# Gryph66/gymwipe

Measured on AMD Instinct MI355X. Metric: env.step()/s at 65 536 parallel envs, counter-traffic band-assign, higher is better.
Workload: dtype f64

## Files before the change

### gymwipe_amd/_native.py

```python
import ctypes as C
import os
import subprocess

_PKG = os.path.dirname(os.path.abspath(__file__))
LIB_PATH = os.environ.get("GW_LIB") or os.path.join(_PKG, "lib", "libgymwipe_amd.so")
CSRC = os.path.join(_PKG, "csrc")

ABI_VERSION = 1
MAX_DEVICES = 32
MAX_RADIOS = MAX_DEVICES + 1
QUEUE_CAP = 100
MAX_NSTATES = 16

OK, EINVAL, ENODEVICE, EHIP, ENOMEM, EUNSUPPORTED, EFIELD = 0, -1, -2, -3, -4, -5, -6
FLAG_CARRY, FLAG_REFEXC, FLAG_TIE, FLAG_BADACT, FLAG_INTERNAL = 1, 2, 4, 8, 16
CFG_PER_ENV_STATS = 1
CFG_EXPLICIT_QUEUE = 2
CFG_NO_COUNTER_TRAFFIC = 4
CFG_PEER_RECEIVE = 8
CFG_FLOAT_DURATION = 16
CFG_PER_ENV_GEOMETRY = 32

EXPORTS = (
    "gw_abi_version", "gw_last_error", "gw_device_count", "gw_config_default", "gw_create",
    "gw_destroy", "gw_reset", "gw_step", "gw_step_fb", "gw_rollout", "gw_rollout_policy", "gw_rollout_policy_stats", "gw_transition_stats", "gw_rollout_episodes", "gw_rollout_episodes_stats", "gw_transition_stats_ep", "gw_rollout_autoreset", "gw_rollout_population", "gw_rollout_episodes_scored", "gw_rollout_population_scored", "gw_rollout_autoreset_scored", "gw_rollout_backlog", "gw_rollout_backlog_population", "gw_rollout_controller", "gw_rollout_controller_population", "gw_rollout_policy_stats_delivered", "gw_rollout_episodes_stats_delivered", "gw_transition_stats_delivered", "gw_set_position", "gw_set_positions", "gw_received", "gw_delivered", "gw_enqueue", "gw_pack_feedback", "gw_unpack_feedback", "gw_get_state",
    "gw_stats_read", "gw_clear_flags", "gw_state_bytes", "gw_snapshot_bytes", "gw_get_snapshot", "gw_set_state", "gw_link_info", "gw_noise_states", "gw_selftest_queue", "gw_selftest_runq",
    "gw_selftest_fastmath", "gw_selftest_launches",
    "gw_plant_config_default", "gw_plant_create", "gw_plant_destroy", "gw_plant_update", "gw_plant_set_input",
    "gw_plant_state_ptr", "gw_plant_get_state", "gw_plant_feedback", "gw_plant_update_feedback", "gw_now_ptr", "gw_pendulum_step",
    "gw_ctrl_config_default", "gw_ctrl_create", "gw_ctrl_destroy", "gw_ctrl_step", "gw_ctrl_get_state",
    "gw_ctrl_set_initial", "gw_ctrl_reset", "gw_ctrl_rollout", "gw_ctrl_rollout_schedules",
    "gw_grid_config_default", "gw_grid_create", "gw_grid_destroy", "gw_grid_run", "gw_grid_get_state", "gw_grid_set_position",
)


class Config(C.Structure):
    _fields_ = [
        ("abi_version", C.c_int32),
        ("hip_device", C.c_int32),
        ("num_envs", C.c_int64),
        ("num_devices", C.c_int32),
        ("flags", C.c_int32),
        ("pos", (C.c_double * 2) * MAX_RADIOS),
        ("mult", C.c_int32 * MAX_DEVICES),
        ("dest", C.c_int32 * MAX_DEVICES),
        ("slot", C.c_double),
        ("frequency", C.c_double),
        ("bandwidth", C.c_double),
        ("temperature_c", C.c_double),
        ("bit_rate", C.c_double),
        ("code_rate", C.c_double),
        ("max_ber", C.c_double),
        ("tx_power_dbm", C.c_double),
        ("counter_interval", C.c_double),
        ("counter_bound", C.c_int32),
        ("payload_value", C.c_int32),
        ("mac_header_bytes", C.c_int32),
        ("net_header_bytes", C.c_int32),
        ("duration_factor", C.c_int32),
        ("max_duration", C.c_int32),
        ("extra_att_db", (C.c_double * MAX_RADIOS) * MAX_RADIOS),
        ("start_time", C.c_double),
    ]


class CtrlConfig(C.Structure):
    _fields_ = [
        ("net", Config),
        ("A", C.c_double * 16), ("B", C.c_double * 4), ("x0", C.c_double * 4), ("u0", C.c_double),
        ("ctrl_start_tick", C.c_int32), ("ctrl_period_ticks", C.c_int32),
    ]


class CtrlEpisodes(C.Structure):
    _fields_ = [("max_steps", C.c_int32), ("pad", C.c_int32), ("fail_deg", C.c_double)]


class PlantConfig(C.Structure):
    _fields_ = [
        ("abi_version", C.c_int32),
# ... 152 lines not shown
    L.gw_transition_stats_ep.restype = C.c_int
    L.gw_rollout_autoreset.argtypes = [vp, i32, vp, vp, C.POINTER(Episodes), vp, vp, vp, vp, vp, vp]
    L.gw_rollout_autoreset.restype = C.c_int
    L.gw_rollout_population.argtypes = [vp, i32, C.POINTER(Population), C.c_uint64, C.c_uint64, C.c_uint64, C.POINTER(Episodes), vp, vp, vp]
    L.gw_rollout_population.restype = C.c_int
    L.gw_rollout_episodes_scored.argtypes = [vp, i32, vp, C.c_uint64, C.c_uint64, C.c_uint64, C.POINTER(Episodes), C.POINTER(Score),
                                             vp, vp, vp, vp, vp, vp, vp, vp, vp, vp]
    L.gw_rollout_episodes_scored.restype = C.c_int
    L.gw_rollout_population_scored.argtypes = [vp, i32, C.POINTER(Population), C.c_uint64, C.c_uint64, C.c_uint64, C.POINTER(Episodes),
                                               C.POINTER(Score), vp, vp, vp]
    L.gw_rollout_population_scored.restype = C.c_int
    L.gw_rollout_autoreset_scored.argtypes = [vp, i32, vp, vp, C.POINTER(Episodes), C.POINTER(Score), vp, vp, vp, vp, vp, vp, vp]
    L.gw_rollout_autoreset_scored.restype = C.c_int
    L.gw_rollout_backlog.argtypes = [vp, i32, C.POINTER(BacklogPolicy), C.POINTER(Episodes), C.POINTER(Score), vp, vp, vp, vp, vp, vp, vp,
                                     vp, vp, vp]
    L.gw_rollout_backlog.restype = C.c_int
    L.gw_rollout_backlog_population.argtypes = [vp, i32, C.POINTER(BacklogPopulation), C.POINTER(Episodes), C.POINTER(Score), vp, vp]
    L.gw_rollout_backlog_population.restype = C.c_int
    L.gw_rollout_controller.argtypes = [vp, i32, C.POINTER(Controller), C.c_uint64, C.c_uint64, C.c_uint64, C.POINTER(Episodes),
                                        C.POINTER(Score), vp, vp, vp, vp, vp, vp, vp, vp, vp, vp, vp]
    L.gw_rollout_controller.restype = C.c_int
    L.gw_rollout_controller_population.argtypes = [vp, i32, C.POINTER(ControllerPopulation), C.c_uint64, C.c_uint64, C.c_uint64,
                                                   C.POINTER(Episodes), C.POINTER(Score), vp, vp, vp]
    L.gw_rollout_controller_population.restype = C.c_int
    L.gw_rollout_policy_stats_delivered.argtypes = L.gw_rollout_policy_stats.argtypes
    L.gw_rollout_policy_stats_delivered.restype = C.c_int
    L.gw_rollout_episodes_stats_delivered.argtypes = L.gw_rollout_episodes_stats.argtypes
    L.gw_rollout_episodes_stats_delivered.restype = C.c_int
    L.gw_transition_stats_delivered.argtypes = [vp, i32, vp, vp, vp, vp, vp, vp, vp, vp, vp, vp]
    L.gw_transition_stats_delivered.restype = C.c_int
    L.gw_received.argtypes, L.gw_received.restype = [vp, vp, vp], C.c_int
    L.gw_enqueue.argtypes, L.gw_enqueue.restype = [vp, i32, vp, vp], C.c_int
    L.gw_pack_feedback.argtypes, L.gw_pack_feedback.restype = [vp, C.c_int64, vp, vp, vp, vp, i32, vp], C.c_int
    L.gw_unpack_feedback.argtypes, L.gw_unpack_feedback.restype = [vp, C.c_int64, vp, vp, vp, vp, vp], C.c_int
    L.gw_delivered.argtypes, L.gw_delivered.restype = [vp, vp, vp], C.c_int
    L.gw_get_state.argtypes, L.gw_get_state.restype = [vp, C.c_char_p, vp, C.c_size_t], C.c_int
    L.gw_stats_read.argtypes, L.gw_stats_read.restype = [vp, C.POINTER(Stats)], C.c_int
    L.gw_state_bytes.argtypes, L.gw_state_bytes.restype = [vp, C.POINTER(C.c_uint64)], C.c_int
    L.gw_snapshot_bytes.argtypes, L.gw_snapshot_bytes.restype = [vp, C.POINTER(C.c_uint64)], C.c_int
    L.gw_get_snapshot.argtypes, L.gw_get_snapshot.restype = [vp, vp, C.c_uint64], C.c_int
    L.gw_set_state.argtypes, L.gw_set_state.restype = [vp, vp, C.c_uint64], C.c_int
    L.gw_link_info.argtypes = [vp, i32, i32, C.POINTER(C.c_double), C.POINTER(C.c_double)]
    L.gw_link_info.restype = C.c_int
    L.gw_noise_states.argtypes = [vp, i32, C.POINTER(i32), C.POINTER(C.c_double)]
    L.gw_noise_states.restype = C.c_int
    L.gw_selftest_queue.argtypes, L.gw_selftest_queue.restype = [C.c_uint64, i32, i32, i32], C.c_int
    L.gw_set_position.argtypes, L.gw_set_position.restype = [vp, i32, vp, vp, vp, vp], C.c_int
    L.gw_set_positions.argtypes, L.gw_set_positions.restype = [vp, vp, vp, vp], C.c_int
    L.gw_clear_flags.argtypes, L.gw_clear_flags.restype = [vp, vp], C.c_int
    L.gw_selftest_runq.argtypes, L.gw_selftest_runq.restype = [C.c_uint64, i32, i32, i32], C.c_int
    L.gw_selftest_fastmath.argtypes = [C.POINTER(Config), C.POINTER(i32)]
    L.gw_selftest_fastmath.restype = C.c_int
    L.gw_selftest_launches.argtypes, L.gw_selftest_launches.restype = [vp, C.c_char_p, i64], i64
    L.gw_plant_config_default.argtypes, L.gw_plant_config_default.restype = [C.POINTER(PlantConfig), i64], C.c_int
    L.gw_plant_create.argtypes, L.gw_plant_create.restype = [C.POINTER(PlantConfig), C.POINTER(vp)], C.c_int
    L.gw_plant_destroy.argtypes, L.gw_plant_destroy.restype = [vp], C.c_int
    L.gw_plant_update.argtypes, L.gw_plant_update.restype = [vp, vp, i64, vp], C.c_int
    L.gw_plant_set_input.argtypes, L.gw_plant_set_input.restype = [vp, vp, vp, vp], C.c_int
    L.gw_plant_state_ptr.argtypes, L.gw_plant_state_ptr.restype = [vp, C.POINTER(vp)], C.c_int
    L.gw_plant_get_state.argtypes, L.gw_plant_get_state.restype = [vp, C.c_char_p, vp, C.c_size_t], C.c_int
    L.gw_plant_feedback.argtypes, L.gw_plant_feedback.restype = [vp, vp, vp, vp, vp], C.c_int
    L.gw_ctrl_config_default.argtypes, L.gw_ctrl_config_default.restype = [C.POINTER(CtrlConfig), i64], C.c_int
    L.gw_ctrl_create.argtypes, L.gw_ctrl_create.restype = [C.POINTER(CtrlConfig), C.POINTER(vp)], C.c_int
    L.gw_ctrl_destroy.argtypes, L.gw_ctrl_destroy.restype = [vp], C.c_int
    L.gw_ctrl_step.argtypes, L.gw_ctrl_step.restype = [vp, vp, vp, vp, vp, vp, vp], C.c_int
    L.gw_ctrl_get_state.argtypes, L.gw_ctrl_get_state.restype = [vp, C.c_char_p, vp, C.c_size_t], C.c_int
    L.gw_ctrl_set_initial.argtypes, L.gw_ctrl_set_initial.restype = [vp, vp, vp, vp, vp], C.c_int
    L.gw_ctrl_reset.argtypes, L.gw_ctrl_reset.restype = [vp, vp, vp, vp], C.c_int
    L.gw_ctrl_rollout.argtypes = [vp, C.c_int32, vp, vp, C.POINTER(CtrlEpisodes), vp, vp, vp, vp, vp]
    L.gw_ctrl_rollout.restype = C.c_int
    L.gw_ctrl_rollout_schedules.argtypes = [vp, C.c_int32, vp, C.c_int32, C.c_int32, C.POINTER(CtrlEpisodes), vp, vp]
    L.gw_ctrl_rollout_schedules.restype = C.c_int
    L.gw_plant_update_feedback.argtypes, L.gw_plant_update_feedback.restype = [vp, vp, C.c_int64, vp, vp, vp, vp], C.c_int
    L.gw_now_ptr.argtypes, L.gw_now_ptr.restype = [vp, C.POINTER(vp), C.POINTER(i64)], C.c_int
    L.gw_pendulum_step.argtypes, L.gw_pendulum_step.restype = [vp, vp, vp, vp, vp, vp, vp, vp], C.c_int
    L.gw_grid_config_default.argtypes, L.gw_grid_config_default.restype = [C.POINTER(GridConfig), i64, i32], C.c_int
    L.gw_grid_create.argtypes, L.gw_grid_create.restype = [C.POINTER(GridConfig), vp, C.POINTER(vp)], C.c_int
    L.gw_grid_destroy.argtypes, L.gw_grid_destroy.restype = [vp], C.c_int
    L.gw_grid_run.argtypes, L.gw_grid_run.restype = [vp, C.c_double, vp], C.c_int
    L.gw_grid_get_state.argtypes, L.gw_grid_get_state.restype = [vp, C.c_char_p, vp, C.c_size_t], C.c_int
    L.gw_grid_set_position.argtypes, L.gw_grid_set_position.restype = [vp, i32, vp, vp, vp], C.c_int
    if L.gw_abi_version() != ABI_VERSION:
        raise ImportError("gymwipe_amd: ABI mismatch (library %d, python %d); rebuild"
                          % (L.gw_abi_version(), ABI_VERSION))
    _lib = L
    return L


_fast = False


def fast():
    global _fast
    if _fast is False:
        _fast = None
        path = os.path.join(os.path.dirname(LIB_PATH), "_gw_fast.so")
        if os.path.exists(path) and not os.environ.get("GW_NO_PYFAST"):
            try:
                import importlib.machinery
                import importlib.util
                loader = importlib.machinery.ExtensionFileLoader("_gw_fast", path)
                spec = importlib.util.spec_from_loader("_gw_fast", loader)
                mod = importlib.util.module_from_spec(spec)
                loader.exec_module(mod)
                L = lib()
                mod.bind(C.cast(L.gw_step, C.c_void_p).value, C.cast(L.gw_pendulum_step, C.c_void_p).value,
# ... 18 lines not shown
```

### gymwipe_amd/csrc/ct_common.hip.h

```cpp
#pragma once
#include <hip/hip_runtime.h>
#include "gw_internal.h"
#include "gw_queue.h"
#include "gw_fastmath.h"

#ifdef GW_STAMPS
#define STAMP(i)                                                                              \
    do {                                                                                      \
        __builtin_amdgcn_sched_barrier(0);                                                    \
        unsigned long long _t;                                                                \
        asm volatile("s_memtime %0\n\ts_waitcnt lgkmcnt(0)" : "=s"(_t)::"memory");            \
        __builtin_amdgcn_sched_barrier(0);                                                    \
        if ((threadIdx.x & 63) == 0)                                                          \
            st.stamps[(((size_t)blockIdx.x * ((blockDim.x + 63) >> 6)) + (threadIdx.x >> 6)) * 16 + (i)] = _t; \
    } while (0)
#else
#define STAMP(i) do { } while (0)
#endif

namespace gwk {

typedef GwTally Tally;

struct TxTimes { double t_s, t_h, t_e, stop; };
// ... 70 lines not shown
        u32x4_ w; __builtin_memcpy(&w, &v, 16);
        asm volatile("global_store_dwordx4 %0, %1, off sc1\n\ts_nop 1" ::"v"(ptr), "v"(w) : "memory");
    } else if constexpr (sizeof(T) == 8) {
        unsigned long long w; __builtin_memcpy(&w, &v, 8);
        asm volatile("global_store_dwordx2 %0, %1, off sc1" ::"v"(ptr), "v"(w) : "memory");
    } else if constexpr (sizeof(T) == 4) {
        unsigned w; __builtin_memcpy(&w, &v, 4);
        asm volatile("global_store_dword %0, %1, off sc1" ::"v"(ptr), "v"(w) : "memory");
    } else {
        static_assert(sizeof(T) == 1, "gw_store_wt: 1, 4, 8 or 16 bytes");
        unsigned w = (unsigned)*reinterpret_cast<const uint8_t*>(&v);
        asm volatile("global_store_byte %0, %1, off sc1" ::"v"(ptr), "v"(w) : "memory");
    }
#endif
}

template <class T, class Off>
__device__ __forceinline__ T ld(const void* base, Off byte_off)
{
    return *reinterpret_cast<const T*>(reinterpret_cast<const char*>(base) + byte_off);
}
template <class T, class Off>
__device__ __forceinline__ T ld_global(const void* base, Off byte_off)
{
#if defined(__HIP_DEVICE_COMPILE__)
    return *(const __attribute__((address_space(1))) T*)(reinterpret_cast<const char*>(base) + byte_off);
#else
    return *reinterpret_cast<const T*>(reinterpret_cast<const char*>(base) + byte_off);
#endif
}
template <class T, class Off>
__device__ __forceinline__ void st_(void* base, Off byte_off, const T& v)
{
    gw_store_wt(reinterpret_cast<T*>(reinterpret_cast<char*>(base) + byte_off), v);
}
template <class T, class Off>
__device__ __forceinline__ void st_plain(void* base, Off byte_off, const T& v)
{
    *reinterpret_cast<T*>(reinterpret_cast<char*>(base) + byte_off) = v;
}

__device__ __forceinline__ uint32_t byte_of(uint32_t x, uint32_t y, uint32_t z, uint32_t w, uint32_t idx)
{
    const uint32_t lo = (idx & 4u) ? y : x;
    const uint32_t hi = (idx & 4u) ? w : z;
    const uint32_t v = (idx & 8u) ? hi : lo;
    return (v >> ((idx & 3u) * 8u)) & 0xffu;
}
__device__ __forceinline__ uint32_t word_of(const uint4& w, int i)
{
    return i == 0 ? w.x : (i == 1 ? w.y : (i == 2 ? w.z : w.w));
}

__device__ __forceinline__ void publish_env_counters(uint32_t* sa, uint32_t N, uint32_t e, uint32_t pop, uint32_t deliv,
                                                     uint32_t bad, uint32_t fl, uint32_t steps)
{
    if (pop)
        __hip_atomic_fetch_add(reinterpret_cast<unsigned long long*>(sa) + e, (unsigned long long)pop | ((unsigned long long)deliv << 32),
                               __ATOMIC_RELAXED, __HIP_MEMORY_SCOPE_AGENT);
    if (bad) __hip_atomic_fetch_add(sa + (size_t)2 * N + e, bad, __ATOMIC_RELAXED, __HIP_MEMORY_SCOPE_AGENT);
    if (fl)  __hip_atomic_fetch_or(sa + (size_t)3 * N + e, fl, __ATOMIC_RELAXED, __HIP_MEMORY_SCOPE_AGENT);
    if (e == 0u)
        __hip_atomic_fetch_add(reinterpret_cast<unsigned long long*>(sa + (size_t)4 * N), (unsigned long long)steps,
                               __ATOMIC_RELAXED, __HIP_MEMORY_SCOPE_AGENT);
}

__device__ __forceinline__ double ber_bpsk_dev(double sig_mw, double noise_mw, double ten_log_br)
{
    const double s = 10 * log10(sig_mw);
    const double n = 10 * log10(noise_mw);
    if (s <= n) return 0.5;
    const double ratio_db = s - n - ten_log_br;
    const double ratio = pow(10.0, ratio_db / 10);
    const double x = sqrt(2 * ratio);
    const double e = 2.718281828459045;
    const double sqrt2pi = 2.5066282746310002;
    return (1 - pow(e, -1.4 * x)) * pow(e, -(pow(x, 2.0) / 2)) / (1.135 * sqrt2pi * x);
}

template <bool PER_ENV>
__device__ __forceinline__ double gw_link(const GwState& st, int R, int from, int to, uint32_t e)
{
    if (PER_ENV) return st.prx_env[((size_t)e * R + from) * gw_rp(R) + to];
    return st.prx_tab[from * R + to];
}
__device__ __forceinline__ double& gw_rx(const GwState& st, int R, int j, int64_t e)
{
    return st.rxp[(size_t)e * gw_rp(R) + j];
}


#define GW_LEAD_PARAMS uint32_t* __restrict__ ip, double* __restrict__ tw, uint32_t* __restrict__ tk, uint8_t* __restrict__ qb, \
                       const int32_t* __restrict__ device, const int32_t* __restrict__ duration, uint32_t n_envs, uint32_t dev_stage
#define GW_LEAD_PARAMS_U64 uint64_t ip_a, uint64_t tw_a, uint64_t tk_a, uint64_t qb_a, uint64_t device_a, uint64_t duration_a, \
                           uint32_t n_envs, uint32_t dev_stage
#define GW_LEAD_ARGS(st_) (st_).ip, (st_).tw, (st_).tk, (st_).qb, device, duration, (uint32_t)(st_).N, \
                          ((uint32_t)(st_).D | ((uint32_t)(st_).stage_chunks << 8))
#if defined(__HIP_DEVICE_COMPILE__)
#define GW_AS_CONST __attribute__((address_space(4)))
#else
#define GW_AS_CONST
#endif
template <int DT>
__device__ __forceinline__ GwDevConst hdr_const(const uint32_t* ip, int n_dev)
{
    const int D = DT > 0 ? DT : n_dev;
    const uint8_t* at = reinterpret_cast<const uint8_t*>(ip) - gw_blob_header(D) + gw_hdr_cst_off(D);
    return *(const GW_AS_CONST GwDevConst*)at;
}
template <class T>
__device__ __forceinline__ T* gw_as_global(T* p)
{
    return (T*)(__attribute__((address_space(1))) T*)p;
}
template <class T>
__device__ __forceinline__ T* gw_global_at(uint64_t address)
{
    return (T*)(__attribute__((address_space(1))) T*)address;
}
template <int DT>
__device__ __forceinline__ GwState hdr_state(uint32_t* ip, double* tw, uint32_t* tk, uint8_t* qb, uint32_t n_envs, int n_dev)
{
    const int D = DT > 0 ? DT : n_dev;
    const uint8_t* base = reinterpret_cast<const uint8_t*>(ip) - gw_blob_header(D);
    GwState st = *(const GW_AS_CONST GwState*)(base + gw_hdr_st_off(D));
    st.ip = ip; st.tw = tw; st.tk = tk; st.qb = qb; st.N = (int64_t)n_envs; st.D = D;
    st.blob = base;
#define GW_G(m) st.m = gw_as_global(st.m)
    GW_G(bph); GW_G(sa); GW_G(trans); GW_G(ber); GW_G(cls); GW_G(ber2); GW_G(cls2); GW_G(rxp); GW_G(prx_tab); GW_G(pos_tab);
    GW_G(extra_tab); GW_G(prx_env); GW_G(pos_env); GW_G(bcache); GW_G(talk); GW_G(stamps); GW_G(cst);
#undef GW_G
    return st;
}

__device__ __forceinline__ int ndigits(int v)
{
    return 1 + (v >= 10) + (v >= 100) + (v >= 1000) + (v >= 10000) + (v >= 100000) + (v >= 1000000) +
           (v >= 10000000) + (v >= 100000000) + (v >= 1000000000);
}


template <int CTRL, int ROW_MASK, bool OR>
__device__ __forceinline__ uint32_t gw_dpp_step(uint32_t v)
{
    const uint32_t o = (uint32_t)__builtin_amdgcn_update_dpp(0, (int)v, CTRL, ROW_MASK, 0xf, false);
    return OR ? (v | o) : (v + o);
}
template <bool OR>
__device__ __forceinline__ uint32_t gw_wave_total(uint32_t v)
{
    v = gw_dpp_step<0x111, 0xf, OR>(v);
    v = gw_dpp_step<0x112, 0xf, OR>(v);
    v = gw_dpp_step<0x114, 0xf, OR>(v);
    v = gw_dpp_step<0x118, 0xf, OR>(v);
    v = gw_dpp_step<0x142, 0xa, OR>(v);
    v = gw_dpp_step<0x143, 0xc, OR>(v);
    return (uint32_t)__builtin_amdgcn_readlane((int)v, 63);
}

__device__ __forceinline__ void publish_totals(unsigned long long* totals, const Tally& k, uint32_t k_steps,
                                               uint32_t k_bad, uint32_t fl_new)
{
    const uint32_t lane = threadIdx.x & 63u;
    const uint32_t w_deliv = gw_wave_total<false>(k.deliv), w_pop = gw_wave_total<false>(k.pop);
    const uint32_t w_app = gw_wave_total<false>(k.app), w_drop = gw_wave_total<false>(k.drop);
    const uint32_t w_steps = (uint32_t)__builtin_popcountll(__builtin_amdgcn_ballot_w64(k_steps != 0u));
    const uint32_t w_bad = (uint32_t)__builtin_popcountll(__builtin_amdgcn_ballot_w64(k_bad != 0u));
    const uint32_t w_tx = w_steps + w_pop;
    uint32_t w_fl = 0u;
    if (__builtin_amdgcn_ballot_w64(fl_new != 0u)) w_fl = gw_wave_total<true>(fl_new);
    if (lane < (uint32_t)GW_T_COUNT) {
        uint32_t w = w_steps;
        w = lane == (uint32_t)GW_T_TX ? w_tx : w;
        w = lane == (uint32_t)GW_T_DELIV ? w_deliv : w;
        w = lane == (uint32_t)GW_T_APP ? w_app : w;
        w = lane == (uint32_t)GW_T_POP ? w_pop : w;
        w = lane == (uint32_t)GW_T_DROP ? w_drop : w;
        w = lane == (uint32_t)GW_T_FLAGS ? w_fl : w;
        w = lane == (uint32_t)GW_T_BAD ? w_bad : w;
// ... 15 lines not shown
```

### gymwipe_amd/csrc/ct_rollout_backlog.hip

```cpp
#include "ct_rollout_sync.hip.h"

namespace {

struct BacklogEpisodes : ScoredStagedEpisodes {
    const uint32_t* s_w;
    const uint8_t* s_dur;
    int32_t* device_out;
    int32_t* duration_out;
    int32_t* seen_len;
    int du_cur;
    uint32_t q_cur;
    __device__ __forceinline__ void stage(const gw_backlog_policy& pol, int D, uint32_t* lds_w, uint8_t* lds_dur) const
    {
        for (int i = threadIdx.x; i < D; i += blockDim.x) lds_w[i] = (uint32_t)pol.w_len[i];
        for (int i = threadIdx.x; i <= GW_QUEUE_CAP; i += blockDim.x) lds_dur[i] = pol.duration_of_len[i];
    }
    template <int DT, class ARR>
    __device__ __forceinline__ int pick(ARR& len, int D, int max_duration)
    {
        const int n = DT ? DT : D;
        uint32_t q = len[0], p = s_w[0] * q;
        int d = 0;
#pragma unroll
        for (int i = 1; i < n; ++i) {
// ... 70 lines not shown
            if (i < (uint32_t)D) lds_w[i] = gw_backlog_weight((int32_t)v);
            if (i >= W) reinterpret_cast<uint32_t*>(lds_dur)[i - W] = v;
        }
    }
};

template <int DT, int MODE>
__global__ __launch_bounds__(64) void ct_rollout_backlog_pop(GwState st, GwDevConst c, int K, GwEpisodeArgs ea, gw_score w,
                                                            const gw_backlog_policy* __restrict__ policies, uint32_t M, int64_t* pop_tally)
{
    __shared__ uint32_t s_score_w[DT == 0 ? GW_MAX_DEVICES : DT];
    __shared__ uint32_t s_backlog_w[DT == 0 ? GW_MAX_DEVICES : DT];
    __shared__ __attribute__((aligned(4))) uint8_t s_backlog_dur[(GW_QUEUE_CAP + 1 + 3) / 4 * 4];
    __shared__ unsigned long long s_ep_tally[GW_EP_COLS];
    static_assert(sizeof(gw_backlog_policy) == 4u * GW_MAX_DEVICES + sizeof s_backlog_dur, "the table's dwords fill its LDS copy");
    BacklogPopulationEpisodes src;
    src.ended = nullptr;
    src.latest_next = 0;
    src.sc.weights_at(s_score_w, w);
    src.delivered_out = nullptr;
    src.d_cur = 0; src.du_cur = 0; src.q_cur = 0;
    src.s_w = s_backlog_w; src.s_dur = s_backlog_dur;
    src.device_out = nullptr; src.duration_out = nullptr; src.seen_len = nullptr;
    const uint32_t pol_next = (blockIdx.x * 64u) / M;
    src.row = pop_tally + (size_t)pol_next * GW_EP_COLS;
#define GW_ROLLOUT_SRC_RESETS
#define GW_ROLLOUT_SRC_QUEUES
#define GW_ROLLOUT_SRC_STAGE                                                                                                     \
    src.sc.stage(w, DT == 0 ? c.D : DT);                                                                                         \
    src.stage_from(policies + pol_next, DT == 0 ? c.D : DT, s_backlog_w, s_backlog_dur);                                         \
    gw_ep_zero(s_ep_tally);
#define GW_BACKLOG_POP_PIN(x) asm volatile("" : "+s"(x))
    GW_BACKLOG_POP_PIN(K);
#define GW_ROLLOUT_SRC_FIRST                                                                                                     \
    src.ep.load(ea, e); src.sc.first();                                                                                          \
    GW_BACKLOG_POP_PIN(src.ep.max_steps); GW_BACKLOG_POP_PIN(src.ep.on_done); GW_BACKLOG_POP_PIN(src.sc.w_reward);
#define GW_ROLLOUT_SRC_TAKE                                                                                                      \
    queues_now();                                                                                                                \
    const int d = src.pick<DT>(len, D, c.max_duration), du = src.du_cur;
#define GW_ROLLOUT_SRC_CHECKED(bad) false
#define GW_ROLLOUT_SRC_STEPPED(at, latest, r, dn)                                                                                \
    (void)at;                                                                                                                    \
    {                                                                                                                            \
        const int32_t score_next = src.sc.of(r, src.d_cur, src.sc.delivered(kt.deliv));                                          \
        GW_ROLLOUT_EP_STEPPED(score_next, dn)                                                                                    \
        src.latest_next = cause_next ? 0 : latest;                                                                               \
    }
#include "ct_rollout_sync_body.h"
#undef GW_BACKLOG_POP_PIN
    GW_ROLLOUT_EP_TAIL(true, src.row)
}

template <bool CLAMP>
__device__ __forceinline__ void gw_backlog_select(const uint8_t* row, uint32_t D, uint32_t md, const gw_backlog_policy& pol, uint32_t& d_out,
                                                  uint32_t& du_out, uint32_t& q_out)
{
    auto weight = [&](uint32_t i) { return CLAMP ? gw_backlog_weight(pol.w_len[i]) : (uint32_t)pol.w_len[i]; };
    uint32_t q = row[0], p = weight(0) * q, d = 0;
    for (uint32_t i = 1; i < D; ++i) {
        const uint32_t qi = row[i], pi = weight(i) * qi;
        const bool more = pi > p;
        p = more ? pi : p; q = more ? qi : q; d = more ? i : d;
    }
    d_out = d;
    du_out = gw_min_u32((uint32_t)pol.duration_of_len[gw_min_u32(q, (uint32_t)GW_QUEUE_CAP)], md - 1u);
    q_out = q;
}
__global__ __launch_bounds__(256) void backlog_select_rows(uint32_t N, uint32_t D, uint32_t RB, uint32_t md, gw_backlog_policy pol,
                                                           const uint8_t* __restrict__ qb, int32_t* __restrict__ device_out,
                                                           int32_t* __restrict__ duration_out, int32_t* __restrict__ seen_len)
{
    const uint32_t e = blockIdx.x * blockDim.x + threadIdx.x;
    if (e >= N) return;
    uint32_t d, du, q;
    gw_backlog_select<false>(qb + (size_t)e * RB, D, md, pol, d, du, q);
    device_out[e] = (int32_t)d;
    duration_out[e] = (int32_t)du;
    seen_len[e] = (int32_t)q;
}
__global__ __launch_bounds__(256) void backlog_select_pop_rows(uint32_t N, uint32_t D, uint32_t RB, uint32_t md, uint32_t M,
                                                               const gw_backlog_policy* __restrict__ policies,
                                                               const uint8_t* __restrict__ qb, int32_t* __restrict__ device_out,
                                                               int32_t* __restrict__ duration_out)
{
    const uint32_t e = blockIdx.x * blockDim.x + threadIdx.x;
    if (e >= N) return;
    uint32_t d, du, q;
    gw_backlog_select<true>(qb + (size_t)e * RB, D, md, policies[e / M], d, du, q);
    device_out[e] = (int32_t)d;
    duration_out[e] = (int32_t)du;
}

}

int gw_launch_rollout_backlog_sfx(const GwState& st, const GwDevConst& cst, const GwChunk& ch, const gw_backlog_policy& pol,
                                  const gw_episodes& ep, const gw_score& score, int32_t* obs_next, const GwRows& out, int32_t* seen_len,
                                  int32_t* delivered)
{
    if (fused_unavailable(st, cst, ch.K, GW_FUSED_NO_TABLE)) return GW_EUNSUPPORTED;
    return launch_fused(st, cst, ch, GW_LS_ROLLOUT_BACKLOG, GW_FUSED_NO_TABLE, GW_KERNEL_OF(ct_rollout_backlog), episode_args(ep, obs_next),
                        score, pol, out.device, out.duration, seen_len, out.obs, out.reward, out.done, out.ended, delivered);
}
int gw_launch_backlog_select(const GwState& st, const GwDevConst& cst, const gw_backlog_policy& pol, const GwRows& row, int32_t* seen_len,
                             void* stream)
{
    hipLaunchKernelGGL(backlog_select_rows, dim3((unsigned)((st.N + 255) / 256)), dim3(256), 0, (hipStream_t)stream, (uint32_t)st.N,
                       (uint32_t)st.D, (uint32_t)st.RB, (uint32_t)cst.max_duration, pol, (const uint8_t*)st.qb, row.device, row.duration,
                       seen_len);
    return gw_launch_status();
}

int gw_launch_rollout_backlog_pop_sfx(const GwState& st, const GwDevConst& cst, const GwChunk& ch, const gw_backlog_population& pop,
                                      const gw_episodes& ep, const gw_score& score, int32_t* obs_next)
{
    if (fused_unavailable(st, cst, ch.K, GW_FUSED_NO_TABLE) || pop.envs_per_policy % 64 != 0) return GW_EUNSUPPORTED;
    return launch_fused(st, cst, ch, GW_LS_ROLLOUT_BACKLOG_POP, GW_FUSED_NO_TABLE, GW_KERNEL_OF(ct_rollout_backlog_pop),
                        episode_args(ep, obs_next), score, pop.policies_dev, (uint32_t)pop.envs_per_policy, pop.tally_dev);
}
int gw_launch_backlog_select_pop(const GwState& st, const GwDevConst& cst, const gw_backlog_population& pop, const GwRows& row, void* stream)
{
    hipLaunchKernelGGL(backlog_select_pop_rows, dim3((unsigned)((st.N + 255) / 256)), dim3(256), 0, (hipStream_t)stream, (uint32_t)st.N,
                       (uint32_t)st.D, (uint32_t)st.RB, (uint32_t)cst.max_duration, (uint32_t)pop.envs_per_policy, pop.policies_dev,
                       (const uint8_t*)st.qb, row.device, row.duration);
    return gw_launch_status();
}
```

### gymwipe_amd/csrc/ct_rollout_sfx.hip

```cpp
#include "ct_rollout_sync.hip.h"

namespace {


constexpr int TP_ENVS = 64, TP_STEPS = 64;

__global__ __launch_bounds__(256) void pack_actions_kernel(uint32_t N, int K, int Kp, const int32_t* __restrict__ device,
                                                           const int32_t* __restrict__ duration, uint16_t* __restrict__ packed)
{
    __shared__ __attribute__((aligned(16))) uint16_t tile[TP_ENVS][TP_STEPS + 2];
    const uint32_t e0 = blockIdx.x * TP_ENVS;
    const int t = threadIdx.x;
    const bool vec_ok = (N & 3u) == 0;
    for (int k0 = 0; k0 < Kp; k0 += TP_STEPS) {
        const int c4 = (t & 15) * 4, r = t >> 4;
#pragma unroll
        for (int pass = 0; pass < TP_STEPS / 16; ++pass) {
            const int kk = pass * 16 + r, k = k0 + kk;
            uint32_t v[4] = {0xffffu, 0xffffu, 0xffffu, 0xffffu};
            if (k < K) {
                int32_t dv[4], du[4];
                const uint32_t e = e0 + (uint32_t)c4;
                if (vec_ok && e + 3 < N) {
                    const int4 a = *reinterpret_cast<const int4*>(device + (size_t)k * N + e);
// ... 66 lines not shown
                    *reinterpret_cast<int4*>(obs + (size_t)k * N + e) = make_int4(o[0], o[1], o[2], o[3]);
                    *reinterpret_cast<float4*>(reward + (size_t)k * N + e) = make_float4(rw[0], rw[1], rw[2], rw[3]);
                    *reinterpret_cast<uchar4*>(done + (size_t)k * N + e) = make_uchar4(dn[0], dn[1], dn[2], dn[3]);
                } else {
                    for (int j = 0; j < 4 && e + j < N; ++j) {
                        obs[(size_t)k * N + e + j] = o[j]; reward[(size_t)k * N + e + j] = rw[j]; done[(size_t)k * N + e + j] = dn[j];
                    }
                }
            }
        }
        __syncthreads();
    }
}

template <int DT, int MODE>
__global__ __launch_bounds__(256) void ct_rollout_sfx_kernel(GwState st, GwDevConst c, int K, int Kp,
                                                            const uint16_t* __restrict__ actions,
                                                            uint8_t* __restrict__ feedback)
{
    constexpr bool GEN = DT == 0;
    constexpr int DM = GEN ? GW_MAX_DEVICES : DT;
    constexpr int NWC = (2 * DM + 1 + 15) / 16;
    constexpr int S = GW_MAX_NSTATES;
    const int D = GEN ? c.D : DT, R = D + 1, RRM = D;
    const uint32_t N = (uint32_t)st.N;
    const uint32_t e = blockIdx.x * blockDim.x + threadIdx.x;

    constexpr int TRANS_B = ((DM + 1) * (DM + 1) * S + 15) / 16 * 16;
    __shared__ __attribute__((aligned(16))) uint8_t s_trans[TRANS_B];
    __shared__ __attribute__((aligned(16))) double  s_ber[2 * DM * S];
    __shared__ __attribute__((aligned(16))) uint8_t s_cls[2 * DM * S];
    __shared__ uint32_t s_cols[GEN ? (3 * DM + 1) * 64 : 1];
    __shared__ uint2 s_mi[GEN ? DM : 1];
    __shared__ uint32_t s_term[GEN ? DM : 1];
    if constexpr (GEN) {
        for (int i = threadIdx.x; i < D; i += blockDim.x) {
            s_mi[i] = make_uint2((uint32_t)st.cst->mult[i], st.cst->inv16[i]);
            s_term[i] = st.cst->term[i];
        }
    }
    {
        const int n_tr = (R * R * S + 15) >> 4, n_be = (2 * D * S * 8) >> 4, n_cl = (2 * D * S) >> 4;
        for (int i = threadIdx.x; i < n_tr; i += blockDim.x) *reinterpret_cast<uint4*>(s_trans + ((uint32_t)i << 4)) = ld<uint4>(st.trans, (uint32_t)i << 4);
        for (int i = threadIdx.x; i < n_be; i += blockDim.x) *reinterpret_cast<uint4*>(reinterpret_cast<uint8_t*>(s_ber) + ((uint32_t)i << 4)) = ld<uint4>(st.ber2, (uint32_t)i << 4);
        for (int i = threadIdx.x; i < n_cl; i += blockDim.x) *reinterpret_cast<uint4*>(s_cls + ((uint32_t)i << 4)) = ld<uint4>(st.cls2, (uint32_t)i << 4);
    }
    __syncthreads();
    if (e >= N) return;

    const uint32_t RB = GEN ? (uint32_t)st.RB : 16u * NWC;
    const uint32_t o16 = e << 4, oq = e * RB;
    const uint4 ip = ld<uint4>(st.ip, o16);
    const double2 tw = ld<double2>(st.tw, o16);
    const uint4 tk = ld<uint4>(st.tk, o16);
    typename ArrSel<GEN, DM>::rw len, tb;
    typename ArrSel<GEN, DM + 1>::rw sta;
    if constexpr (GEN) {
        uint32_t* col = s_cols + (threadIdx.x & 63);
        len.p = col; tb.p = col + DM * 64; sta.p = col + 2 * DM * 64;
        for (int i = 0; i < D; ++i) len[i] = st.qb[oq + (uint32_t)i];
        for (int j = 0; j < R; ++j) sta[j] = st.qb[oq + (uint32_t)(D + j)];
    } else {
        uint4 qw[NWC];
#pragma unroll
        for (int w = 0; w < NWC; ++w) qw[w] = ld<uint4>(st.qb, oq + 16u * w);
#pragma unroll
        for (int i = 0; i < DT; ++i) len[i] = (word_of(qw[i >> 4], (i >> 2) & 3) >> ((i & 3) * 8)) & 0xffu;
#pragma unroll
        for (int j = 0; j < DT + 1; ++j) sta[j] = (word_of(qw[(DT + j) >> 4], ((DT + j) >> 2) & 3) >> (((DT + j) & 3) * 8)) & 0xffu;
    }
    double now = tw.x, wake = tw.y;
    uint32_t tau = tk.x;
    const uint32_t nbp = tk.y;
    GwBp bpc, bpp;
    bpc.t0 = ip.x; bpc.c0 = ip.y;
    bpp.t0 = ip.z; bpp.c0 = ip.w;
    const GwBp* hist = st.bph + ((size_t)e << 7);
    uint32_t rvm = tk.z;
    int32_t last_abs = (int32_t)(tk.w & 0x7fffffffu);
    uint32_t dn = tk.w >> 31;

    constexpr bool FAST = MODE >= 1, NOLIM = MODE == 2;
    const StepMathT<FAST, NOLIM> m(c);
    const double slot = c.slot, br = c.bit_rate, hd = c.hdr_dur, hdr_bits = c.hdr_bits, interval = c.counter_interval;
    const double inv_interval = c.inv_interval, tie_filter = c.tie_filter;
    const bool fast_ticks = FAST || c.fast_ticks != 0;
    const uint32_t bound = (uint32_t)c.counter_bound, base_bytes = (uint32_t)(c.mac_hdr + c.net_hdr);
    const int mh = c.mac_hdr, pv = c.payload_value;
    uint32_t live_mask = 0u;
    if constexpr (GEN) {
        for (int i = 0; i < D; ++i) live_mask |= ((s_term[i] >> sta[i]) & 1u) ? 0u : (1u << i);
    }
    typename ArrSel<GEN, DM>::ro mult, term, inv16;
    if constexpr (GEN) {
        mult.p = st.cst->mult; mult.shift16 = 0; term.p = st.cst->term; term.shift16 = 1; inv16.p = st.cst->inv16; inv16.shift16 = 0;
    } else {
#pragma unroll
        for (int i = 0; i < DT; ++i) { mult.v[i] = (uint32_t)c.mult[i]; term.v[i] = c.term[i]; inv16.v[i] = c.inv16[i]; }
    }

    Tally kt = {0, 0, 0, 0, 0};
    uint32_t k_bad = 0, fl = 0;

    int k = 0;
    bool data_mode = false;
    bool finish = false;
    int d = 0;
    uint32_t len_d = 0, mult_d = 0, inv16_d = 65536u;
#pragma unroll
    for (int i = 0; i < D; ++i) tb[i] = tau;
    uint32_t n_data = 0, s_r_run = 0;
    double cur = now, stopw = 0.0, t_end = 0.0;
    bool cls_valid = false;
    uint32_t fbw = 0;

    const uint16_t* act = actions + (size_t)e * Kp;
    uint8_t* fbp = feedback + (size_t)e * Kp;
    uint4 aw = ld<uint4>(act, 0);

    auto put_feedback = [&](uint32_t byte) {
        fbw |= byte << ((k & 3) * 8);
        if ((k & 3) == 3 || k == K - 1) { st_plain(fbp, (uint32_t)(k & ~3), fbw); fbw = 0; }
        k++;
        if ((k & 7) == 0 && k < K) aw = ld<uint4>(act, (uint32_t)k * 2u);
    };

    while (k < K) {
        uint32_t s = 0;
        if (data_mode && !finish) {
            bool have = true;
            if (len_d == 0) {
                if (mult_d != 0u && wake < stopw) {
// ... 147 lines not shown
        {
            uint32_t kk = 0;
            double wj = wake;
            bool tiej = false;
            if (fast_ticks && gw_tick_jump(wake, cur, interval, inv_interval, incl, &kk, &wj, &tiej)) {
                wake = wj;
                if (tiej) fl |= GW_FLAG_TIE;
            } else {
                kk = 0;
                for (;;) {
                    const double w1 = wake + interval, w2 = w1 + interval, w3 = w2 + interval, w4 = w3 + interval;
                    const bool b0 = incl ? (wake <= cur) : (wake < cur);
                    const bool b1 = incl ? (w1 <= cur) : (w1 < cur);
                    const bool b2 = incl ? (w2 <= cur) : (w2 < cur);
                    const bool b3 = incl ? (w3 <= cur) : (w3 < cur);
                    if (incl && (wake == cur || w1 == cur || w2 == cur || w3 == cur)) fl |= GW_FLAG_TIE;
                    kk += (uint32_t)b0 + (uint32_t)b1 + (uint32_t)b2 + (uint32_t)b3;
                    wake = b3 ? w4 : (b2 ? w3 : (b1 ? w2 : (b0 ? w1 : wake)));
                    if (!b3) break;
                }
            }
            tau += kk;
            len_d = gw_len_after_ticks(len_d, kk, mult_d, kt);
        }
    }

    {
        uint32_t kk = 0;
        while (wake <= now) { if (wake == now) fl |= GW_FLAG_TIE; wake = wake + interval; kk++; }
        tau += kk;
#pragma unroll
        for (int i = 0; i < D; ++i) len[i] = gw_len_after_ticks(len[i], tau - tb[i], mult[i], kt);
    }

    if constexpr (GEN) {
        for (int i = 0; i < D; ++i) st.qb[oq + (uint32_t)i] = (uint8_t)len[i];
        for (int j = 0; j < R; ++j) st.qb[oq + (uint32_t)(D + j)] = (uint8_t)sta[j];
    } else {
        uint32_t nb[16 * NWC];
#pragma unroll
        for (int b = 0; b < 16 * NWC; ++b) nb[b] = 0u;
#pragma unroll
        for (int i = 0; i < DT; ++i) nb[i] = len[i];
#pragma unroll
        for (int j = 0; j < DT + 1; ++j) nb[DT + j] = sta[j];
#pragma unroll
        for (int w = 0; w < NWC; ++w) {
            const int b = 16 * w;
            uint4 o;
            o.x = nb[b + 0] | (nb[b + 1] << 8) | (nb[b + 2] << 16) | (nb[b + 3] << 24);
            o.y = nb[b + 4] | (nb[b + 5] << 8) | (nb[b + 6] << 16) | (nb[b + 7] << 24);
            o.z = nb[b + 8] | (nb[b + 9] << 8) | (nb[b + 10] << 16) | (nb[b + 11] << 24);
            o.w = nb[b + 12] | (nb[b + 13] << 8) | (nb[b + 14] << 16) | (nb[b + 15] << 24);
            st_plain(st.qb, oq + 16u * w, o);
        }
    }
    st_plain(st.tw, o16, make_double2(now, wake));
    st_plain(st.tk, o16, make_uint4(tau, nbp, rvm, (uint32_t)last_abs | (dn << 31)));
    publish_env_counters(st.sa, N, e, kt.pop, kt.deliv, k_bad, fl, (uint32_t)K);
}

template <int DT, int MODE>
__global__ __launch_bounds__(64) void ct_rollout_sync_kernel(GwState st, GwDevConst c, int K,
                                                            const int32_t* __restrict__ device, const int32_t* __restrict__ duration,
                                                            int32_t* __restrict__ obs, float* __restrict__ reward, uint8_t* __restrict__ done)
{
#define GW_ROLLOUT_SRC_STAGE
#define GW_ROLLOUT_SRC_FIRST GW_ROLLOUT_STAGED_FIRST
#define GW_ROLLOUT_SRC_TAKE GW_ROLLOUT_STAGED_TAKE
#define GW_ROLLOUT_SRC_CHECKED(bad) GW_ROLLOUT_STAGED_CHECKED(bad)
#define GW_ROLLOUT_SRC_STEPPED(at, latest, r, dn) GW_ROLLOUT_STORE_OUTPUTS(at, latest, r, dn)
#include "ct_rollout_sync_body.h"
}

}

int gw_launch_rollout_sfx(const GwState& st, const GwDevConst& cst, const GwChunk& ch, const int32_t* device, const int32_t* duration,
                          const GwRows& out)
{
    const int K = ch.K, Kp = (K + 15) / 16 * 16, k_cap = st.rcap;
    uint16_t* const act_buf = st.ract;
    uint8_t* const fb_buf = st.rfb;
    int32_t* const obs = out.obs;
    float* const reward = out.reward;
    uint8_t* const done = out.done;
    if (K <= 0 || Kp > k_cap) return GW_EUNSUPPORTED;
    const bool event_loop = getenv("GW_ROLLOUT_EVENT_LOOP") != nullptr && act_buf != nullptr && fb_buf != nullptr;
    if (!event_loop)
        return launch_fused(st, cst, ch, GW_LS_ROLLOUT_SYNC, GW_FUSED_NO_TABLE, GW_KERNEL_OF(ct_rollout_sync_kernel), device, duration,
                            obs, reward, done);
    const unsigned grid = (unsigned)((st.N + 63) / 64);
    const int mode = gw_step_mode(cst, ch.below_limits, false);
    hipStream_t s = (hipStream_t)ch.stream;
    uint64_t* const rec = ch.rec;
    if (cst.max_duration > 0xfe) return GW_EUNSUPPORTED;
    const uint32_t N = (uint32_t)st.N;
    const unsigned g256 = (unsigned)((st.N + TP_ENVS - 1) / TP_ENVS);
    hipLaunchKernelGGL(pack_actions_kernel, dim3(g256), dim3(256), 0, s, N, K, Kp, device, duration, act_buf);
    gw_with_dt<GW_DTS_ROLLOUT_LOOP>(st.D, [&](auto dt) {
        gw_with_mode(mode, [&](auto m) {
            gw_note_launch(rec, GW_LS_ROLLOUT + 3 * gw_ls_dt(decltype(dt)::value) + decltype(m)::value);
            hipLaunchKernelGGL((ct_rollout_sfx_kernel<decltype(dt)::value, decltype(m)::value>), dim3(grid), dim3(64), 0, s,
                               st, cst, K, Kp, (const uint16_t*)act_buf, fb_buf);
        });
    });
    if (const int rc = gw_launch_status()) return rc;
    hipLaunchKernelGGL(expand_feedback_kernel, dim3(g256), dim3(256), 0, s, N, K, Kp, cst.counter_bound,
                       cst.payload_value, fb_buf, obs, reward, done);
    return gw_launch_status();
}
```

### gymwipe_amd/csrc/ct_rollout_sync_body.h

```cpp
    constexpr bool GEN = DT == 0;
    constexpr int DM = GEN ? GW_MAX_DEVICES : DT;
    constexpr int NWC = (2 * DM + 1 + 15) / 16;
    constexpr int S = GW_MAX_NSTATES;
    const int D = GEN ? c.D : DT, R = D + 1, RRM = D;
    const uint32_t N = (uint32_t)st.N;
    const uint32_t e = blockIdx.x * blockDim.x + threadIdx.x;

    constexpr int TRANS_B = ((DM + 1) * (DM + 1) * S + 15) / 16 * 16;
    __shared__ __attribute__((aligned(16))) uint8_t s_trans[TRANS_B];
    __shared__ __attribute__((aligned(16))) double  s_ber[2 * DM * S];
    __shared__ __attribute__((aligned(16))) uint8_t s_cls[2 * DM * S];
    __shared__ uint32_t s_cols[GEN ? (3 * DM + 1) * 64 : 1];
    __shared__ uint2 s_mi[GEN ? DM : 1];
    __shared__ uint32_t s_term[GEN ? DM : 1];
    if constexpr (GEN) {
        for (int i = threadIdx.x; i < D; i += blockDim.x) {
            s_mi[i] = make_uint2((uint32_t)st.cst->mult[i], st.cst->inv16[i]);
            s_term[i] = st.cst->term[i];
        }
    }
    {
        const int n_tr = (R * R * S + 15) >> 4, n_be = (2 * D * S * 8) >> 4, n_cl = (2 * D * S) >> 4;
        for (int i = threadIdx.x; i < n_tr; i += blockDim.x) *reinterpret_cast<uint4*>(s_trans + ((uint32_t)i << 4)) = ld<uint4>(st.trans, (uint32_t)i << 4);
        for (int i = threadIdx.x; i < n_be; i += blockDim.x) *reinterpret_cast<uint4*>(reinterpret_cast<uint8_t*>(s_ber) + ((uint32_t)i << 4)) = ld<uint4>(st.ber2, (uint32_t)i << 4);
        for (int i = threadIdx.x; i < n_cl; i += blockDim.x) *reinterpret_cast<uint4*>(s_cls + ((uint32_t)i << 4)) = ld<uint4>(st.cls2, (uint32_t)i << 4);
    }
    GW_ROLLOUT_SRC_STAGE
    __syncthreads();
    if (e >= N) return;

    const uint32_t RB = GEN ? (uint32_t)st.RB : 16u * NWC;
    const uint32_t o16 = e << 4, oq = e * RB;
    const uint4 ip = ld<uint4>(st.ip, o16);
    const double2 tw = ld<double2>(st.tw, o16);
    const uint4 tk = ld<uint4>(st.tk, o16);
    typename ArrSel<GEN, DM>::rw len, tb;
    typename ArrSel<GEN, DM + 1>::rw sta;
    if constexpr (GEN) {
        uint32_t* col = s_cols + (threadIdx.x & 63);
        len.p = col; tb.p = col + DM * 64; sta.p = col + 2 * DM * 64;
        for (int i = 0; i < D; ++i) len[i] = st.qb[oq + (uint32_t)i];
        for (int j = 0; j < R; ++j) sta[j] = st.qb[oq + (uint32_t)(D + j)];
    } else {
        uint4 qw[NWC];
#pragma unroll
        for (int w = 0; w < NWC; ++w) qw[w] = ld<uint4>(st.qb, oq + 16u * w);
#pragma unroll
        for (int i = 0; i < DT; ++i) len[i] = (word_of(qw[i >> 4], (i >> 2) & 3) >> ((i & 3) * 8)) & 0xffu;
#pragma unroll
        for (int j = 0; j < DT + 1; ++j) sta[j] = (word_of(qw[(DT + j) >> 4], ((DT + j) >> 2) & 3) >> (((DT + j) & 3) * 8)) & 0xffu;
    }
    double now = tw.x, wake = tw.y;
    uint32_t tau = tk.x;
    uint32_t nbp = tk.y;
    GwBp bpc, bpp;
    bpc.t0 = ip.x; bpc.c0 = ip.y;
    bpp.t0 = ip.z; bpp.c0 = ip.w;
    const GwBp* hist = st.bph + ((size_t)e << 7);
    uint32_t rvm = tk.z;
    int32_t last_abs = (int32_t)(tk.w & 0x7fffffffu);
    uint32_t dn = tk.w >> 31;

    constexpr bool FAST = MODE >= 1, NOLIM = MODE == 2;
    const StepMathT<FAST, NOLIM> m(c);
    const double slot = c.slot, br = c.bit_rate, hd = c.hdr_dur, hdr_bits = c.hdr_bits, interval = c.counter_interval;
    const double inv_interval = c.inv_interval, tie_filter = c.tie_filter, coded_factor = c.coded_factor;
    const bool fast_ticks = FAST || c.fast_ticks != 0;
    const bool idem = c.idem_states != 0;
    const uint32_t bound = (uint32_t)c.counter_bound, base_bytes = (uint32_t)(c.mac_hdr + c.net_hdr);
    const int mh = c.mac_hdr, pv = c.payload_value;
    uint32_t live_mask = 0u;
    if constexpr (GEN) {
        for (int i = 0; i < D; ++i) live_mask |= ((s_term[i] >> sta[i]) & 1u) ? 0u : (1u << i);
    }
    typename ArrSel<GEN, DM>::ro mult, term, inv16;
    if constexpr (GEN) {
        mult.p = st.cst->mult; mult.shift16 = 0; term.p = st.cst->term; term.shift16 = 1; inv16.p = st.cst->inv16; inv16.shift16 = 0;
    } else {
#pragma unroll
        for (int i = 0; i < DT; ++i) { mult.v[i] = (uint32_t)c.mult[i]; term.v[i] = c.term[i]; inv16.v[i] = c.inv16[i]; }
    }
#pragma unroll
    for (int i = 0; i < D; ++i) tb[i] = tau;

    Tally kt = {0, 0, 0, 0, 0};
    uint32_t k_bad = 0, fl = 0;
    int k = 0;
    GW_ROLLOUT_SRC_FIRST
#ifdef GW_ROLLOUT_SRC_RESETS
    auto reset_env = [&]() {
        uint32_t kk = 0;
        while (wake <= now) { if (wake == now) fl |= GW_FLAG_TIE; wake = wake + interval; kk++; }
        tau += kk;
        GwBp* ring = st.bph + ((size_t)e << 7);
        GwBp cur; cur.t0 = bpc.t0; cur.c0 = 0u;
        if (bpc.t0 == tau) {
            ring[(nbp - 1u) & GW_RING_MASK] = cur;
        } else {
            bpp = bpc;
            cur.t0 = tau;
            ring[nbp & GW_RING_MASK] = cur;
            nbp += 1u;
        }
        bpc = cur;
        rvm = 0u; last_abs = 0; dn = 0u;
    };
#endif
#ifdef GW_ROLLOUT_SRC_QUEUES
    auto queues_now = [&]() {
        uint32_t kk = 0;
        while (wake <= now) { if (wake == now) fl |= GW_FLAG_TIE; wake = wake + interval; kk++; }
        tau += kk;
#pragma unroll
// ... 189 lines not shown
            for (int i = 0; i < D; ++i)
                if (i == d) { len[i] = len_d; tb[i] = tau; }
        }
        if (!all_term) {
#pragma unroll
            for (int i = 0; i < D; ++i) {
                if (i == d) continue;
                uint32_t si = s_trans[(uint32_t)((i * R + RRM) * S) + sta[i]];
                for (uint32_t n = 0; n < n_data; ++n) {
                    const uint32_t s2 = s_trans[(uint32_t)((i * R + d) * S) + si];
                    if (s2 == si) break;
                    si = s2;
                }
                sta[i] = si;
                if constexpr (GEN) live_mask = ((term[i] >> si) & 1u) ? (live_mask & ~(1u << i)) : (live_mask | (1u << i));
            }
        }
        sta[RRM] = s_r;
        const int32_t latest = pv * ((int)(rvm & 1u) - (int)((rvm >> 1) & 1u));
        const int32_t abs_d = latest < 0 ? -latest : latest;
        int32_t r = last_abs - abs_d;
        last_abs = abs_d;
        r = r > 10 ? 10 : (r < -10 ? -10 : r);
        now = t_end;
        put_feedback(latest, r);
    }

    {
        uint32_t kk = 0;
        while (wake <= now) { if (wake == now) fl |= GW_FLAG_TIE; wake = wake + interval; kk++; }
        tau += kk;
#pragma unroll
        for (int i = 0; i < D; ++i) len[i] = gw_len_after_ticks(len[i], tau - tb[i], mult[i], kt);
    }
    if constexpr (GEN) {
        for (int i = 0; i < D; ++i) st.qb[oq + (uint32_t)i] = (uint8_t)len[i];
        for (int j = 0; j < R; ++j) st.qb[oq + (uint32_t)(D + j)] = (uint8_t)sta[j];
    } else {
        uint32_t nb[16 * NWC];
#pragma unroll
        for (int b = 0; b < 16 * NWC; ++b) nb[b] = 0u;
#pragma unroll
        for (int i = 0; i < DT; ++i) nb[i] = len[i];
#pragma unroll
        for (int j = 0; j < DT + 1; ++j) nb[DT + j] = sta[j];
#pragma unroll
        for (int w = 0; w < NWC; ++w) {
            const int b = 16 * w;
            uint4 o;
            o.x = nb[b + 0] | (nb[b + 1] << 8) | (nb[b + 2] << 16) | (nb[b + 3] << 24);
            o.y = nb[b + 4] | (nb[b + 5] << 8) | (nb[b + 6] << 16) | (nb[b + 7] << 24);
            o.z = nb[b + 8] | (nb[b + 9] << 8) | (nb[b + 10] << 16) | (nb[b + 11] << 24);
            o.w = nb[b + 12] | (nb[b + 13] << 8) | (nb[b + 14] << 16) | (nb[b + 15] << 24);
            st_plain(st.qb, oq + 16u * w, o);
        }
    }
    st_plain(st.tw, o16, make_double2(now, wake));
    st_plain(st.tk, o16, make_uint4(tau, nbp, rvm, (uint32_t)last_abs | (dn << 31)));
    publish_env_counters(st.sa, N, e, kt.pop, kt.deliv, k_bad, fl, (uint32_t)K);
#undef GW_ROLLOUT_SRC_RESETS
#undef GW_ROLLOUT_SRC_QUEUES
#undef GW_ROLLOUT_SRC_STAGE
#undef GW_ROLLOUT_SRC_FIRST
#undef GW_ROLLOUT_SRC_TAKE
#undef GW_ROLLOUT_SRC_CHECKED
#undef GW_ROLLOUT_SRC_STEPPED
```

### gymwipe_amd/csrc/ct_step_sfx.hip

```cpp
#include "ct_common.hip.h"
#include "gw_dispatch.h"
#include "gw_queue.h"

using namespace gwk;


namespace {



#define PIN_V(x) asm volatile("" : "+v"(x))
#define PIN_S(x) asm volatile("" : "+s"(x))

template <int DT, bool FEEDBACK, int MODE, bool HALF = false>
__device__ __forceinline__ void ct_step_sfx_body(const GwState& st, const GwDevConst& c,
                                                 const int32_t* __restrict__ device,
                                                 const int32_t* __restrict__ duration,
                                                 int32_t* __restrict__ obs,
                                                 float* __restrict__ reward,
                                                 uint8_t* __restrict__ done,
                                                 uint8_t* __restrict__ fb,
                                                 int n_stage,
                                                 double& now_out, bool& live_out)
{
    constexpr bool PACKED = DT > 0;
    constexpr bool FAST = MODE >= 1, NOLIM = MODE == 2;
    constexpr int NWC = DT > 0 ? (2 * DT + 1 + 15) / 16 : 1;
    const uint32_t N = (uint32_t)st.N;
    const uint32_t e = HALF ? blockIdx.x * 32u + (threadIdx.x & 31u) : blockIdx.x * 64u + threadIdx.x;
    const int D = DT > 0 ? DT : c.D;
    const int R = D + 1, RRM = D;
    constexpr int S = GW_MAX_NSTATES;
    const uint32_t RB = PACKED ? 16u * NWC : (uint32_t)st.RB;

    STAMP(0);
    constexpr int DM = DT > 0 ? DT : GW_MAX_DEVICES;
    constexpr GwStripeLayout LM(DM);
    const GwStripeLayout L(D);
    constexpr int MAX_CH = LM.staged_chunks(GW_MAX_NSTATES);
    const int n_ch = n_stage < MAX_CH ? n_stage : MAX_CH;
    const int tid = threadIdx.x;
    constexpr int nthr = 64;
    constexpr int PER_FULL = (MAX_CH + 63) / 64;
    constexpr int PER = (DT > 0 && PER_FULL <= 11) ? PER_FULL : 1;
    constexpr bool one_pass = DT > 0 && PER_FULL <= 11;
    __shared__ __attribute__((aligned(16))) uint8_t s_blob[one_pass ? PER * 64 * 16 : MAX_CH * 16];
    uint4 r_ch[PER];
    if (one_pass) {
#pragma unroll
        for (int i = 0; i < PER; ++i) {
            const int ch = tid + i * nthr;
            r_ch[i] = ld<uint4>(st.blob, (uint32_t)(ch < n_ch ? ch : 0) << 4);
        }
    }

    Tally k = {0, 0, 0, 0, 0};
    uint32_t k_bad = 0;

    const bool live = e < N && (!HALF || threadIdx.x < 32u);
    const uint32_t el = live ? e : 0u;
    const uint32_t o16 = e << 4, o16l = el << 4;
    const uint32_t oq = e * RB, oql = el * RB;
    int d = device[el];
    int du = duration[el];
    uint4 ip = ld<uint4>(st.ip, o16l);
    const double2 tw = ld<double2>(st.tw, o16l);
    const uint4 tk = ld<uint4>(st.tk, o16l);
    uint4 qw[NWC];
#pragma unroll
    for (int w = 0; w < NWC; ++w) qw[w] = PACKED ? ld<uint4>(st.qb, oql + 16u * w) : make_uint4(0u, 0u, 0u, 0u);
    now_out = tw.x;
    live_out = live;
    if (one_pass) {
#pragma unroll
        for (int i = 0; i < PER; ++i) {
            const int ch = tid + i * nthr;
            *reinterpret_cast<uint4*>(s_blob + ((uint32_t)ch << 4)) = r_ch[i];
        }
    } else {
        for (int i = tid; i < n_ch; i += nthr) *reinterpret_cast<uint4*>(s_blob + ((uint32_t)i << 4)) = ld<uint4>(st.blob, (uint32_t)i << 4);
    }
    STAMP(1);
    __syncthreads();
    STAMP(2);

    StepMathT<FAST, NOLIM> m(c);
    double slot = c.slot, br = c.bit_rate, hd = c.hdr_dur, hdr_bits = c.hdr_bits, interval = c.counter_interval;
    double coded_factor = c.coded_factor, cls_limit = c.cls_limit, inv_interval_lo = c.inv_interval_lo, inv_slot_lo = c.inv_slot_lo;
    int pv = c.payload_value, cbound = c.counter_bound, max_duration = c.max_duration, dfactor = c.duration_factor;
    int mh = c.mac_hdr, base_b = c.mac_hdr + c.net_hdr, idem_i = c.idem_states, fast_ticks = c.fast_ticks;
    __builtin_amdgcn_sched_barrier(0);
    PIN_S(m.slot); PIN_S(m.inv_slot); PIN_S(m.fmod_limit); PIN_S(m.dr); PIN_S(m.rcp_dr); PIN_S(m.max_ber);
    if (!FAST) { PIN_S(m.fast_fmod); PIN_S(m.fast_div); PIN_S(m.fast_decide); }
    PIN_S(slot); PIN_S(br); PIN_S(hd); PIN_S(hdr_bits); PIN_S(interval); PIN_S(coded_factor); PIN_S(cls_limit); PIN_S(inv_interval_lo); PIN_S(inv_slot_lo);
    PIN_S(pv); PIN_S(cbound); PIN_S(max_duration); PIN_S(dfactor); PIN_S(mh); PIN_S(base_b); PIN_S(idem_i); PIN_S(fast_ticks);
    if (FEEDBACK) { PIN_S(obs); PIN_S(reward); PIN_S(done); PIN_S(fb); }
    __builtin_amdgcn_sched_barrier(0);

    PIN_V(d); PIN_V(du);
    PIN_V(ip.x); PIN_V(ip.y); PIN_V(ip.z); PIN_V(ip.w);
    const uint2* s_mi = reinterpret_cast<const uint2*>(s_blob + L.mi);
    const uint8_t* s_st = s_blob + L.s0;
    const uint8_t* g_h2 = st.blob + L.h2;
    const uint32_t STR = (uint32_t)L.stripe, DD = (uint32_t)D;
    auto t_ber0 = [&](uint32_t dd, uint32_t ss) { return *reinterpret_cast<const double*>(s_st + ss * STR + (uint32_t)L.ber0 + dd * 8u); };
    auto t_ber1 = [&](uint32_t dd, uint32_t ss) { return *reinterpret_cast<const double*>(s_st + ss * STR + (uint32_t)L.ber1 + dd * 8u); };
    auto t_h1 = [&](uint32_t j, uint32_t ss) { return (uint32_t)s_st[ss * STR + (uint32_t)L.h1 + j]; };
    auto t_r1 = [&](uint32_t dd, uint32_t ss) { return (uint32_t)s_st[ss * STR + (uint32_t)L.r1 + dd]; };
    auto t_cls0 = [&](uint32_t dd, uint32_t ss) { return (uint32_t)s_st[ss * STR + (uint32_t)L.cls0 + dd]; };
    auto t_cls1 = [&](uint32_t dd, uint32_t ss) { return (uint32_t)s_st[ss * STR + (uint32_t)L.cls1 + dd]; };
    auto t_h2 = [&](uint32_t j, uint32_t dd, uint32_t ss) { return (uint32_t)g_h2[(ss * DD + j) * DD + dd]; };

    if (live) {
        uint32_t rvm = tk.z;
#ifdef GW_STAMPS
        asm volatile("" : "+v"(rvm));
#endif
        STAMP(3);
        int32_t last_abs = (int32_t)(tk.w & 0x7fffffffu);
        uint32_t dn = tk.w >> 31;
        uint32_t fl = 0;

        if ((unsigned)d >= (unsigned)D || (unsigned)du >= (unsigned)max_duration) {
            fl = GW_FLAG_BADACT;
            k_bad = 1;
            const int32_t latest = pv * ((int)(rvm & 1u) - (int)((rvm >> 1) & 1u));
            if (FEEDBACK) {
                obs[e] = latest + cbound;
                reward[e] = 0.0f;
                done[e] = (uint8_t)dn;
                if (fb) fb[e] = (uint8_t)((uint32_t)(((latest > 0) - (latest < 0)) + 1) | (10u << 2) | (dn << 7));
            }
        } else {
            const uint32_t bound = (uint32_t)cbound;
            const uint32_t base_bytes = (uint32_t)base_b;
            const bool idem = FAST || idem_i != 0;

            uint32_t len_d, s_d_old, s_r_old;
            if (PACKED) {
                if (NWC == 1) {
                    uint32_t q0 = qw[0].x, q1 = qw[0].y, q2 = qw[0].z, q3 = qw[0].w;
                    asm volatile("" : "+v"(q0), "+v"(q1), "+v"(q2), "+v"(q3));
                    len_d = byte_of(q0, q1, q2, q3, (uint32_t)d);
                    s_d_old = byte_of(q0, q1, q2, q3, (uint32_t)(DT + d));
                } else {
                    uint32_t lx = 0, ly = 0, lz = 0, lw = 0, sx = 0, sy = 0, sz = 0, sw = 0;
#pragma unroll
                    for (int w = 0; w < NWC; ++w) {
                        uint32_t q0 = qw[w].x, q1 = qw[w].y, q2 = qw[w].z, q3 = qw[w].w;
                        asm volatile("" : "+v"(q0), "+v"(q1), "+v"(q2), "+v"(q3));
                        const bool hl = ((uint32_t)d >> 4) == (uint32_t)w, hs = ((uint32_t)(DT + d) >> 4) == (uint32_t)w;
                        lx = hl ? q0 : lx; ly = hl ? q1 : ly; lz = hl ? q2 : lz; lw = hl ? q3 : lw;
                        sx = hs ? q0 : sx; sy = hs ? q1 : sy; sz = hs ? q2 : sz; sw = hs ? q3 : sw;
                    }
                    len_d = byte_of(lx, ly, lz, lw, (uint32_t)d & 15u);
                    s_d_old = byte_of(sx, sy, sz, sw, (uint32_t)(DT + d) & 15u);
                }
                s_r_old = (word_of(qw[(2 * DT) >> 4], ((2 * DT) >> 2) & 3) >> (((2 * DT) & 3) * 8)) & 0xffu;
            } else {
                len_d = st.qb[oq + (uint32_t)d];
                s_d_old = st.qb[oq + (uint32_t)(D + d)];
                s_r_old = st.qb[oq + (uint32_t)(2 * D)];
            }
            const double t_a = tw.x;
            double wake = tw.y;
            const uint32_t tau0 = tk.x, nbp = tk.y;
            GwBp bpc, bpp;
            bpc.t0 = ip.x; bpc.c0 = ip.y;
            bpp.t0 = ip.z; bpp.c0 = ip.w;
            const GwBp* hist = st.bph + ((size_t)e << 7);
            const uint32_t s_d = t_h1((uint32_t)d, s_d_old);
            const uint32_t s_r1 = t_r1((uint32_t)d, s_r_old);
            const uint2 mi = s_mi[d];
            uint32_t nb[PACKED ? 16 * NWC : 1];
            uint32_t n1[PACKED ? DT : 1], n2[PACKED ? DT : 1], mlt[PACKED ? DT : 1];
            if (PACKED) {
#pragma unroll
                for (int b = 0; b < 16 * NWC; ++b) nb[b] = (word_of(qw[b >> 4], (b >> 2) & 3) >> ((b & 3) * 8)) & 0xffu;
#pragma unroll
                for (int i = 0; i < DT; ++i) {
                    n1[i] = t_h1((uint32_t)i, nb[DT + i]);
                    n2[i] = t_h2((uint32_t)i, (uint32_t)d, nb[DT + i]);
                    mlt[i] = s_mi[i].x;
                }
            }
            const double ber_a = t_ber0((uint32_t)d, s_d);
            const uint32_t cls_a = t_cls0((uint32_t)d, s_d);
            const double ber_x1 = t_ber1((uint32_t)d, s_r1);
            const uint32_t cls_x1 = t_cls1((uint32_t)d, s_r1);
            uint32_t s_r = s_r_old;
            const uint32_t mult_d = mi.x;
            const uint32_t inv16_d = mi.y;
// ... 132 lines not shown
                        s_r = s_r1;
                    } else {
                        s_r = st.trans[(uint32_t)((RRM * R + d) * S) + s_r];
                        ber_x = st.ber[(uint32_t)((RRM * R + d) * S) + s_r];
                        cls_x = st.cls[(uint32_t)((RRM * R + d) * S) + s_r];
                    }
                    const bool ok = decode(m, cls_x, cls_valid, ber_x, x, br, hdr_bits,
                                           (double)(pay * 8) * coded_factor, fl);
                    k.deliv += ok ? 1u : 0u;
                    rvm |= ok ? (1u << d) : 0u;
                    dn = (ok && pv == cbound) ? 1u : dn;
                    fl |= !(x.t_e < t_end) ? (uint32_t)GW_FLAG_CARRY : 0u;
                    ticks_upto(x.t_e, true);
                    cur = x.t_e;
                    if (!(cur < stopw)) break;
                }
            }

            STAMP(7);
            ticks_upto(t_end, true);
            STAMP(8);
            const uint32_t n_ticks = tau - tau0;
            k.app += kd.app;
            k.drop += kd.drop;

            auto heard_slow = [&](int j, uint32_t s0) {
                uint32_t s = st.trans[(uint32_t)((j * R + RRM) * S) + s0];
                for (int n = 0; n < n_data; ++n) s = st.trans[(uint32_t)((j * R + d) * S) + s];
                return s;
            };
            if (PACKED) {
                const uint32_t heard_data = n_data ? 0xffffffffu : 0u;
#pragma unroll
                for (int i = 0; i < DT; ++i) {
                    Tally ki = {0, 0, 0, 0, 0};
                    const uint32_t li = gw_len_after_ticks(nb[i], n_ticks, mlt[i], ki);
                    uint32_t si = (n2[i] & heard_data) | (n1[i] & ~heard_data);
                    if (!idem) si = heard_slow(i, nb[DT + i]);
                    if (i != d) { k.app += ki.app; k.drop += ki.drop; }
                    nb[i] = (i == d) ? len_d : li;
                    nb[DT + i] = (i == d) ? s_d : si;
                }
                nb[2 * DT] = s_r;
                uint4 o[NWC];
#pragma unroll
                for (int w = 0; w < NWC; ++w) {
                    const int b = 16 * w;
                    o[w].x = nb[b + 0] | (nb[b + 1] << 8) | (nb[b + 2] << 16) | (nb[b + 3] << 24);
                    o[w].y = nb[b + 4] | (nb[b + 5] << 8) | (nb[b + 6] << 16) | (nb[b + 7] << 24);
                    o[w].z = nb[b + 8] | (nb[b + 9] << 8) | (nb[b + 10] << 16) | (nb[b + 11] << 24);
                    o[w].w = nb[b + 12] | (nb[b + 13] << 8) | (nb[b + 14] << 16) | (nb[b + 15] << 24);
                }
                STAMP(9);
#pragma unroll
                for (int w = 0; w < NWC; ++w) st_(st.qb, oq + 16u * w, o[w]);
            } else {
                for (int i = 0; i < D; ++i) {
                    if (i == d) continue;
                    const uint32_t l0 = st.qb[oq + (uint32_t)i];
                    const uint32_t s0 = st.qb[oq + (uint32_t)(D + i)];
                    const uint32_t s1 = !idem ? heard_slow(i, s0)
                                              : (n_data ? t_h2((uint32_t)i, (uint32_t)d, s0) : t_h1((uint32_t)i, s0));
                    st.qb[oq + (uint32_t)i] = (uint8_t)gw_len_after_ticks(l0, n_ticks, s_mi[i].x, k);
                    if (s1 != s0) st.qb[oq + (uint32_t)(D + i)] = (uint8_t)s1;
                }
                st.qb[oq + (uint32_t)d] = (uint8_t)len_d;
                if (s_d != s_d_old) st.qb[oq + (uint32_t)(D + d)] = (uint8_t)s_d;
                if (s_r != s_r_old) st.qb[oq + (uint32_t)(2 * D)] = (uint8_t)s_r;
            }

            STAMP(10);
            const int32_t latest = pv * ((int)(rvm & 1u) - (int)((rvm >> 1) & 1u));
            const int32_t abs_d = latest < 0 ? -latest : latest;
            int32_t r = last_abs - abs_d;
            last_abs = abs_d;
            r = r > 10 ? 10 : (r < -10 ? -10 : r);
            if (FEEDBACK) {
                st_(obs, e << 2, (int32_t)(latest + cbound));
                st_(reward, e << 2, (float)r);
                st_(done, e, (uint8_t)dn);
                if (fb) st_(fb, e, (uint8_t)((uint32_t)(((latest > 0) - (latest < 0)) + 1) | ((uint32_t)(r + 10) << 2) | (dn << 7)));
            }
            now_out = t_end;

            st_(st.tw, o16, make_double2(t_end, wake));
            st_(st.tk, o16, make_uint4(tau, nbp, rvm, (uint32_t)last_abs | (dn << 31)));
        }
        STAMP(11);
        publish_env_counters(st.sa, N, e, k.pop, k.deliv, k_bad, fl, 1u);
    }
    STAMP(12);
}

template <int DT, int MODE>
__global__ __launch_bounds__(64) void ct_step_sfx_kernel(GW_LEAD_PARAMS_U64, uint64_t obs_a, uint64_t reward_a, uint64_t done_a, uint64_t fb_a)
{
    uint32_t* __restrict__ ip = gw_global_at<uint32_t>(ip_a);
    double* __restrict__ tw = gw_global_at<double>(tw_a);
    uint32_t* __restrict__ tk = gw_global_at<uint32_t>(tk_a);
    uint8_t* __restrict__ qb = gw_global_at<uint8_t>(qb_a);
    const int32_t* __restrict__ device = gw_global_at<const int32_t>(device_a);
    const int32_t* __restrict__ duration = gw_global_at<const int32_t>(duration_a);
    int32_t* __restrict__ obs = gw_global_at<int32_t>(obs_a);
    float* __restrict__ reward = gw_global_at<float>(reward_a);
    uint8_t* __restrict__ done = gw_global_at<uint8_t>(done_a);
    uint8_t* __restrict__ fb = gw_global_at<uint8_t>(fb_a);
    const int n_dev = (int)(dev_stage & 0xffu);
    const GwState st = hdr_state<DT>(ip, tw, tk, qb, n_envs, n_dev);
    const GwDevConst c = hdr_const<DT>(ip, n_dev);
    double now_new;
    bool live;
    ct_step_sfx_body<DT, true, MODE>(st, c, device, duration, obs, reward, done, fb, (int)(dev_stage >> 8), now_new, live);
}

typedef double v4f64 __attribute__((ext_vector_type(4)));

template <int MODE, bool HALF>
__global__ __launch_bounds__(64) void pend_step_kernel(GW_LEAD_PARAMS, GwPlantDev p,
                                                       int32_t* __restrict__ obs, float* __restrict__ reward,
                                                       double* __restrict__ angle_deg)
{
    const int n_dev = (int)(dev_stage & 0xffu);
    const GwState st = hdr_state<2>(ip, tw, tk, qb, n_envs, n_dev);
    const GwDevConst c = hdr_const<2>(ip, n_dev);
    constexpr int EPW = HALF ? 32 : 64;
    constexpr int NR = EPW / 16;
    __shared__ double s_x[EPW][5];
    const int lane = threadIdx.x;
    const int64_t e = (int64_t)blockIdx.x * EPW + (lane & (EPW - 1));
    const bool mine = e < p.N && lane < EPW;
    const int64_t el = e < p.N ? e : 0;
    const double2 x01 = *reinterpret_cast<const double2*>(p.x + el * 4);
    const double2 x23 = *reinterpret_cast<const double2*>(p.x + el * 4 + 2);
    const double u = p.u[el];
    const double tl = p.t_last[el];
    const unsigned long long nsub0 = p.nsub[el];
    __shared__ double s_pop[(GW_PLANT_KMAX / 4) * 64];
#pragma unroll
    for (int grp = 0; grp < GW_PLANT_KMAX / 4; ++grp) s_pop[grp * 64 + lane] = p.Pop[grp * 64 + lane];
    __shared__ double s_q[(GW_PLANT_KMAX + 1) * 4];
    for (int i = lane; i < (GW_PLANT_KMAX + 1) * 4; i += 64) s_q[i] = p.Qtab[i];

    double now_new;
    bool live;
    ct_step_sfx_body<2, false, MODE, HALF>(st, c, device, duration, nullptr, nullptr, nullptr, nullptr, (int)(dev_stage >> 8), now_new, live);
#ifdef GW_EXP_NO_EPILOGUE
    if (now_new >= 0.0) return;
#endif

    int n = 0;
    if (mine && live && now_new > tl) n = (int)llrint((now_new - tl) * p.inv_dt);
    STAMP(13);
    if (lane < EPW) { s_x[lane][0] = x01.x; s_x[lane][1] = x01.y; s_x[lane][2] = x23.x; s_x[lane][3] = x23.y; }
    __syncthreads();
    const int g = lane >> 4, col = lane & 15;
    double xg[NR], uq[NR];
    int nq[NR];
#pragma unroll
    for (int q = 0; q < NR; ++q) {
        const int src = 16 * q + col;
        xg[q] = s_x[src][g];
        uq[q] = __shfl(u, src);
        nq[q] = __shfl(n, src);
    }
    int nmax = n;
#pragma unroll
    for (int o = 32; o > 0; o >>= 1) { const int t = __shfl_xor(nmax, o); nmax = t > nmax ? t : nmax; }
    nmax = __builtin_amdgcn_readfirstlane(nmax);
    STAMP(14);
#ifdef GW_EXP_NO_MFMA
    nmax = 0;
#endif
    while (nmax > 0) {
        const int cmax = nmax > GW_PLANT_KMAX ? GW_PLANT_KMAX : nmax;
        int chunk[NR], mygrp[NR];
        v4f64 acc[NR];
#pragma unroll
        for (int q = 0; q < NR; ++q) {
            chunk[q] = nq[q] > GW_PLANT_KMAX ? GW_PLANT_KMAX : nq[q];
            mygrp[q] = (chunk[q] - 1) >> 2;
            acc[q] = v4f64{0.0, 0.0, 0.0, 0.0};
        }
        const int ngrp = (cmax + 3) >> 2;
#pragma unroll 1
        for (int grp = 0; grp < ngrp; ++grp) {
            const double a_p = s_pop[grp * 64 + lane];
#pragma unroll
            for (int q = 0; q < NR; ++q) {
                const double b = (mygrp[q] == grp) ? xg[q] : 0.0;
                acc[q] = __builtin_amdgcn_mfma_f64_16x16x4f64(a_p, b, acc[q], 0, 0, 0);
            }
        }
#pragma unroll
        for (int q = 0; q < NR; ++q) {
            const int r = (chunk[q] - 1) & 3;
            const double lo = (r & 1) ? acc[q].y : acc[q].x, hi = (r & 1) ? acc[q].w : acc[q].z;
            const double pick = (r & 2) ? hi : lo;
            xg[q] = chunk[q] > 0 ? fma(s_q[chunk[q] * 4 + g], uq[q], pick) : xg[q];
            nq[q] -= chunk[q];
        }
        nmax -= cmax;
    }
    STAMP(15);
#pragma unroll
    for (int q = 0; q < NR; ++q) s_x[16 * q + col][g] = xg[q];
    __syncthreads();
    if (mine) {
        const double a0 = s_x[lane][0], a1 = s_x[lane][1], a2 = s_x[lane][2], a3 = s_x[lane][3];
        if (n > 0) {
            gwk::gw_store_wt(reinterpret_cast<double2*>(p.x + e * 4), make_double2(a0, a1));
            gwk::gw_store_wt(reinterpret_cast<double2*>(p.x + e * 4 + 2), make_double2(a2, a3));
            gwk::gw_store_wt(p.t_last + e, now_new);
            gwk::gw_store_wt(p.nsub + e, nsub0 + (unsigned long long)n);
        }
        const double deg = a2 * (180.0 / 3.141592653589793);
        if (obs) gwk::gw_store_wt(obs + e, (int32_t)deg);
        if (reward) gwk::gw_store_wt(reward + e, (float)fabs(180.0 - deg));
        if (angle_deg) gwk::gw_store_wt(angle_deg + e, deg);
    }
}

__global__ void ct_init_sfx_kernel(GwState st)
{
    const uint32_t e = blockIdx.x * blockDim.x + threadIdx.x;
    if (e >= (uint32_t)st.N) return;
    const uint32_t o16 = e << 4;
    st_(st.tw, o16, make_double2(st.cst->start_time, st.cst->start_time));
    st_(st.tk, o16, make_uint4(0u, 1u, 0u, 0u));
    st_(st.ip, o16, make_uint4(0u, 1u, 0u, 0u));
    for (int b = 0; b < st.RB; ++b) st.qb[e * (uint32_t)st.RB + b] = 0;
    GwBp b0; b0.t0 = 0u; b0.c0 = 1u;
    st.bph[(size_t)e << 7] = b0;
    for (int w = 0; w < GW_SA_WORDS; ++w) st.sa[(size_t)w * st.N + e] = 0u;
    if (e == 0u) { st.sa[(size_t)4 * st.N] = 0u; st.sa[(size_t)4 * st.N + 1] = 0u; }
}

__global__ void ct_reset_sfx_kernel(uint32_t* __restrict__ ip, uint32_t n_envs, uint32_t n_dev, const uint8_t* __restrict__ mask,
                                    int32_t* __restrict__ obs)
{
    const uint32_t e = blockIdx.x * blockDim.x + threadIdx.x;
    if (e >= n_envs) return;
    const uint8_t* base = reinterpret_cast<const uint8_t*>(ip) - gw_blob_header((int)n_dev);
    const GW_AS_CONST GwState* hs = (const GW_AS_CONST GwState*)(base + gw_hdr_st_off((int)n_dev));
    uint32_t* tkp = gw_as_global(hs->tk);
    GwBp* bph = gw_as_global(hs->bph);
    const GW_AS_CONST GwDevConst* c = (const GW_AS_CONST GwDevConst*)(base + gw_hdr_cst_off((int)n_dev));
    const uint32_t o16 = e << 4;
    uint32_t rvm;
    if (!mask || mask[e]) {
        uint4 tk = ld<uint4>(tkp, o16);
        uint4 bp = ld<uint4>(ip, o16);
        GwBp cur; cur.t0 = bp.x; cur.c0 = 0u;
        if (bp.x == tk.x) {
            bph[((size_t)e << 7) + ((tk.y - 1u) & GW_RING_MASK)] = cur;
            bp.y = 0u;
        } else {
            bp.z = bp.x; bp.w = bp.y;
            cur.t0 = tk.x;
            bph[((size_t)e << 7) + (tk.y & GW_RING_MASK)] = cur;
            tk.y += 1u; bp.x = cur.t0; bp.y = 0u;
        }
        tk.z = 0u; tk.w = 0u;
        st_(tkp, o16, tk);
        st_(ip, o16, bp);
        rvm = 0u;
    } else {
        rvm = ld<uint4>(tkp, o16).z;
    }
    if (obs) obs[e] = c->payload_value * ((int)(rvm & 1u) - (int)((rvm >> 1) & 1u)) + c->counter_bound;
}

__global__ void ct_received_sfx_kernel(GwState st, int32_t* __restrict__ out)
{
    const int64_t idx = (int64_t)blockIdx.x * blockDim.x + threadIdx.x;
    const int D = st.D;
    if (idx >= st.N * D) return;
    const uint32_t e = (uint32_t)(idx / D);
    const int i = (int)(idx - (int64_t)e * D);
    const uint32_t rvm = ld<uint4>(st.tk, e << 4).z;
    out[idx] = ((rvm >> i) & 1u) ? st.cst->payload_value : 0;
}

__global__ void ct_delivered_sfx_kernel(GwState st, uint32_t* __restrict__ out)
{
    const uint32_t e = blockIdx.x * blockDim.x + threadIdx.x;
    if (e < (uint32_t)st.N) out[e] = st.sa[(size_t)2 * e + 1];
}

__global__ void ct_clear_flags_kernel(GwState st)
{
    const int64_t e = (int64_t)blockIdx.x * blockDim.x + threadIdx.x;
    if (e < st.N) {
        if (st.sa) st.sa[(size_t)3 * st.N + e] = 0u;
        if (st.xc) st.xc[(size_t)e * 4 + 3] = 0u;
    }
    if (st.totals && e < st.n_slots) st.totals[(size_t)e * GW_T_COUNT + GW_T_FLAGS] = 0ull;
}

struct StepArgs {
    uint64_t ip, tw, tk, qb, device, duration;
    uint32_t n_envs, dev_stage;
    uint64_t obs, reward, done, fb;
};
static_assert(sizeof(StepArgs) == 88, "StepArgs must mirror ct_step_sfx_kernel's parameter list");

template <class K>
void* function_of(K kernel)
{
    hipFunction_t f = nullptr;
    if (hipGetFuncBySymbol(&f, reinterpret_cast<const void*>(kernel)) != hipSuccess) { (void)hipGetLastError(); f = nullptr; }
    return f;
}

}

void gw_resolve_sfx_functions(int D, GwSfxFns* out)
{
    gw_with_dt<GW_DTS_STEP>(D, [&](auto dt) {
        constexpr int DT = decltype(dt)::value;
        out->step[0] = function_of(&ct_step_sfx_kernel<DT, 0>);
        out->step[1] = function_of(&ct_step_sfx_kernel<DT, 1>);
        out->step[2] = function_of(&ct_step_sfx_kernel<DT, 2>);
        out->step_slot = GW_LS_STEP_SFX + 3 * gw_ls_dt(DT);
    });
    out->reset = function_of(&ct_reset_sfx_kernel);
}

int gw_launch_step_sfx(const GwState& st, const GwDevConst& cst, const int32_t* device, const int32_t* duration,
                       int32_t* obs, float* reward, uint8_t* done, uint8_t* fb, void* stream, bool below_limits, uint64_t* rec,
                       const GwSfxFns* fns)
{
    const unsigned grid = (unsigned)((st.N + 63) / 64);
    const int mode = gw_step_mode(cst, below_limits, true);
    const uint32_t dev_stage = (uint32_t)st.D | ((uint32_t)st.stage_chunks << 8);
    if (fns && fns->step[mode]) {
        gw_note_launch(rec, fns->step_slot + mode);
        StepArgs a = {(uint64_t)st.ip, (uint64_t)st.tw, (uint64_t)st.tk, (uint64_t)st.qb, (uint64_t)device, (uint64_t)duration,
                      (uint32_t)st.N, dev_stage, (uint64_t)obs, (uint64_t)reward, (uint64_t)done, (uint64_t)fb};
        size_t size = sizeof a;
        void* extra[] = {HIP_LAUNCH_PARAM_BUFFER_POINTER, &a, HIP_LAUNCH_PARAM_BUFFER_SIZE, &size, HIP_LAUNCH_PARAM_END};
        return gw_launch_status(hipModuleLaunchKernel((hipFunction_t)fns->step[mode], grid, 1, 1, 64, 1, 1, 0, (hipStream_t)stream, nullptr, extra));
    }
    gw_with_dt<GW_DTS_STEP>(st.D, [&](auto dt) {
        gw_with_mode(mode, [&](auto m) {
            gw_note_launch(rec, GW_LS_STEP_SFX + 3 * gw_ls_dt(decltype(dt)::value) + decltype(m)::value);
            hipLaunchKernelGGL((ct_step_sfx_kernel<decltype(dt)::value, decltype(m)::value>), dim3(grid), dim3(64), 0, (hipStream_t)stream,
                               (uint64_t)st.ip, (uint64_t)st.tw, (uint64_t)st.tk, (uint64_t)st.qb, (uint64_t)device, (uint64_t)duration,
                               (uint32_t)st.N, dev_stage, (uint64_t)obs, (uint64_t)reward, (uint64_t)done, (uint64_t)fb);
        });
    });
    return gw_launch_status();
}

int gw_launch_init_sfx(const GwState& st, void* stream)
{
    const unsigned grid = (unsigned)((st.N + 255) / 256);
    hipLaunchKernelGGL(ct_init_sfx_kernel, dim3(grid), dim3(256), 0, (hipStream_t)stream, st);
    return gw_launch_status();
}

struct ResetArgs { uint32_t* ip; uint32_t n_envs, n_dev; const uint8_t* mask; int32_t* obs; };
static_assert(sizeof(ResetArgs) == 32, "ResetArgs must mirror ct_reset_sfx_kernel's parameter list");

int gw_launch_reset_sfx(const GwState& st, const uint8_t* mask, int32_t* obs, void* stream, const GwSfxFns* fns)
{
    const unsigned grid = (unsigned)((st.N + 255) / 256);
    if (fns && fns->reset) {
        ResetArgs a = {st.ip, (uint32_t)st.N, (uint32_t)st.D, mask, obs};
        size_t size = sizeof a;
        void* extra[] = {HIP_LAUNCH_PARAM_BUFFER_POINTER, &a, HIP_LAUNCH_PARAM_BUFFER_SIZE, &size, HIP_LAUNCH_PARAM_END};
        return gw_launch_status(hipModuleLaunchKernel((hipFunction_t)fns->reset, grid, 1, 1, 256, 1, 1, 0, (hipStream_t)stream, nullptr, extra));
    }
    hipLaunchKernelGGL(ct_reset_sfx_kernel, dim3(grid), dim3(256), 0, (hipStream_t)stream, st.ip, (uint32_t)st.N, (uint32_t)st.D, mask, obs);
    return gw_launch_status();
}

int gw_launch_delivered_sfx(const GwState& st, uint32_t* out, void* stream)
{
    hipLaunchKernelGGL(ct_delivered_sfx_kernel, dim3((unsigned)((st.N + 255) / 256)), dim3(256), 0, (hipStream_t)stream, st, out);
    return gw_launch_status();
}

int gw_launch_received_sfx(const GwState& st, int32_t* out, void* stream)
{
    const int64_t total = st.N * (int64_t)st.D;
    const unsigned grid = (unsigned)((total + 255) / 256);
    hipLaunchKernelGGL(ct_received_sfx_kernel, dim3(grid), dim3(256), 0, (hipStream_t)stream, st, out);
    return gw_launch_status();
}

int gw_launch_pend_step(const GwState& st, const GwDevConst& cst, const GwPlantDev& p, const int32_t* device, const int32_t* duration,
                        int32_t* obs, float* reward, double* angle_deg, void* stream, bool below_limits, uint64_t* rec)
{
    const bool half = st.N <= 32 * 1024;
    const unsigned grid = (unsigned)((st.N + (half ? 31 : 63)) / (half ? 32 : 64));
    gw_with_mode(gw_step_mode(cst, below_limits, true), [&](auto m) {
        gw_with_flag(half, [&](auto h) {
            gw_note_launch(rec, GW_LS_PEND + 2 * decltype(m)::value + (decltype(h)::value ? 1 : 0));
            hipLaunchKernelGGL((pend_step_kernel<decltype(m)::value, decltype(h)::value>), dim3(grid), dim3(64), 0, (hipStream_t)stream,
                               GW_LEAD_ARGS(st), p, obs, reward, angle_deg);
// ... 12 lines not shown
```

### gymwipe_amd/csrc/gw_api.cpp

```cpp
#include "gw_internal.h"
#include "gw_queue.h"
#include "gw_runq.h"
#include "gw_fastmath.h"

#include <hip/hip_runtime.h>

#include <math.h>
#include <stdarg.h>
#include <stdio.h>
#include <stdlib.h>
#include <string.h>
#include <new>
#include <vector>
#include <deque>
#include <atomic>
#include <string>

namespace {

thread_local char g_err[512] = "";

int fail(int code, const char* fmt, ...)
{
    va_list ap;
// ... 113 lines not shown
    if ((c.flags & (GW_CFG_NO_COUNTER_TRAFFIC | GW_CFG_PEER_RECEIVE | GW_CFG_FLOAT_DURATION)) && !(c.flags & GW_CFG_EXPLICIT_QUEUE))
        return fail(GW_EUNSUPPORTED, "GW_CFG_NO_COUNTER_TRAFFIC / PEER_RECEIVE / FLOAT_DURATION need GW_CFG_EXPLICIT_QUEUE");
    for (int a = 0; a <= c.num_devices; ++a)
        for (int b = 0; b <= c.num_devices; ++b)
            if (!(c.extra_att_db[a][b] == c.extra_att_db[b][a]) || (a == b && c.extra_att_db[a][b] != 0.0))
                return fail(GW_EINVAL, "extra_att_db must be symmetric with a zero diagonal (pair %d,%d)", a, b);
    if (!(c.start_time >= 0.0) || !(c.start_time < 1e12)) return fail(GW_EINVAL, "start_time out of range");
    if ((int64_t)c.max_duration * c.duration_factor > 100000000)
        return fail(GW_EINVAL, "max_duration*duration_factor too large");
    return GW_OK;
}

void set_fast_paths(const gw_config& cfg_ref, const GwHostTables& tab, GwDevConst& k)
{
    const gw_config* cfg = &cfg_ref;
    const int R = tab.R;
    k.inv_slot = 1.0 / cfg->slot;
    k.rcp_data_rate = 1.0 / tab.data_rate;
    k.fmod_limit = 0.0;
    const bool no_fast = getenv("GW_NO_FASTMATH") != nullptr;
    k.fast_fmod = (!no_fast && gw_fast_fmod_ok(cfg->slot, &k.fmod_limit)) ? 1 : 0;
    const int64_t max_bytes = (int64_t)cfg->mac_header_bytes + cfg->net_header_bytes + cfg->counter_bound + 64;
    k.fast_div = (!no_fast && gw_fast_div_ok(tab.data_rate, max_bytes)) ? 1 : 0;
    k.cls_limit = (no_fast || getenv("GW_NO_CLASSES")) ? 0.0 : 1.0e6;
    k.fast_decide = (!no_fast && cfg->max_ber == 0.25 && tab.coded_factor * 8.0 == floor(tab.coded_factor * 8.0)) ? 1 : 0;
    k.inv_interval = 1.0 / cfg->counter_interval;
    k.inv_slot_lo = gw_inv_lo(cfg->slot);
    k.inv_interval_lo = gw_inv_c_lo(cfg->counter_interval);
    {
        const double step_max = (double)cfg->max_duration * cfg->duration_factor * cfg->slot + 0.05;
        const double jmax = ceil(step_max / cfg->counter_interval) + 2.0;
        k.tie_filter = 8.0 * jmax * ldexp(1.0, 21 - 52) / (2.0 * cfg->counter_interval);
        if (!(k.tie_filter < 0.25)) k.tie_filter = 1.0;
    }
    k.fast_ticks = (!no_fast && !getenv("GW_NO_TICKJUMP") && gw_fast_ticks_ok(cfg->counter_interval)) ? 1 : 0;
    k.idem_states = 1;
    for (int to = 0; to < R && k.idem_states; ++to)
        for (int from = 0; from < R && k.idem_states; ++from) {
            if (to == from) continue;
            for (int s = 0; s < tab.nstates[to]; ++s) {
                const uint8_t s1 = tab.trans[((size_t)to * R + from) * GW_MAX_NSTATES + s];
                const uint8_t s2 = tab.trans[((size_t)to * R + from) * GW_MAX_NSTATES + s1];
                if (s1 != s2) { k.idem_states = 0; break; }
            }
        }
    if (tab.overflow) k.idem_states = 0;
    if (getenv("GW_NO_IDEM")) k.idem_states = 0;
}

int launch_step(gw_env* env, const int32_t* device, const int32_t* duration,
                int32_t* obs, float* reward, uint8_t* done, void* stream, uint8_t* fb, bool* fb_done)
{
    if (fb_done) *fb_done = false;
    if (env->dyn && env->st.tk) return gw_launch_step_dyn(env->st, env->cst_host, device, duration, obs, reward, done, stream, env->launches);
    if (env->st.tk) {
        if (fb_done) *fb_done = true;
        return gw_launch_step_sfx(env->st, env->cst_host, device, duration, obs, reward, done, fb, stream, gw_env_below_limits(env, stream),
                                  env->launches, &env->fns);
    }
    return gw_launch_step(env->st, device, duration, obs, reward, done, stream, env->no_split != 0, env->launches);
}

void expand_sfx(uint32_t bound, uint32_t base, uint32_t mult, uint32_t len, uint32_t tau,
                GwBp cur, GwBp prev, uint32_t nbp, const GwBp* hist, uint32_t* out )
{
    const uint64_t total = (uint64_t)mult * tau;
    for (uint32_t p = 0; p < len; ++p) {
        const uint64_t a = total - len + p;
        out[p] = base + gw_tick_value((uint32_t)(a / mult), cur, prev, nbp, hist, bound);
    }
}

}

int gw_fill_dev_const(const gw_config& cfg, const GwHostTables& tab, GwDevConst& k)
{
    const int D = cfg.num_devices, R = D + 1;
    k.D = D; k.R = R;
    k.counter_bound = cfg.counter_bound; k.payload_value = cfg.payload_value;
    k.mac_hdr = cfg.mac_header_bytes; k.net_hdr = cfg.net_header_bytes;
    k.duration_factor = cfg.duration_factor; k.max_duration = cfg.max_duration;
    for (int i = 0; i < D; ++i) { k.mult[i] = cfg.mult[i]; k.inv16[i] = cfg.mult[i] > 0 ? (65536u + (uint32_t)cfg.mult[i] - 1u) / (uint32_t)cfg.mult[i] : 0u; }
    for (int i = 0; i < D; ++i) k.inv20[i] = cfg.mult[i] > 0 ? ((1u << 20) + (uint32_t)cfg.mult[i] - 1u) / (uint32_t)cfg.mult[i] : 0u;
    k.ten_log_br = 10 * log10(cfg.bit_rate);
    k.twenty_log_f = 20 * log10(cfg.frequency);
    k.tx_power_dbm = cfg.tx_power_dbm;
    k.start_time = cfg.start_time;
    k.no_traffic = (cfg.flags & GW_CFG_NO_COUNTER_TRAFFIC) ? 1 : 0;
    k.peer_receive = (cfg.flags & GW_CFG_PEER_RECEIVE) ? 1 : 0;
    k.float_duration = (cfg.flags & GW_CFG_FLOAT_DURATION) ? 1 : 0;
    for (int i = 0; i < D; ++i) k.dest[i] = cfg.dest[i];
    k.slot = cfg.slot; k.data_rate = tab.data_rate; k.bit_rate = cfg.bit_rate;
    k.coded_factor = tab.coded_factor; k.max_ber = cfg.max_ber; k.counter_interval = cfg.counter_interval;
    {
        volatile double hb = (double)(cfg.mac_header_bytes * 8);
        k.hdr_dur = hb / tab.data_rate;
        k.hdr_bits = hb * tab.coded_factor;
    }

    set_fast_paths(cfg, tab, k);
    for (int j = 0; j < R; ++j) {
        uint16_t m = 0;
        for (int s0 = 0; s0 < tab.nstates[j]; ++s0) {
            bool fixed = true;
            for (int f = 0; f < R && fixed; ++f)
                if (f != j && tab.trans[((size_t)j * R + f) * GW_MAX_NSTATES + s0] != s0) fixed = false;
            if (fixed) m |= (uint16_t)(1u << s0);
        }
        k.term[j] = m;
    }
    return GW_OK;
}

int gw_validate_config(const gw_config& cfg) { return validate(cfg); }

struct GwEnvCounts { std::vector<uint64_t> steps, tx, deliv, app, pop, drop, bad; std::vector<uint32_t> flags; };
static int derive_env_counts(gw_env* env, GwEnvCounts& c)
{
    const GwState& st = env->st;
    const int64_t N = st.N;
    const int D = st.D, RB = st.RB;
    std::vector<uint32_t> sa((size_t)N * GW_SA_WORDS + 2), tk((size_t)N * 4);
    std::vector<uint8_t> qb((size_t)N * RB);
    HIP_TRY(hipMemcpy(sa.data(), st.sa, sa.size() * sizeof(uint32_t), hipMemcpyDeviceToHost));
    HIP_TRY(hipMemcpy(tk.data(), st.tk, tk.size() * sizeof(uint32_t), hipMemcpyDeviceToHost));
    HIP_TRY(hipMemcpy(qb.data(), st.qb, qb.size(), hipMemcpyDeviceToHost));
    uint64_t mult_sum = 0;
    for (int i = 0; i < D; ++i) mult_sum += (uint64_t)env->cfg.mult[i];
    const uint64_t n_steps = (uint64_t)sa[(size_t)4 * N] | ((uint64_t)sa[(size_t)4 * N + 1] << 32);
    c.steps.resize(N); c.tx.resize(N); c.deliv.resize(N); c.app.resize(N); c.pop.resize(N); c.drop.resize(N); c.bad.resize(N);
    c.flags.resize(N);
    for (int64_t e = 0; e < N; ++e) {
        uint64_t queued = 0;
        for (int i = 0; i < D; ++i) queued += qb[(size_t)e * RB + i];
        c.pop[e] = sa[(size_t)2 * e];
        c.deliv[e] = sa[(size_t)2 * e + 1];
        c.bad[e] = sa[(size_t)2 * N + e];
        c.flags[e] = sa[(size_t)3 * N + e];
        c.steps[e] = n_steps - c.bad[e];
        c.tx[e] = c.steps[e] + c.pop[e];
        c.app[e] = (uint64_t)tk[(size_t)e * 4] * mult_sum;
        c.drop[e] = c.app[e] - c.pop[e] - queued;
    }
    return GW_OK;
}

void gw_env_add_steps(gw_env* env, uint64_t n) { env->t_bound += (double)n * env->step_max; }
uint64_t* gw_env_launch_record(gw_env* env) { return env->launches; }

static std::atomic<uint64_t> g_launches[GW_LS_COUNT];
void gw_note_launch(uint64_t* rec, int slot)
{
    if (rec) ++rec[slot];
    g_launches[slot].fetch_add(1, std::memory_order_relaxed);
}
bool gw_env_below_limits(gw_env* env, void* stream)
{
    if (env->captured) return false;
    hipStreamCaptureStatus cs = hipStreamCaptureStatusNone;
    if (stream) {
        if (hipStreamIsCapturing((hipStream_t)stream, &cs) != hipSuccess) (void)hipGetLastError();
        else if (cs != hipStreamCaptureStatusNone) {
            env->captured = 1;
            return false;
        }
    }
    return env->t_bound + env->step_max < env->t_limit;
}

template <class F>
static int fused_chunks(gw_env* env, int32_t steps, void* stream, int32_t* s, F&& launch, int32_t longest)
{
    const int32_t cap = env->st.rcap < longest ? env->st.rcap : longest;
    while (env->st.tk && !env->dyn && cap > 0 && *s < steps) {
        const int32_t chunk = steps - *s < cap ? steps - *s : cap;
        const bool below = gw_env_below_limits(env, stream) && env->t_bound + (double)(chunk + 1) * env->step_max < env->t_limit;
        const int rc = launch(*s, GwChunk{chunk, stream, below, env->launches});
        if (rc == GW_EUNSUPPORTED) {
            if (getenv("GW_ROLLOUT_STRICT")) return fail(GW_EUNSUPPORTED, "no fused rollout for this handle (GW_ROLLOUT_STRICT is set)");
            break;
        }
        if (rc) return fail(GW_EHIP, "rollout kernel launch failed at step %d", *s);
        *s += chunk;
        gw_env_add_steps(env, (uint64_t)chunk);
    }
    return GW_OK;
}

int gw_env_internals(gw_env* env, const GwState** st, const GwDevConst** cst, int* hip_device)
{
    if (!env) return fail(GW_EINVAL, "env is NULL");
    if (env->dyn) return fail(GW_EUNSUPPORTED, "not available in the live-PHY mode (per-env geometry / open noise-state set)");
    *st = &env->st; *cst = &env->cst_host; *hip_device = env->cfg.hip_device;
    return GW_OK;
}

namespace {

struct EnvGuard {
    gw_env* env;
    ~EnvGuard() { if (env) gw_destroy(env); }
};

int create_host_side(gw_env* env)
{
    const gw_config& cfg = env->cfg;
    char msg[256] = "";
    int rc = gw_build_tables(cfg, env->tab, msg, sizeof msg);
    if (rc) return fail(rc, "%s", msg);
    if ((rc = select_device(env))) return rc;
    if (!(cfg.flags & GW_CFG_EXPLICIT_QUEUE)) gw_resolve_sfx_functions(cfg.num_devices, &env->fns);

    GwDevConst& k = env->cst_host;
    gw_fill_dev_const(cfg, env->tab, k);
    const double max_slots = (double)(cfg.max_duration - 1) * cfg.duration_factor;
    env->step_max = ((max_slots + 3.0) * cfg.slot + (double)(cfg.mac_header_bytes + 16) * 8.0 / env->tab.data_rate) * (1.0 + 1e-9) + 1e-9;
    env->t_bound = cfg.start_time;
    env->t_limit = (k.fast_fmod && k.cls_limit > 0.0) ? (k.fmod_limit < k.cls_limit ? k.fmod_limit : k.cls_limit) : 0.0;

    GwState& st = env->st;
    st.N = cfg.num_envs; st.D = cfg.num_devices; st.R = st.D + 1;
    const char* kb = getenv("GW_BLOCK");
    st.block = kb ? atoi(kb) : 64;
    if (st.block != 16 && st.block != 32 && st.block != 64 && st.block != 128 && st.block != 256) st.block = 64;
    env->no_split = getenv("GW_NO_SPLIT") ? 1 : 0;
    env->dyn = ((cfg.flags & GW_CFG_PER_ENV_GEOMETRY) || env->tab.overflow) ? 1 : 0;
    return GW_OK;
}

int create_alloc(gw_env* env)
{
    const gw_config& cfg = env->cfg;
    GwState& st = env->st;
    const int64_t N = st.N;
    const int D = st.D, R = st.R;
    const bool explicit_q = (cfg.flags & GW_CFG_EXPLICIT_QUEUE) != 0;
    const bool per_env_geo = (cfg.flags & GW_CFG_PER_ENV_GEOMETRY) != 0;
    int rc = GW_OK;
    auto alloc = [&](auto& ptr, size_t count) { if (!rc) rc = dev_alloc(env, &ptr, count); };
    if (explicit_q) {
        st.XB = 16 * ((R + 15) / 16);
        alloc(st.xw, N * 2);    alloc(st.xc, N * 4);    alloc(st.xs, N * st.XB);
        alloc(st.qrec, N * D);  alloc(st.runs, N * D * GW_RING_PHYS);
    } else {
        st.RB = 16 * ((2 * D + 1 + 15) / 16);
        alloc(st.tw, N * 2);   alloc(st.tk, N * 4);
        alloc(st.blob, (size_t)gw_blob_header(D) + (size_t)N * 16);
        if (!rc) st.ip = reinterpret_cast<uint32_t*>(const_cast<uint8_t*>(st.blob) + gw_blob_header(D));
        alloc(st.qb, N * st.RB);  alloc(st.bph, N * GW_RING_PHYS);
        alloc(st.sa, N * GW_SA_WORDS + 2);
        const char* rc_env = getenv("GW_ROLLOUT_CAP");
        int cap = rc_env ? atoi(rc_env) : 64;
        if (cap < 0) cap = 0;
        st.rcap = (cap + 15) / 16 * 16;
        if (st.rcap > 0 && getenv("GW_ROLLOUT_EVENT_LOOP")) { alloc(st.ract, N * st.rcap);  alloc(st.rfb, N * st.rcap); }
    }
    if (env->dyn) {
        const int RP = gw_rp(R);
        alloc(st.rxp, N * RP);  alloc(st.prx_tab, R * R);  alloc(st.pos_tab, R * 2);  alloc(st.extra_tab, R * R);
        if (!explicit_q) { alloc(st.bcache, N * 2 * D * 2);  alloc(st.rxr, N); }
        if (per_env_geo) { alloc(st.prx_env, N * R * RP);  alloc(st.pos_env, N * R * 2); }
        if (per_env_geo && explicit_q) alloc(st.talk, N);
    }
    if (explicit_q && (cfg.flags & GW_CFG_PEER_RECEIVE)) alloc(st.peer_rx, N * D);
    if (explicit_q && (cfg.flags & GW_CFG_PER_ENV_STATS)) alloc(st.pe_stats, N * 5);
    st.n_slots = (N + 15) / 16 + 1;
    if (explicit_q) alloc(st.totals, st.n_slots * GW_T_COUNT);
#ifdef GW_STAMPS
    alloc(st.stamps, st.n_slots * 16);
#endif
    const size_t tcount = (size_t)R * R * GW_MAX_NSTATES;
    alloc(st.cst, 1);  alloc(st.trans, tcount + 16);  alloc(st.ber, tcount);  alloc(st.cls, tcount);
    alloc(st.ber2, 2 * D * GW_MAX_NSTATES + 2);  alloc(st.cls2, 2 * D * GW_MAX_NSTATES + 16);
    if (explicit_q) alloc(st.blob, GwBlobLayout(D).total + 16);
    return rc;
}

int upload(const void* dev, const void* host, size_t bytes)
{
    HIP_TRY(hipMemcpy(const_cast<void*>(dev), host, bytes, hipMemcpyHostToDevice));
    return GW_OK;
}

int upload_header_structs(const gw_env* env)
{
    const int D = env->st.D;
    int rc = upload(env->st.blob + gw_hdr_cst_off(D), &env->cst_host, sizeof env->cst_host);
    return rc ? rc : upload(env->st.blob + gw_hdr_st_off(D), &env->st, sizeof env->st);
}

int create_upload(gw_env* env)
{
    GwState& st = env->st;
    const GwHostTables& tab = env->tab;
    const int64_t N = st.N;
    const int D = st.D, R = st.R;
    const size_t tcount = (size_t)R * R * GW_MAX_NSTATES;
    int rc;
    if ((rc = upload(st.cst, &env->cst_host, sizeof env->cst_host)) || (rc = upload(st.trans, tab.trans, tcount * sizeof(uint8_t))) ||
        (rc = upload(st.ber, tab.ber, tcount * sizeof(double))) || (rc = upload(st.cls, tab.cls, tcount * sizeof(uint8_t))))
        return rc;
    std::vector<double> ber2;
// ... 163 lines not shown
    c->code_rate = 0.75;
    c->max_ber = 0.25;
    c->tx_power_dbm = 0.0;
    c->counter_interval = 0.001;
    c->counter_bound = 65536;
    c->payload_value = 2;
    c->mac_header_bytes = 13;
    c->net_header_bytes = 12;
    c->duration_factor = 1000;
    c->max_duration = 20;
    return GW_OK;
}

int gw_create(const gw_config* cfg, gw_env** out)
{
    if (!cfg || !out) return fail(GW_EINVAL, "cfg/out is NULL");
    *out = nullptr;
    int rc = validate(*cfg);
    if (rc) return rc;

    int ndev = 0;
    if (hipGetDeviceCount(&ndev) != hipSuccess || ndev <= 0)
        return fail(GW_ENODEVICE, "no HIP device available (this library has no CPU fallback)");
    if (cfg->hip_device < 0 || cfg->hip_device >= ndev)
        return fail(GW_EINVAL, "hip_device %d out of range (have %d)", cfg->hip_device, ndev);

    EnvGuard guard = {new (std::nothrow) gw_env()};
    gw_env* env = guard.env;
    if (!env) return fail(GW_ENOMEM, "out of host memory");
    memset(env, 0, sizeof *env);
    env->cfg = *cfg;
    if ((rc = create_host_side(env)) || (rc = create_alloc(env)) || (rc = create_upload(env)) || (rc = create_init(env))) return rc;
    env->nblocks_create = env->nblocks;
    if ((rc = dev_alloc(env, &env->ep_mask, (size_t)cfg->num_envs))) return rc;
    guard.env = nullptr;
    *out = env;
    return GW_OK;
}

int gw_destroy(gw_env* env)
{
    if (!env) return GW_OK;
    (void)hipSetDevice(env->cfg.hip_device);
    for (int i = 0; i < env->nblocks; ++i) (void)hipFree(env->blocks[i]);
    delete env;
    return GW_OK;
}

int gw_reset(gw_env* env, const uint8_t* mask_dev, int32_t* obs_dev, void* stream)
{
    if (!env) return fail(GW_EINVAL, "env is NULL");
    int rc = select_device(env);
    if (rc) return rc;
    if (env->st.tk ? gw_launch_reset_sfx(env->st, mask_dev, obs_dev, stream, &env->fns)
                    : gw_launch_reset(env->st, mask_dev, obs_dev, stream))
        return fail(GW_EHIP, "reset kernel launch failed");
    return GW_OK;
}

int gw_step(gw_env* env, const int32_t* device_dev, const int32_t* duration_dev,
            int32_t* obs_dev, float* reward_dev, uint8_t* done_dev, void* stream)
{
    if (!env) return fail(GW_EINVAL, "env is NULL");
    if (!device_dev || !duration_dev || !obs_dev || !reward_dev || !done_dev)
        return fail(GW_EINVAL, "gw_step: NULL device pointer");
    int rc = select_device(env);
    if (rc) return rc;
    if (launch_step(env, device_dev, duration_dev, obs_dev, reward_dev, done_dev, stream))
        return fail(GW_EHIP, "step kernel launch failed: %s", hipGetErrorString(hipGetLastError()));
    gw_env_add_steps(env, 1);
    return GW_OK;
}

int gw_step_fb(gw_env* env, const int32_t* device_dev, const int32_t* duration_dev,
               int32_t* obs_dev, float* reward_dev, uint8_t* done_dev, uint8_t* feedback_byte_dev, void* stream)
{
    if (!feedback_byte_dev) return gw_step(env, device_dev, duration_dev, obs_dev, reward_dev, done_dev, stream);
    if (!env) return fail(GW_EINVAL, "env is NULL");
    if (!device_dev || !duration_dev || !obs_dev || !reward_dev || !done_dev)
        return fail(GW_EINVAL, "gw_step_fb: NULL device pointer");
    int rc = select_device(env);
    if (rc) return rc;
    bool fused = false;
    if (launch_step(env, device_dev, duration_dev, obs_dev, reward_dev, done_dev, stream, feedback_byte_dev, &fused))
        return fail(GW_EHIP, "step kernel launch failed: %s", hipGetErrorString(hipGetLastError()));
    gw_env_add_steps(env, 1);
    if (!fused)
        return gw_pack_feedback(env, env->st.N, obs_dev, reward_dev, done_dev, feedback_byte_dev, 0, stream);
    return GW_OK;
}

int gw_rollout(gw_env* env, int32_t steps, const int32_t* device_dev, const int32_t* duration_dev,
               int32_t* obs_dev, float* reward_dev, uint8_t* done_dev, void* stream)
{
    int rc = rollout_checks(env, steps, device_dev && duration_dev && obs_dev && reward_dev && done_dev, "gw_rollout");
    if (rc || (rc = select_device(env))) return rc;
    const int64_t N = env->st.N;
    const GwRows out = {nullptr, nullptr, obs_dev, reward_dev, done_dev, nullptr};
    return rollout_drive(env, steps, stream, true, INT32_MAX, nullptr,
        [&](int32_t s0, const GwChunk& ch) {
            return gw_launch_rollout_sfx(env->st, env->cst_host, ch, device_dev + s0 * N, duration_dev + s0 * N, out.at(s0 * N));
        },
        [&](int32_t s) { return plain_step(env, s, device_dev + s * N, duration_dev + s * N, out.at(s * N), stream); });
}

int gw_rollout_policy(gw_env* env, int32_t steps, const uint32_t* cdf_dev, uint64_t seed, uint64_t step0, uint64_t env_id0,
                      const int32_t* obs_prev_dev, int32_t* device_out_dev, int32_t* duration_out_dev,
// ... 453 lines not shown
    if (count > 0 && gw_launch_pack_feedback(count, env->cfg.counter_bound, env->cfg.payload_value, obs_dev, reward_dev, done_dev,
                                             packed_dev, env->pack_bad, stream))
        return fail(GW_EHIP, "pack kernel launch failed");
    if (check) {
        uint32_t bad = 0;
        HIP_TRY(hipStreamSynchronize((hipStream_t)stream));
        HIP_TRY(hipMemcpy(&bad, env->pack_bad, sizeof bad, hipMemcpyDeviceToHost));
        if (bad) return fail(GW_EINVAL, "%u element group(s) were not the built-in interpreter's feedback (not representable in one byte)", bad);
    }
    return GW_OK;
}

int gw_unpack_feedback(gw_env* env, int64_t count, const uint8_t* packed_dev, int32_t* obs_dev, float* reward_dev,
                       uint8_t* done_dev, void* stream)
{
    if (!env || count < 0) return fail(GW_EINVAL, "env is NULL or count negative");
    if (count == 0) return GW_OK;
    if (!obs_dev || !reward_dev || !done_dev || !packed_dev) return fail(GW_EINVAL, "a buffer is NULL");
    int rc = select_device(env);
    if (rc) return rc;
    if (gw_launch_unpack_feedback(count, env->cfg.counter_bound, env->cfg.payload_value, packed_dev, obs_dev, reward_dev, done_dev, stream))
        return fail(GW_EHIP, "unpack kernel launch failed");
    return GW_OK;
}

int gw_set_position(gw_env* env, int32_t radio, const double* x_dev, const double* y_dev, const uint8_t* mask_dev, void* stream)
{
    if (!env || !x_dev || !y_dev) return fail(GW_EINVAL, "env/x/y is NULL");
    if (!env->st.prx_env) return fail(GW_EUNSUPPORTED, "gw_set_position needs GW_CFG_PER_ENV_GEOMETRY");
    if (radio < 0 || radio > env->st.D) return fail(GW_EINVAL, "radio index out of range");
    int rc = select_device(env);
    if (rc) return rc;
    if (gw_launch_set_position(env->st, env->cst_host, radio, x_dev, y_dev, nullptr, mask_dev, stream))
        return fail(GW_EHIP, "set_position kernel launch failed");
    return GW_OK;
}

int gw_set_positions(gw_env* env, const double* pos_dev, const uint8_t* mask_dev, void* stream)
{
    if (!env || !pos_dev) return fail(GW_EINVAL, "env/pos is NULL");
    if (!env->st.prx_env) return fail(GW_EUNSUPPORTED, "gw_set_positions needs GW_CFG_PER_ENV_GEOMETRY");
    int rc = select_device(env);
    if (rc) return rc;
    if (gw_launch_set_position(env->st, env->cst_host, -1, nullptr, nullptr, pos_dev, mask_dev, stream))
        return fail(GW_EHIP, "set_position kernel launch failed");
    return GW_OK;
}

int gw_received(gw_env* env, int32_t* out_dev, void* stream)
{
    if (!env || !out_dev) return fail(GW_EINVAL, "env/out is NULL");
    int rc = select_device(env);
    if (rc) return rc;
    if (env->st.tk ? gw_launch_received_sfx(env->st, out_dev, stream) : gw_launch_received(env->st, out_dev, stream))
        return fail(GW_EHIP, "received kernel launch failed");
    return GW_OK;
}

int gw_clear_flags(gw_env* env, void* stream)
{
    if (!env) return fail(GW_EINVAL, "env is NULL");
    int rc = select_device(env);
    if (rc) return rc;
    if (gw_launch_clear_flags(env->st, stream)) return fail(GW_EHIP, "clear_flags kernel launch failed");
    return GW_OK;
}

int gw_stats_read(gw_env* env, gw_stats* out)
{
    if (!env || !out) return fail(GW_EINVAL, "env/out is NULL");
    int rc = select_device(env);
    if (rc) return rc;
    unsigned long long t[GW_T_COUNT] = {0};
    HIP_TRY(hipDeviceSynchronize());
    if (env->st.sa) {
        GwEnvCounts c;
        if ((rc = derive_env_counts(env, c))) return rc;
        memset(out, 0, sizeof *out);
        for (int64_t e = 0; e < env->st.N; ++e) {
            out->steps += c.steps[e]; out->transmissions += c.tx[e]; out->delivered += c.deliv[e]; out->appended += c.app[e];
            out->popped += c.pop[e]; out->dropped += c.drop[e]; out->bad_actions += c.bad[e]; out->flags_or |= c.flags[e];
        }
        return GW_OK;
    }
    std::vector<unsigned long long> slots((size_t)env->st.n_slots * GW_T_COUNT);
    HIP_TRY(hipMemcpy(slots.data(), env->st.totals, slots.size() * sizeof(unsigned long long), hipMemcpyDeviceToHost));
    for (int64_t w = 0; w < env->st.n_slots; ++w)
        for (int j = 0; j < GW_T_COUNT; ++j) {
            if (j == GW_T_FLAGS) t[j] |= slots[(size_t)w * GW_T_COUNT + j];
            else t[j] += slots[(size_t)w * GW_T_COUNT + j];
        }
    out->steps = t[GW_T_STEPS]; out->transmissions = t[GW_T_TX]; out->delivered = t[GW_T_DELIV];
    out->appended = t[GW_T_APP]; out->popped = t[GW_T_POP]; out->dropped = t[GW_T_DROP];
    out->flags_or = t[GW_T_FLAGS]; out->bad_actions = t[GW_T_BAD];
    return GW_OK;
}

int gw_now_ptr(gw_env* env, const void** now_dev, int64_t* stride_bytes)
{
    if (!env || !now_dev || !stride_bytes) return fail(GW_EINVAL, "env/now/stride is NULL");
    if (env->st.tw) { *now_dev = env->st.tw; *stride_bytes = 16; }
    else { *now_dev = env->st.xw; *stride_bytes = 16; }
    return GW_OK;
}

struct GwSnapHeader {
    uint32_t magic, abi;
    uint64_t total;
    gw_config cfg;
    int32_t nblocks, dyn;
    uint64_t block_bytes[32];
    double t_bound;
    int32_t captured, pad;
};
static const uint32_t kSnapMagic = 0x4e535747u;

int gw_snapshot_bytes(gw_env* env, uint64_t* bytes)
{
    if (!env || !bytes) return fail(GW_EINVAL, "env/bytes is NULL");
    uint64_t t = sizeof(GwSnapHeader);
    for (int i = 0; i < env->nblocks_create; ++i) t += env->block_bytes[i];
    *bytes = t;
    return GW_OK;
}

int gw_get_snapshot(gw_env* env, void* dst, uint64_t bytes)
{
    if (!env || !dst) return fail(GW_EINVAL, "env/dst is NULL");
    uint64_t need = 0;
    int rc = gw_snapshot_bytes(env, &need);
    if (rc) return rc;
    if (bytes != need) return fail(GW_EINVAL, "snapshot needs %llu bytes, got %llu", (unsigned long long)need, (unsigned long long)bytes);
    if ((rc = select_device(env))) return rc;
    HIP_TRY(hipDeviceSynchronize());
    GwSnapHeader h;
    memset(&h, 0, sizeof h);
    h.magic = kSnapMagic; h.abi = GW_ABI_VERSION; h.total = need; h.cfg = env->cfg; h.nblocks = env->nblocks_create; h.dyn = env->dyn;
    for (int i = 0; i < env->nblocks_create; ++i) h.block_bytes[i] = env->block_bytes[i];
    h.t_bound = env->t_bound;
    h.captured = env->captured;
    uint8_t* o = (uint8_t*)dst;
    memcpy(o, &h, sizeof h);
    o += sizeof h;
    for (int i = 0; i < env->nblocks_create; ++i) {
        HIP_TRY(hipMemcpy(o, env->blocks[i], env->block_bytes[i], hipMemcpyDeviceToHost));
        o += env->block_bytes[i];
    }
    return GW_OK;
}

int gw_set_state(gw_env* env, const void* src, uint64_t bytes)
{
    if (!env || !src) return fail(GW_EINVAL, "env/src is NULL");
    uint64_t need = 0;
    int rc = gw_snapshot_bytes(env, &need);
    if (rc) return rc;
    if (bytes != need) return fail(GW_EINVAL, "a snapshot of this handle has %llu bytes, got %llu", (unsigned long long)need, (unsigned long long)bytes);
    GwSnapHeader h;
    memcpy(&h, src, sizeof h);
    if (h.magic != kSnapMagic || h.abi != (uint32_t)GW_ABI_VERSION || h.total != bytes) return fail(GW_EINVAL, "not a snapshot of this ABI");
    gw_config a = h.cfg, b = env->cfg;
    a.hip_device = b.hip_device = 0;
    if (memcmp(&a, &b, sizeof a) != 0 || h.nblocks != env->nblocks_create || h.dyn != env->dyn)
        return fail(GW_EINVAL, "snapshot belongs to a handle with another configuration");
    for (int i = 0; i < h.nblocks; ++i)
        if (h.block_bytes[i] != env->block_bytes[i]) return fail(GW_EINVAL, "snapshot belongs to a handle with another layout");
    if ((rc = select_device(env))) return rc;
    HIP_TRY(hipDeviceSynchronize());
    const uint8_t* in = (const uint8_t*)src + sizeof h;
    for (int i = 0; i < h.nblocks; ++i) {
        HIP_TRY(hipMemcpy(env->blocks[i], in, env->block_bytes[i], hipMemcpyHostToDevice));
        in += env->block_bytes[i];
    }
    if (env->st.ip && (rc = upload_header_structs(env))) return rc;
    env->t_bound = h.t_bound > env->t_bound ? h.t_bound : env->t_bound;
    env->captured |= h.captured;
    HIP_TRY(hipDeviceSynchronize());
    return GW_OK;
}

int gw_state_bytes(gw_env* env, uint64_t* bytes)
{
    if (!env || !bytes) return fail(GW_EINVAL, "env/bytes is NULL");
    *bytes = env->bytes;
    return GW_OK;
}

int gw_link_info(gw_env* env, int32_t from, int32_t to, double* att, double* prx)
{
    if (!env) return fail(GW_EINVAL, "env is NULL");
    const int R = env->tab.R;
    if (from < 0 || from >= R || to < 0 || to >= R || from == to) return fail(GW_EINVAL, "radio index out of range");
    if (att) *att = env->tab.att[from][to];
    if (prx) *prx = env->tab.prx[from][to];
    return GW_OK;
}

int gw_noise_states(gw_env* env, int32_t radio, int32_t* count, double* values)
{
    if (!env || !count) return fail(GW_EINVAL, "env/count is NULL");
    if (radio < 0 || radio >= env->tab.R) return fail(GW_EINVAL, "radio index out of range");
    *count = env->tab.nstates[radio];
    if (values) for (int i = 0; i < GW_MAX_NSTATES; ++i) values[i] = i < *count ? env->tab.state_val[radio][i] : 0.0;
    return GW_OK;
}

static void launch_slot_name(int slot, char* out, size_t cap)
{
    static const int dts[GW_LS_NDT] = {GW_LS_DTS};
    static const char* const tf[2] = {"false", "true"};
    if (slot < GW_LS_PEND) {
        static const char* const fam[3] = {"ct_step_sfx_kernel", "ct_rollout_sync_kernel", "ct_rollout_sfx_kernel"};
        const int f = slot / (3 * GW_LS_NDT), i = slot % (3 * GW_LS_NDT);
// ... 10 lines not shown
    } else if (slot < GW_LS_ROLLOUT_PSTATS) {
        const int i = slot - GW_LS_ROLLOUT_POLICY;
        snprintf(out, cap, "ct_rollout_policy<%d, %d>", dts[i / 3], i % 3);
    } else {
        static const char* const fam[14] = {"ct_rollout_pstats", "ct_rollout_policy_ep", "ct_rollout_pstats_ep", "ct_rollout_sync_ep",
                                            "ct_rollout_pop_ep", "ct_rollout_policy_eps", "ct_rollout_pop_eps", "ct_rollout_sync_eps",
                                            "ct_rollout_backlog", "ct_rollout_backlog_pop", "ct_rollout_fsc", "ct_rollout_fsc_pop",
                                            "ct_rollout_pstats_d", "ct_rollout_pstats_epd"};
        static_assert(GW_LS_COUNT == GW_LS_ROLLOUT_PSTATS + 14 * 3 * GW_LS_NDT, "a family without a name");
        const int f = (slot - GW_LS_ROLLOUT_PSTATS) / (3 * GW_LS_NDT), i = (slot - GW_LS_ROLLOUT_PSTATS) % (3 * GW_LS_NDT);
        snprintf(out, cap, "%s<%d, %d>", fam[f], dts[i / 3], i % 3);
    }
}

int64_t gw_selftest_launches(gw_env* env, char* out, int64_t cap)
{
    if (cap < 0 || (cap > 0 && !out)) return fail(GW_EINVAL, "gw_selftest_launches: bad buffer");
    std::string text;
    for (int s = 0; s < GW_LS_COUNT; ++s) {
        const uint64_t n = env ? env->launches[s] : g_launches[s].load(std::memory_order_relaxed);
        if (!n) continue;
        char line[96];
        launch_slot_name(s, line, sizeof line);
        text += line;
        snprintf(line, sizeof line, " %llu\n", (unsigned long long)n);
        text += line;
    }
    if (cap > 0) {
        const size_t k = text.size() < (size_t)cap ? text.size() : (size_t)cap - 1;
        memcpy(out, text.data(), k);
        out[k] = 0;
    }
    return (int64_t)text.size();
}

int gw_selftest_fastmath(const gw_config* cfg, int32_t* max_noise_states)
{
    if (!cfg) return fail(GW_EINVAL, "cfg is NULL");
    int rc = validate(*cfg);
    if (rc) return rc;
    GwHostTables* tab = new GwHostTables();
    char msg[256] = "";
    rc = gw_build_tables(*cfg, *tab, msg, sizeof msg);
    if (rc) { delete tab; return fail(rc, "%s", msg); }
    GwDevConst k;
    memset(&k, 0, sizeof k);
    set_fast_paths(*cfg, *tab, k);
    int mx = 0;
    for (int r = 0; r < tab->R; ++r) mx = tab->nstates[r] > mx ? tab->nstates[r] : mx;
    if (tab->overflow) mx = GW_MAX_NSTATES + 1;
    if (max_noise_states) *max_noise_states = mx;
    delete tab;
    return (k.fast_fmod ? 1 : 0) | (k.fast_div ? 2 : 0) | (k.fast_decide ? 4 : 0) | (k.idem_states ? 8 : 0) | (k.fast_ticks ? 16 : 0);
}

int gw_selftest_queue(uint64_t seed, int32_t operations, int32_t mult, int32_t counter_bound)
{
    if (operations < 0 || mult < 1 || mult > GW_MAX_MULT || counter_bound < 1)
        return fail(GW_EINVAL, "gw_selftest_queue: bad arguments");
    uint64_t x = seed * 6364136223846793005ull + 1442695040888963407ull;
    auto rnd = [&x](uint32_t n) {
        x ^= x >> 12; x ^= x << 25; x ^= x >> 27;
        return (uint32_t)(((x * 2685821657736338717ull) >> 33) % n);
    };
    const uint32_t bound = (uint32_t)counter_bound, base = 25u;
    const uint32_t mults[2] = {(uint32_t)mult, mult > 1 ? 1u : 3u};
    uint32_t inv16[2];
    for (int i = 0; i < 2; ++i) inv16[i] = (65536u + mults[i] - 1u) / mults[i];
    std::vector<GwBp> hist(GW_RING_PHYS);
    GwBp cur = {0u, 1u}, prev = cur;
    hist[0] = cur;
    uint32_t nbp = 1, tau = 0, len[2] = {0, 0}, bad = 0, ctr = 1;
    std::deque<uint32_t> ref[2];
    GwTally tally = {0, 0, 0, 0, 0};
    uint64_t ref_drops = 0;
    for (int32_t op = 0; op < operations; ++op) {
        const uint32_t what = rnd(16);
        if (what < 9) {
            const uint32_t kk = 1 + rnd(what < 5 ? 3 : 22);
            for (uint32_t t = 0; t < kk; ++t) {
                for (int i = 0; i < 2; ++i)
                    for (uint32_t j = 0; j < mults[i]; ++j) {
                        if (ref[i].size() == GW_QUEUE_CAP) { ref[i].pop_front(); ++ref_drops; }
                        ref[i].push_back(base + ctr);
                    }
                if (ctr < bound) ++ctr;
            }
            tau += kk;
            for (int i = 0; i < 2; ++i) len[i] = gw_len_after_ticks(len[i], kk, mults[i], tally);
        } else if (what < 12) {
            ctr = 0;
            if (cur.t0 == tau) { cur.c0 = 0; hist[(nbp - 1) & GW_RING_MASK] = cur; }
            else { prev = cur; cur.t0 = tau; cur.c0 = 0; hist[nbp & GW_RING_MASK] = cur; ++nbp; }
        } else {
            const int i = (int)rnd(2);
            uint32_t n = 1 + rnd(what == 15 ? 40 : 4);
            while (n-- && !ref[i].empty()) {
                const uint32_t age = gw_ceil_div(len[i], mults[i], inv16[i]);
                const uint32_t hv = base + gw_tick_value(tau - age, cur, prev, nbp, hist.data(), bound);
                if (len[i] != ref[i].size() || hv != ref[i].front()) ++bad;
                ref[i].pop_front();
                len[i]--;
            }
        }
        if (gw_min_u32(cur.c0 + (tau - cur.t0), bound) != ctr) ++bad;
        for (int i = 0; i < 2; ++i) {
// ... 77 lines not shown
                    if (c < bound) ++c;
                }
                gw_runq_pop1_ticks(q, k, ctr, bound, base, ring.data(), m, inv20, tally);
                ctr = c;
            }
        }
        q = gw_runq_unpack(gw_runq_pack(q));
        uint32_t out[GW_QUEUE_CAP];
        const uint32_t n = gw_runq_expand(q, ring.data(), m, cap, out);
        bool same = n == ref.size() && q.len == ref.size();
        for (uint32_t p = 0; same && p < n; ++p) same = out[p] == ref[p];
        if (!same) ++bad;
    }
    if (tally.drop != ref_drops || tally.app != ref_apps) ++bad;
    return (int)bad;
}

static int read_geometry(const GwState& st, bool positions, void* dst, size_t bytes, const char* field)
{
    const int64_t N = st.N;
    const int R = st.R, RP = gw_rp(R);
    const int per = positions ? R * 2 : R * R;
    if (bytes != (size_t)N * per * sizeof(double))
        return fail(GW_EFIELD, "field %s needs %zu bytes, got %zu", field, (size_t)N * per * sizeof(double), bytes);
    double* o = (double*)dst;
    if (positions) { HIP_TRY(hipMemcpy(o, st.pos_env, bytes, hipMemcpyDeviceToHost)); return GW_OK; }
    std::vector<double> v((size_t)N * R * RP);
    HIP_TRY(hipMemcpy(v.data(), st.prx_env, v.size() * sizeof(double), hipMemcpyDeviceToHost));
    for (int64_t e = 0; e < N; ++e)
        for (int a = 0; a < R; ++a) for (int b = 0; b < R; ++b) o[(e * R + a) * R + b] = v[((size_t)e * R + a) * RP + b];
    return GW_OK;
}

int gw_get_state(gw_env* env, const char* field, void* dst, size_t bytes)
{
    if (!env || !field || !dst) return fail(GW_EINVAL, "env/field/dst is NULL");
    int rc = select_device(env);
    if (rc) return rc;
    HIP_TRY(hipDeviceSynchronize());
    const GwState& st = env->st;
    const int64_t N = st.N;
    const int D = st.D, R = st.R;

#define NEED(count, type) do { if (bytes != (size_t)(count) * sizeof(type)) \
        return fail(GW_EFIELD, "field %s needs %zu bytes, got %zu", field, (size_t)(count) * sizeof(type), bytes); } while (0)

#ifdef GW_STAMPS
    if (!strcmp(field, "stamps")) {
        NEED(st.n_slots * 16, uint64_t);
        HIP_TRY(hipMemcpy(dst, st.stamps, bytes, hipMemcpyDeviceToHost));
        return GW_OK;
    }
#endif
    if (st.tk) {
        {
            static const char* names[6] = {"n_tx", "n_delivered", "n_appended", "n_popped", "n_dropped", "flags"};
            for (int k = 0; k < 6; ++k)
                if (!strcmp(field, names[k])) {
                    GwEnvCounts c;
                    if ((rc = derive_env_counts(env, c))) return rc;
                    if (k == 5) { NEED(N, uint32_t); memcpy(dst, c.flags.data(), bytes); return GW_OK; }
                    NEED(N, uint64_t);
                    const std::vector<uint64_t>& v = k == 0 ? c.tx : (k == 1 ? c.deliv : (k == 2 ? c.app : (k == 3 ? c.pop : c.drop)));
                    memcpy(dst, v.data(), bytes);
                    return GW_OK;
                }
        }
        const int RB = st.RB;
        std::vector<double> tw((size_t)N * 2);
        std::vector<uint32_t> tk((size_t)N * 4), ip((size_t)N * 4);
        std::vector<uint8_t> qb((size_t)N * RB);
        HIP_TRY(hipMemcpy(tw.data(), st.tw, tw.size() * sizeof(double), hipMemcpyDeviceToHost));
        HIP_TRY(hipMemcpy(tk.data(), st.tk, tk.size() * sizeof(uint32_t), hipMemcpyDeviceToHost));
        HIP_TRY(hipMemcpy(ip.data(), st.ip, ip.size() * sizeof(uint32_t), hipMemcpyDeviceToHost));
        HIP_TRY(hipMemcpy(qb.data(), st.qb, qb.size(), hipMemcpyDeviceToHost));
        const uint32_t bound = (uint32_t)env->cfg.counter_bound;
        const int pv = env->cfg.payload_value;
        if (!strcmp(field, "now")) { NEED(N, double); double* o = (double*)dst; for (int64_t e = 0; e < N; ++e) o[e] = tw[e * 2]; return GW_OK; }
        if (!strcmp(field, "wake")) {
            NEED(N * D, double); double* o = (double*)dst;
            for (int64_t e = 0; e < N; ++e) for (int i = 0; i < D; ++i) o[e * D + i] = tw[e * 2 + 1];
            return GW_OK;
        }
        if (!strcmp(field, "counter")) {
            NEED(N * D, uint32_t); uint32_t* o = (uint32_t*)dst;
            for (int64_t e = 0; e < N; ++e) {
                const uint32_t v = gw_min_u32(ip[e * 4 + 1] + (tk[e * 4] - ip[e * 4]), bound);
                for (int i = 0; i < D; ++i) o[e * D + i] = v;
            }
            return GW_OK;
        }
        if (!strcmp(field, "last_abs")) { NEED(N, int32_t); int32_t* o = (int32_t*)dst; for (int64_t e = 0; e < N; ++e) o[e] = (int32_t)(tk[e * 4 + 3] & 0x7fffffffu); return GW_OK; }
        if (!strcmp(field, "latest_diff")) {
            NEED(N, int32_t); int32_t* o = (int32_t*)dst;
            for (int64_t e = 0; e < N; ++e) { const uint32_t m = tk[e * 4 + 2]; o[e] = pv * ((int)(m & 1u) - (int)((m >> 1) & 1u)); }
            return GW_OK;
        }
        if (!strcmp(field, "received")) {
            NEED(N * D, int32_t); int32_t* o = (int32_t*)dst;
            for (int64_t e = 0; e < N; ++e) for (int i = 0; i < D; ++i) o[e * D + i] = ((tk[e * 4 + 2] >> i) & 1u) ? pv : 0;
            return GW_OK;
        }
        if (!strcmp(field, "qlen")) {
            NEED(N * D, int32_t); int32_t* o = (int32_t*)dst;
            for (int64_t e = 0; e < N; ++e) for (int i = 0; i < D; ++i) o[e * D + i] = qb[(size_t)e * RB + i];
            return GW_OK;
        }
        if (!strcmp(field, "rx_power")) {
            NEED(N * R, double); double* o = (double*)dst;
            if (st.rxp) {
                const int RP = gw_rp(R);
                std::vector<double> rx((size_t)N * RP);
                HIP_TRY(hipMemcpy(rx.data(), st.rxp, rx.size() * sizeof(double), hipMemcpyDeviceToHost));
                for (int64_t e = 0; e < N; ++e) for (int r = 0; r < R; ++r) o[e * R + r] = rx[(size_t)e * RP + r];
                return GW_OK;
            }
            for (int64_t e = 0; e < N; ++e) for (int r = 0; r < R; ++r) o[e * R + r] = env->tab.state_val[r][qb[(size_t)e * RB + D + r]];
            return GW_OK;
        }
        if (!strcmp(field, "pos") || !strcmp(field, "link_power")) {
            if (!st.prx_env) return fail(GW_EFIELD, "field %s needs GW_CFG_PER_ENV_GEOMETRY", field);
            return read_geometry(st, field[0] == 'p', dst, bytes, field);
        }
        if (!strcmp(field, "queue")) {
            NEED(N * D * GW_QUEUE_CAP, uint32_t);
            std::vector<GwBp> hist((size_t)N * GW_RING_PHYS);
            HIP_TRY(hipMemcpy(hist.data(), st.bph, hist.size() * sizeof(GwBp), hipMemcpyDeviceToHost));
            uint32_t* o = (uint32_t*)dst;
// ... 110 lines not shown
```

### gymwipe_amd/csrc/gw_internal.h

```cpp
#pragma once
#include <stdint.h>
#include <stddef.h>
#include <vector>
#include "../../include/gymwipe_amd.h"

#define GW_RING_PHYS      128
#define GW_RING_MASK      (GW_RING_PHYS - 1)
#ifndef GW_MAX_NSTATES
#define GW_MAX_NSTATES    16
#endif

struct GwDevConst {
    int32_t D, R;
    int32_t counter_bound, payload_value, mac_hdr, net_hdr, duration_factor, max_duration;
    int32_t mult[GW_MAX_DEVICES];
    double  slot, data_rate, bit_rate, coded_factor, max_ber, counter_interval;
    double  hdr_dur;
    double  hdr_bits;
    uint32_t inv16[GW_MAX_DEVICES];
    uint16_t term[GW_MAX_RADIOS + 1];
    double  inv_slot;
    double  fmod_limit;
    double  rcp_data_rate;
    double  cls_limit;
    int32_t fast_fmod, fast_div, fast_decide, idem_states;
    double  start_time;
    int32_t fast_ticks;
    double  inv_interval;
    double  tie_filter;
    int32_t no_traffic, peer_receive, float_duration;
    int32_t dest[GW_MAX_DEVICES];
    double  ten_log_br, twenty_log_f, tx_power_dbm;
    uint32_t inv20[GW_MAX_DEVICES];
    double  inv_slot_lo, inv_interval_lo;
};

struct GwBp { uint32_t t0, c0; };
struct alignas(16) GwRec { uint32_t x, y, z, w; };

struct GwState {
    int64_t   N;
    int32_t   D, R;
    int32_t   stage_chunks;

    double*   xw;
    uint32_t* xc;
    uint8_t*  xs;
    int32_t   XB;
    GwRec*    qrec;
    uint64_t* runs;

    double*   tw;
    uint32_t* tk;
    uint32_t* ip;
    uint8_t*  qb;
    GwBp*     bph;
    int32_t   RB;
    uint16_t* ract;
    uint8_t*  rfb;
    int32_t   rcap;
    uint32_t* sa;

    uint32_t* peer_rx;
    int32_t   block;
    uint64_t* pe_stats;
    unsigned long long* totals;

    int64_t   n_slots;
    unsigned long long* stamps;
    const GwDevConst* cst;
    const uint8_t*    trans;
    const double*     ber;
    const uint8_t*    cls;
    const double*     ber2;
    const uint8_t*    cls2;
    const uint8_t*    blob;

    double*   rxp;
    const double* prx_tab;
    const double* pos_tab;
    const double* extra_tab;
    double*   prx_env;
    double*   pos_env;
    double*   bcache;
    double*   rxr;
    uint64_t* talk;
};
#if defined(__HIPCC__)
__host__ __device__
#endif
constexpr int gw_rp(int R)
{
    return R <= 2 ? 2 : (R <= 4 ? 4 : (R <= 8 ? 8 : (R <= 16 ? 16 : ((R + 15) & ~15))));
}

struct GwBlobLayout {
    int ber, mi, h1, r1, cls, lds_total, h2, total;
#if defined(__HIPCC__)
    __host__ __device__
#endif
    constexpr explicit GwBlobLayout(int D)
        : ber(0), mi(2 * D * GW_MAX_NSTATES * 8), h1(mi + (D * 8 + 15) / 16 * 16), r1(h1 + D * GW_MAX_NSTATES),
          cls(r1 + D * GW_MAX_NSTATES), lds_total(cls + 2 * D * GW_MAX_NSTATES), h2(lds_total),
          total(h2 + D * D * GW_MAX_NSTATES) {}
};

struct GwStripeLayout {
    int mi, s0, stripe, ber0, ber1, h1, r1, cls0, cls1, h2, total;
#if defined(__HIPCC__)
    __host__ __device__
#endif
    constexpr explicit GwStripeLayout(int D)
        : mi(0), s0((8 * D + 15) / 16 * 16), stripe((20 * D + 15) / 16 * 16), ber0(0), ber1(8 * D), h1(16 * D), r1(17 * D),
          cls0(18 * D), cls1(19 * D), h2(s0 + GW_MAX_NSTATES * stripe), total(h2 + D * D * GW_MAX_NSTATES) {}
#if defined(__HIPCC__)
    __host__ __device__
#endif
    constexpr int staged_chunks(int nstates) const { return (s0 + nstates * stripe + 15) / 16; }
};

#if defined(__HIPCC__)
#define GW_HDC __host__ __device__
#else
#define GW_HDC
#endif
GW_HDC constexpr int gw_hdr_cst_off(int D) { return (GwStripeLayout(D).total + 16 + 15) / 16 * 16; }
GW_HDC constexpr int gw_hdr_st_off(int D) { return gw_hdr_cst_off(D) + ((int)sizeof(GwDevConst) + 15) / 16 * 16; }
GW_HDC constexpr int gw_blob_header(int D) { return (gw_hdr_st_off(D) + (int)sizeof(GwState) + 255) / 256 * 256; }

enum { GW_CLS_COMPUTE = 0, GW_CLS_OK = 1, GW_CLS_HDR_FAIL = 2, GW_CLS_PAY_FAIL = 3 };

enum { GW_SA_WORDS = 4 };

enum { GW_T_STEPS = 0, GW_T_TX, GW_T_DELIV, GW_T_APP, GW_T_POP, GW_T_DROP, GW_T_FLAGS, GW_T_BAD, GW_T_COUNT };

struct GwPlantDev {
    int64_t N;
    double* x;
    double* u;
    double* t_last;
// ... 133 lines not shown
                                  const gw_episodes& ep, const gw_score& score, int32_t* obs_next, const GwRows& out, int32_t* seen_len,
                                  int32_t* delivered);
int gw_launch_backlog_select(const GwState& st, const GwDevConst& cst, const gw_backlog_policy& pol, const GwRows& row, int32_t* seen_len,
                             void* stream);
int gw_launch_rollout_backlog_pop_sfx(const GwState& st, const GwDevConst& cst, const GwChunk& ch, const gw_backlog_population& pop,
                                      const gw_episodes& ep, const gw_score& score, int32_t* obs_next);
int gw_launch_backlog_select_pop(const GwState& st, const GwDevConst& cst, const gw_backlog_population& pop, const GwRows& row, void* stream);
int gw_launch_rollout_pop_ep_sfx(const GwState& st, const GwDevConst& cst, const GwChunk& ch, const gw_population& pop,
                                 const GwPolicyStream& pol, const gw_episodes& ep, const gw_score* score, const int32_t* obs_prev,
                                 int32_t* obs_next);
int gw_launch_rollout_fsc_sfx(const GwState& st, const GwDevConst& cst, const GwChunk& ch, const gw_controller& ctl,
                              const GwPolicyStream& pol, const gw_episodes& ep, const gw_score& score, const int32_t* obs_prev,
                              int32_t* obs_next, const GwRows& out, int32_t* delivered, uint8_t* node_out);
int gw_launch_rollout_fsc_pop_sfx(const GwState& st, const GwDevConst& cst, const GwChunk& ch, const gw_controller_population& pop,
                                  const GwPolicyStream& pol, const gw_episodes& ep, const gw_score& score, const int32_t* obs_prev,
                                  int32_t* obs_next);
int gw_launch_transition_stats(int64_t N, int K, int D, int max_duration, int counter_bound, const int32_t* obs_prev,
                               const int32_t* device, const int32_t* duration, const int32_t* obs, const float* reward,
                               const uint8_t* done, const uint8_t* ended, int64_t* table, void* stream);
int gw_launch_rollout_pstats_d_sfx(const GwState& st, const GwDevConst& cst, const GwChunk& ch, const GwPolicyStream& pol,
                                   const int32_t* obs_prev, int32_t* obs_last, int32_t* ret, int64_t* table);
int gw_launch_rollout_pstats_epd_sfx(const GwState& st, const GwDevConst& cst, const GwChunk& ch, const GwPolicyStream& pol,
                                     const gw_episodes& ep, const int32_t* obs_prev, int32_t* obs_next, int64_t* table);
int gw_launch_transition_stats_d(int64_t N, int K, int D, int max_duration, int counter_bound, const int32_t* obs_prev,
                                 const int32_t* device, const int32_t* duration, const int32_t* obs, const float* reward,
                                 const uint8_t* done, const uint8_t* ended, const int32_t* delivered, int64_t* table, void* stream);
int gw_launch_policy_sample(const GwState& st, const GwDevConst& cst, const GwPolicyStream& pol, int64_t M, const int32_t* obs_in,
                            const GwRows& row, uint32_t* deliv_before, void* stream);
int gw_launch_episodes_step(const GwState& st, const GwDevConst& cst, const gw_episodes& ep, const gw_score* score, int64_t M,
                            int64_t* pop_tally, const uint32_t* deliv_before, int32_t* obs_next, const GwRows& row, uint8_t* mask,
                            int32_t* delivered_out, void* stream);
int gw_launch_received_sfx(const GwState& st, int32_t* out, void* stream);
int gw_launch_delivered_sfx(const GwState& st, uint32_t* out, void* stream);
int gw_launch_clear_flags(const GwState& st, void* stream);
int gw_launch_step_dyn(const GwState& st, const GwDevConst& cst, const int32_t* device, const int32_t* duration,
                       int32_t* obs, float* reward, uint8_t* done, void* stream, uint64_t* rec);
int gw_launch_init_dyn(const GwState& st, const GwDevConst& cst, double thermal, void* stream);
int gw_launch_set_position(const GwState& st, const GwDevConst& cst, int radio, const double* xs, const double* ys,
                           const double* all_pos, const uint8_t* mask, void* stream);

int gw_launch_pack_feedback(int64_t count, int center, int pv, const int32_t* obs, const float* reward, const uint8_t* done,
                            uint8_t* packed, uint32_t* bad, void* stream);
int gw_launch_unpack_feedback(int64_t count, int center, int pv, const uint8_t* packed, int32_t* obs, float* reward, uint8_t* done,
                              void* stream);

#define GW_MAX_MULT        100

#define GW_DTS_STEP          2, 3, 4, 5, 6, 7, 8, 16, 32
#define GW_DTS_ROLLOUT_SYNC  2, 3, 4, 5, 6, 7, 8, 16, 32
#define GW_DTS_ROLLOUT_LOOP  2, 3, 4, 6, 8, 16, 32
#define GW_DTS_LIVE          2, 3, 4, 6, 8, 16, 32
#define GW_DTS_GENERIC       2, 3, 4, 8, 16
#define GW_DTS_GENERIC_LIVE  4, 16

#define GW_LS_DTS GW_DTS_STEP, 0
enum {
    GW_LS_NDT = 10,
    GW_LS_STEP_SFX = 0,
    GW_LS_ROLLOUT_SYNC = GW_LS_STEP_SFX + 3 * GW_LS_NDT,
    GW_LS_ROLLOUT = GW_LS_ROLLOUT_SYNC + 3 * GW_LS_NDT,
    GW_LS_PEND = GW_LS_ROLLOUT + 3 * GW_LS_NDT,
    GW_LS_GENERIC = GW_LS_PEND + 6,
    GW_LS_LIVE = GW_LS_GENERIC + 8 * GW_LS_NDT,
    GW_LS_ROLLOUT_POLICY = GW_LS_LIVE + 2 * GW_LS_NDT,
    GW_LS_ROLLOUT_PSTATS = GW_LS_ROLLOUT_POLICY + 3 * GW_LS_NDT,
    GW_LS_ROLLOUT_POLICY_EP = GW_LS_ROLLOUT_PSTATS + 3 * GW_LS_NDT,
    GW_LS_ROLLOUT_PSTATS_EP = GW_LS_ROLLOUT_POLICY_EP + 3 * GW_LS_NDT,
    GW_LS_ROLLOUT_SYNC_EP = GW_LS_ROLLOUT_PSTATS_EP + 3 * GW_LS_NDT,
    GW_LS_ROLLOUT_POP_EP = GW_LS_ROLLOUT_SYNC_EP + 3 * GW_LS_NDT,
    GW_LS_ROLLOUT_POLICY_EPS = GW_LS_ROLLOUT_POP_EP + 3 * GW_LS_NDT,
    GW_LS_ROLLOUT_POP_EPS = GW_LS_ROLLOUT_POLICY_EPS + 3 * GW_LS_NDT,
    GW_LS_ROLLOUT_SYNC_EPS = GW_LS_ROLLOUT_POP_EPS + 3 * GW_LS_NDT,
    GW_LS_ROLLOUT_BACKLOG = GW_LS_ROLLOUT_SYNC_EPS + 3 * GW_LS_NDT,
    GW_LS_ROLLOUT_BACKLOG_POP = GW_LS_ROLLOUT_BACKLOG + 3 * GW_LS_NDT,
    GW_LS_ROLLOUT_FSC = GW_LS_ROLLOUT_BACKLOG_POP + 3 * GW_LS_NDT,
    GW_LS_ROLLOUT_FSC_POP = GW_LS_ROLLOUT_FSC + 3 * GW_LS_NDT,
    GW_LS_ROLLOUT_PSTATS_D = GW_LS_ROLLOUT_FSC_POP + 3 * GW_LS_NDT,
    GW_LS_ROLLOUT_PSTATS_EPD = GW_LS_ROLLOUT_PSTATS_D + 3 * GW_LS_NDT,
    GW_LS_COUNT = GW_LS_ROLLOUT_PSTATS_EPD + 3 * GW_LS_NDT
};
constexpr int gw_ls_dt(int DT)
{
    constexpr int dts[GW_LS_NDT] = {GW_LS_DTS};
    int i = 0;
    while (i < GW_LS_NDT - 1 && dts[i] != DT) ++i;
    return i;
}
void gw_note_launch(uint64_t* rec, int slot);
```

### gymwipe_amd/csrc/gw_plant_api.cpp

```cpp
#include "gw_internal.h"

#include <hip/hip_runtime.h>

#include <math.h>
#include <stdio.h>
#include <string.h>
#include <new>
#include <vector>


int gw_plant_launch_update(const GwPlantDev& p, const void* now_base, int64_t stride, int32_t* obs, float* reward, double* angle_deg,
                           void* stream);
int gw_plant_launch_set_input(const GwPlantDev& p, const double* u, const uint8_t* mask, void* stream);
int gw_plant_launch_init(const GwPlantDev& p, const double* x0, double u0, void* stream);
int gw_plant_launch_feedback(const GwPlantDev& p, int32_t* obs, float* reward, double* angle_deg, void* stream);

int gw_set_error(int code, const char* fmt, ...);
int gw_env_internals(gw_env* env, const GwState** st, const GwDevConst** cst, int* hip_device);
void gw_env_add_steps(gw_env* env, uint64_t n);
int gw_launch_pend_step(const GwState& st, const GwDevConst& cst, const GwPlantDev& p, const int32_t* device, const int32_t* duration,
                        int32_t* obs, float* reward, double* angle_deg, void* stream, bool below_limits,
                        uint64_t* rec);
bool gw_env_below_limits(gw_env* env, void* stream);
uint64_t* gw_env_launch_record(gw_env* env);
// ... 94 lines not shown
    const int64_t N = cfg->num_envs;
    double *dP = nullptr, *dQ = nullptr;
    int rc;
#define PA(ptr, cnt) do { rc = palloc(p, &(ptr), (size_t)(cnt)); if (rc) { gw_plant_destroy(p); return rc; } } while (0)
    PA(p->dev.x, N * 4); PA(p->dev.u, N); PA(p->dev.t_last, N); PA(p->dev.nsub, N);
    PA(dP, pop.size()); PA(dQ, qop.size());
#undef PA
    p->dev.N = N; p->dev.Pop = dP; p->dev.Qtab = dQ; p->dev.dt = cfg->dt; p->dev.inv_dt = 1.0 / cfg->dt;
    PLANT_HIP(hipMemcpy(dP, pop.data(), pop.size() * sizeof(double), hipMemcpyHostToDevice), gw_plant_destroy(p));
    PLANT_HIP(hipMemcpy(dQ, qop.data(), qop.size() * sizeof(double), hipMemcpyHostToDevice), gw_plant_destroy(p));
    if (gw_plant_launch_init(p->dev, cfg->x0, cfg->u0, nullptr)) { gw_plant_destroy(p); return gw_set_error(GW_EHIP, "plant init launch failed"); }
    PLANT_HIP(hipDeviceSynchronize(), gw_plant_destroy(p));
    *out = p;
    return GW_OK;
}

int gw_plant_destroy(gw_plant* p)
{
    if (!p) return GW_OK;
    (void)hipSetDevice(p->cfg.hip_device);
    for (int i = 0; i < p->nblocks; ++i) (void)hipFree(p->blocks[i]);
    delete p;
    return GW_OK;
}

int gw_plant_update(gw_plant* p, const void* now_dev, int64_t stride_bytes, void* stream)
{
    if (!p || !now_dev) return gw_set_error(GW_EINVAL, "plant/now is NULL");
    if (stride_bytes < 8 || (stride_bytes & 7)) return gw_set_error(GW_EINVAL, "stride_bytes must be a multiple of 8");
    PLANT_HIP(hipSetDevice(p->cfg.hip_device), (void)0);
    if (gw_plant_launch_update(p->dev, now_dev, stride_bytes, nullptr, nullptr, nullptr, stream)) return gw_set_error(GW_EHIP, "plant update launch failed");
    return GW_OK;
}

int gw_plant_update_feedback(gw_plant* p, const void* now_dev, int64_t stride_bytes, int32_t* obs_dev, float* reward_dev,
                             double* angle_deg_dev, void* stream)
{
    if (!p || !now_dev) return gw_set_error(GW_EINVAL, "plant/now is NULL");
    if (stride_bytes < 8 || (stride_bytes & 7)) return gw_set_error(GW_EINVAL, "stride_bytes must be a multiple of 8");
    PLANT_HIP(hipSetDevice(p->cfg.hip_device), (void)0);
    if (gw_plant_launch_update(p->dev, now_dev, stride_bytes, obs_dev, reward_dev, angle_deg_dev, stream))
        return gw_set_error(GW_EHIP, "plant update launch failed");
    return GW_OK;
}

int gw_pendulum_step(gw_env* env, gw_plant* p, const int32_t* device_dev, const int32_t* duration_dev, int32_t* obs_dev,
                     float* reward_dev, double* angle_deg_dev, void* stream)
{
    if (!env || !p) return gw_set_error(GW_EINVAL, "env/plant is NULL");
    if (!device_dev || !duration_dev) return gw_set_error(GW_EINVAL, "gw_pendulum_step: NULL action pointer");
    const GwState* st = nullptr; const GwDevConst* cst = nullptr; int dev = 0;
    int rc = gw_env_internals(env, &st, &cst, &dev);
    if (rc) return rc;
    if (!st->tk) return gw_set_error(GW_EUNSUPPORTED, "gw_pendulum_step needs the default (suffix) queue mode");
    if (st->D != 2) return gw_set_error(GW_EUNSUPPORTED, "gw_pendulum_step: the env's network has two assignable devices (sensor, controller)");
    if (st->N != p->dev.N || dev != p->cfg.hip_device) return gw_set_error(GW_EINVAL, "env and plant differ in num_envs or hip_device");
    PLANT_HIP(hipSetDevice(dev), (void)0);
    if (gw_launch_pend_step(*st, *cst, p->dev, device_dev, duration_dev, obs_dev, reward_dev, angle_deg_dev, stream, gw_env_below_limits(env, stream),
                            gw_env_launch_record(env)))
        return gw_set_error(GW_EHIP, "pendulum step launch failed");
    gw_env_add_steps(env, 1);
    return GW_OK;
}

int gw_plant_set_input(gw_plant* p, const double* u_dev, const uint8_t* mask_dev, void* stream)
{
    if (!p || !u_dev) return gw_set_error(GW_EINVAL, "plant/u is NULL");
    PLANT_HIP(hipSetDevice(p->cfg.hip_device), (void)0);
    if (gw_plant_launch_set_input(p->dev, u_dev, mask_dev, stream)) return gw_set_error(GW_EHIP, "plant set_input launch failed");
    return GW_OK;
}

int gw_plant_feedback(gw_plant* p, int32_t* obs_dev, float* reward_dev, double* angle_deg_dev, void* stream)
{
    if (!p) return gw_set_error(GW_EINVAL, "plant is NULL");
    PLANT_HIP(hipSetDevice(p->cfg.hip_device), (void)0);
    if (gw_plant_launch_feedback(p->dev, obs_dev, reward_dev, angle_deg_dev, stream)) return gw_set_error(GW_EHIP, "plant feedback launch failed");
    return GW_OK;
}

int gw_plant_state_ptr(gw_plant* p, double** x_dev)
{
    if (!p || !x_dev) return gw_set_error(GW_EINVAL, "plant/x is NULL");
    *x_dev = p->dev.x;
    return GW_OK;
}

int gw_plant_get_state(gw_plant* p, const char* field, void* dst, size_t bytes)
{
    if (!p || !field || !dst) return gw_set_error(GW_EINVAL, "plant/field/dst is NULL");
    PLANT_HIP(hipSetDevice(p->cfg.hip_device), (void)0);
    PLANT_HIP(hipDeviceSynchronize(), (void)0);
    const int64_t N = p->dev.N;
    const void* src = nullptr; size_t need = 0;
    if (!strcmp(field, "x")) { src = p->dev.x; need = (size_t)N * 4 * sizeof(double); }
    else if (!strcmp(field, "u")) { src = p->dev.u; need = (size_t)N * sizeof(double); }
    else if (!strcmp(field, "t_last")) { src = p->dev.t_last; need = (size_t)N * sizeof(double); }
    else if (!strcmp(field, "substeps")) { src = p->dev.nsub; need = (size_t)N * sizeof(uint64_t); }
    else return gw_set_error(GW_EFIELD, "unknown plant field %s", field);
    if (bytes != need) return gw_set_error(GW_EFIELD, "field %s needs %zu bytes, got %zu", field, need, bytes);
    PLANT_HIP(hipMemcpy(dst, src, need, hipMemcpyDeviceToHost), (void)0);
    return GW_OK;
}

}
```

### include/gymwipe_amd.h

```cpp
#ifndef GYMWIPE_AMD_H
#define GYMWIPE_AMD_H

#include <stddef.h>
#include <stdint.h>

#ifdef __cplusplus
extern "C" {
#endif

#define GW_ABI_VERSION   1

#define GW_MAX_DEVICES   32
#define GW_MAX_RADIOS    (GW_MAX_DEVICES + 1)
#define GW_QUEUE_CAP     100

#define GW_OK             0
#define GW_EINVAL        -1
#define GW_ENODEVICE     -2
#define GW_EHIP          -3
#define GW_ENOMEM        -4
#define GW_EUNSUPPORTED  -5
#define GW_EFIELD        -6

#define GW_FLAG_CARRY    1u
// ... 269 lines not shown
    double  send_interval;
    int32_t header_bytes;
    int32_t payload_bytes;
    double  move_interval;
    double  move_span;
    uint64_t seed;
} gw_grid_config;

typedef struct gw_grid gw_grid;

int gw_grid_config_default(gw_grid_config* cfg, int64_t num_envs, int32_t num_devices);
int gw_grid_create(const gw_grid_config* cfg, const double* initial_delays_host, gw_grid** out);
int gw_grid_destroy(gw_grid* g);
int gw_grid_run(gw_grid* g, double seconds, void* stream);
int gw_grid_set_position(gw_grid* g, int32_t device, const double* x_host, const double* y_host, void* stream);
int gw_grid_get_state(gw_grid* g, const char* field, void* dst_host, size_t bytes);

typedef struct gw_ctrl_config {
    gw_config net;
    double  A[16], B[4];
    double  x0[4], u0;
    int32_t ctrl_start_tick;
    int32_t ctrl_period_ticks;
} gw_ctrl_config;

typedef struct gw_ctrl gw_ctrl;

int gw_ctrl_config_default(gw_ctrl_config* cfg, int64_t num_envs);
int gw_ctrl_create(const gw_ctrl_config* cfg, gw_ctrl** out);
int gw_ctrl_destroy(gw_ctrl* c);
int gw_ctrl_step(gw_ctrl* c, const int32_t* device_dev, const int32_t* duration_dev, int32_t* obs_dev, float* reward_dev,
                 double* angle_deg_dev, void* stream);
int gw_ctrl_get_state(gw_ctrl* c, const char* field, void* dst_host, size_t bytes);

int gw_ctrl_set_initial(gw_ctrl* c, const double* x0_dev, const double* u0_dev, const uint8_t* mask_dev, void* stream);
int gw_ctrl_reset(gw_ctrl* c, const uint8_t* mask_dev, int32_t* obs_dev, void* stream);

typedef struct gw_ctrl_episodes {
    int32_t max_steps;
    int32_t pad;
    double  fail_deg;
} gw_ctrl_episodes;

int gw_ctrl_rollout(gw_ctrl* c, int32_t steps, const int32_t* device_dev, const int32_t* duration_dev, const gw_ctrl_episodes* ep,
                    int32_t* obs_dev, float* reward_dev, double* angle_deg_dev, uint8_t* ended_dev, void* stream);

int gw_ctrl_rollout_schedules(gw_ctrl* c, int32_t steps, const uint8_t* sched_dev, int32_t P, int32_t L, const gw_ctrl_episodes* ep,
                              double* tally_dev, void* stream);

int gw_selftest_queue(uint64_t seed, int32_t operations, int32_t mult, int32_t counter_bound);

int gw_selftest_runq(uint64_t seed, int32_t operations, int32_t mult, int32_t counter_bound);

int gw_selftest_fastmath(const gw_config* cfg, int32_t* max_noise_states);

int64_t gw_selftest_launches(gw_env* env, char* out, int64_t cap);

#ifdef __cplusplus
}
#endif
#endif
```

Measured before the change: 17.50 billion.

## Pack per-env tick and queue-length state into one 16-byte record for small sender counts

For 2–4 sender devices, the separate tick word (tk) and queue-byte row (qb) are merged into a single 16-byte tq record. Queue lengths, noise states, the receive mask, the last-abs flag and the done bit are bit-packed into 64 bits, with tau and nbp in the remaining words. This replaces two per-env global loads and stores with one each in the step and rollout kernels, cutting memory traffic. The cost is extra bit packing and unpacking, plus last_abs reduced to a flag that is rebuilt from the payload value.

```diff
diff --git a/gymwipe_amd/_native.py b/gymwipe_amd/_native.py
--- a/gymwipe_amd/_native.py
+++ b/gymwipe_amd/_native.py
@@ -25,7 +25,7 @@
     "gw_abi_version", "gw_last_error", "gw_device_count", "gw_config_default", "gw_create",
     "gw_destroy", "gw_reset", "gw_step", "gw_step_fb", "gw_rollout", "gw_rollout_policy", "gw_rollout_policy_stats", "gw_transition_stats", "gw_rollout_episodes", "gw_rollout_episodes_stats", "gw_transition_stats_ep", "gw_rollout_autoreset", "gw_rollout_population", "gw_rollout_episodes_scored", "gw_rollout_population_scored", "gw_rollout_autoreset_scored", "gw_rollout_backlog", "gw_rollout_backlog_population", "gw_rollout_controller", "gw_rollout_controller_population", "gw_rollout_policy_stats_delivered", "gw_rollout_episodes_stats_delivered", "gw_transition_stats_delivered", "gw_set_position", "gw_set_positions", "gw_received", "gw_delivered", "gw_enqueue", "gw_pack_feedback", "gw_unpack_feedback", "gw_get_state",
     "gw_stats_read", "gw_clear_flags", "gw_state_bytes", "gw_snapshot_bytes", "gw_get_snapshot", "gw_set_state", "gw_link_info", "gw_noise_states", "gw_selftest_queue", "gw_selftest_runq",
-    "gw_selftest_fastmath", "gw_selftest_launches",
+    "gw_selftest_fastmath", "gw_selftest_launches", "gw_selftest_tq",
     "gw_plant_config_default", "gw_plant_create", "gw_plant_destroy", "gw_plant_update", "gw_plant_set_input",
     "gw_plant_state_ptr", "gw_plant_get_state", "gw_plant_feedback", "gw_plant_update_feedback", "gw_now_ptr", "gw_pendulum_step",
     "gw_ctrl_config_default", "gw_ctrl_create", "gw_ctrl_destroy", "gw_ctrl_step", "gw_ctrl_get_state",
@@ -284,6 +284,7 @@
     L.gw_selftest_fastmath.argtypes = [C.POINTER(Config), C.POINTER(i32)]
     L.gw_selftest_fastmath.restype = C.c_int
     L.gw_selftest_launches.argtypes, L.gw_selftest_launches.restype = [vp, C.c_char_p, i64], i64
+    L.gw_selftest_tq.argtypes, L.gw_selftest_tq.restype = [i32], C.c_int
     L.gw_plant_config_default.argtypes, L.gw_plant_config_default.restype = [C.POINTER(PlantConfig), i64], C.c_int
     L.gw_plant_create.argtypes, L.gw_plant_create.restype = [C.POINTER(PlantConfig), C.POINTER(vp)], C.c_int
     L.gw_plant_destroy.argtypes, L.gw_plant_destroy.restype = [vp], C.c_int
diff --git a/gymwipe_amd/csrc/ct_common.hip.h b/gymwipe_amd/csrc/ct_common.hip.h
--- a/gymwipe_amd/csrc/ct_common.hip.h
+++ b/gymwipe_amd/csrc/ct_common.hip.h
@@ -146,6 +146,70 @@
     return i == 0 ? w.x : (i == 1 ? w.y : (i == 2 ? w.z : w.w));
 }
 
+template <int DT, class Off>
+__device__ __forceinline__ uint4 gw_ld_tk(const GwState& st, Off o16, uint64_t& f)
+{
+    if constexpr (gw_tq_dt(DT)) {
+        const uint4 r = ld<uint4>(st.tq, o16);
+        f = (uint64_t)r.x | ((uint64_t)r.y << 32);
+        return make_uint4(r.z, r.w, gw_tq_rvm(f), gw_tq_la(f) | (gw_tq_done(f) << 31));
+    } else {
+        f = 0ull;
+        return ld<uint4>(st.tk, o16);
+    }
+}
+template <int DT, bool QW, int NWC, class Off>
+__device__ __forceinline__ void gw_ld_qw(const GwState& st, Off oq, uint64_t f, uint4 (&qw)[NWC])
+{
+    if constexpr (gw_tq_dt(DT)) {
+        static_assert(NWC == 1 && QW, "the packed record's bytes are one 16-byte word");
+        uint32_t w[3] = {0u, 0u, 0u};
+#pragma unroll
+        for (int i = 0; i < DT; ++i) w[i >> 2] |= gw_tq_len(f, (uint32_t)i) << ((i & 3) * 8);
+#pragma unroll
+        for (int j = 0; j <= DT; ++j) w[(DT + j) >> 2] |= gw_tq_state(f, (uint32_t)j) << (((DT + j) & 3) * 8);
+        qw[0] = make_uint4(w[0], w[1], w[2], 0u);
+    } else {
+#pragma unroll
+        for (int w = 0; w < NWC; ++w) qw[w] = QW ? ld<uint4>(st.qb, oq + 16u * w) : make_uint4(0u, 0u, 0u, 0u);
+    }
+}
+template <int DT>
+__device__ __forceinline__ int32_t gw_tkq_last_abs(uint32_t tk_w, int32_t pv)
+{
+    if constexpr (gw_tq_dt(DT)) return gw_tq_last_abs(tk_w & 1u, pv);
+    else return (int32_t)(tk_w & 0x7fffffffu);
+}
+template <int DT, bool WT, class Off>
+__device__ __forceinline__ void gw_st_qw(const GwState& st, Off o16, Off oq, int w, const uint4& o, uint32_t tau, uint32_t nbp,
+                                         uint32_t rvm, int32_t last_abs, uint32_t dn)
+{
+    if constexpr (gw_tq_dt(DT)) {
+        const uint32_t b[3] = {o.x, o.y, o.z};
+        uint64_t f = 0ull;
+#pragma unroll
+        for (int i = 0; i < DT; ++i) f |= (uint64_t)((b[i >> 2] >> ((i & 3) * 8)) & 0x7fu) << (GW_TQ_LEN_AT + GW_TQ_LEN_BITS * i);
+#pragma unroll
+        for (int j = 0; j <= DT; ++j)
+            f |= (uint64_t)((b[(DT + j) >> 2] >> (((DT + j) & 3) * 8)) & 0xfu) << (GW_TQ_STATE_AT + GW_TQ_STATE_BITS * j);
+        f |= (uint64_t)(rvm & ((1u << GW_TQ_MAX_D) - 1u)) << GW_TQ_RVM_AT;
+        f |= (uint64_t)(last_abs != 0 ? 1u : 0u) << GW_TQ_LA_AT;
+        f |= (uint64_t)(dn & 1u) << GW_TQ_DONE_AT;
+        const uint4 r = make_uint4((uint32_t)f, (uint32_t)(f >> 32), tau, nbp);
+        if (WT) st_(st.tq, o16, r); else st_plain(st.tq, o16, r);
+    } else {
+        if (WT) st_(st.qb, oq + 16u * w, o); else st_plain(st.qb, oq + 16u * w, o);
+    }
+}
+template <int DT, bool WT, class Off>
+__device__ __forceinline__ void gw_st_tk(const GwState& st, Off o16, uint32_t tau, uint32_t nbp, uint32_t rvm, int32_t last_abs, uint32_t dn)
+{
+    if constexpr (!gw_tq_dt(DT)) {
+        if (WT) st_(st.tk, o16, make_uint4(tau, nbp, rvm, (uint32_t)last_abs | (dn << 31)));
+        else st_plain(st.tk, o16, make_uint4(tau, nbp, rvm, (uint32_t)last_abs | (dn << 31)));
+    }
+}
+
 __device__ __forceinline__ void publish_env_counters(uint32_t* sa, uint32_t N, uint32_t e, uint32_t pop, uint32_t deliv,
                                                      uint32_t bad, uint32_t fl, uint32_t steps)
 {
@@ -188,7 +252,7 @@
                        const int32_t* __restrict__ device, const int32_t* __restrict__ duration, uint32_t n_envs, uint32_t dev_stage
 #define GW_LEAD_PARAMS_U64 uint64_t ip_a, uint64_t tw_a, uint64_t tk_a, uint64_t qb_a, uint64_t device_a, uint64_t duration_a, \
                            uint32_t n_envs, uint32_t dev_stage
-#define GW_LEAD_ARGS(st_) (st_).ip, (st_).tw, (st_).tk, (st_).qb, device, duration, (uint32_t)(st_).N, \
+#define GW_LEAD_ARGS(st_) (st_).ip, (st_).tw, gw_tk_or_tq(st_), (st_).qb, device, duration, (uint32_t)(st_).N, \
                           ((uint32_t)(st_).D | ((uint32_t)(st_).stage_chunks << 8))
 #if defined(__HIP_DEVICE_COMPILE__)
 #define GW_AS_CONST __attribute__((address_space(4)))
@@ -212,13 +276,15 @@
 {
     return (T*)(__attribute__((address_space(1))) T*)address;
 }
-template <int DT>
+template <int DT, bool TQ = false>
 __device__ __forceinline__ GwState hdr_state(uint32_t* ip, double* tw, uint32_t* tk, uint8_t* qb, uint32_t n_envs, int n_dev)
 {
     const int D = DT > 0 ? DT : n_dev;
     const uint8_t* base = reinterpret_cast<const uint8_t*>(ip) - gw_blob_header(D);
     GwState st = *(const GW_AS_CONST GwState*)(base + gw_hdr_st_off(D));
-    st.ip = ip; st.tw = tw; st.tk = tk; st.qb = qb; st.N = (int64_t)n_envs; st.D = D;
+    st.ip = ip; st.tw = tw; st.N = (int64_t)n_envs; st.D = D;
+    if constexpr (TQ) { static_assert(gw_tq_dt(DT), "no packed record at this sender count"); st.tq = tk; st.tk = nullptr; st.qb = nullptr; }
+    else { st.tk = tk; st.qb = qb; }
     st.blob = base;
 #define GW_G(m) st.m = gw_as_global(st.m)
     GW_G(bph); GW_G(sa); GW_G(trans); GW_G(ber); GW_G(cls); GW_G(ber2); GW_G(cls2); GW_G(rxp); GW_G(prx_tab); GW_G(pos_tab);
diff --git a/gymwipe_amd/csrc/ct_rollout_backlog.hip b/gymwipe_amd/csrc/ct_rollout_backlog.hip
--- a/gymwipe_amd/csrc/ct_rollout_backlog.hip
+++ b/gymwipe_amd/csrc/ct_rollout_backlog.hip
@@ -146,13 +146,15 @@
 }
 
 template <bool CLAMP>
-__device__ __forceinline__ void gw_backlog_select(const uint8_t* row, uint32_t D, uint32_t md, const gw_backlog_policy& pol, uint32_t& d_out,
+__device__ __forceinline__ void gw_backlog_select(const uint8_t* row, bool tq, uint32_t D, uint32_t md, const gw_backlog_policy& pol, uint32_t& d_out,
                                                   uint32_t& du_out, uint32_t& q_out)
 {
     auto weight = [&](uint32_t i) { return CLAMP ? gw_backlog_weight(pol.w_len[i]) : (uint32_t)pol.w_len[i]; };
-    uint32_t q = row[0], p = weight(0) * q, d = 0;
+    const uint64_t f = tq ? *reinterpret_cast<const uint64_t*>(row) : 0ull;
+    auto len_of = [&](uint32_t i) { return tq ? gw_tq_len(f, i) : (uint32_t)row[i]; };
+    uint32_t q = len_of(0), p = weight(0) * q, d = 0;
     for (uint32_t i = 1; i < D; ++i) {
-        const uint32_t qi = row[i], pi = weight(i) * qi;
+        const uint32_t qi = len_of(i), pi = weight(i) * qi;
         const bool more = pi > p;
         p = more ? pi : p; q = more ? qi : q; d = more ? i : d;
     }
@@ -160,19 +162,19 @@
     du_out = gw_min_u32((uint32_t)pol.duration_of_len[gw_min_u32(q, (uint32_t)GW_QUEUE_CAP)], md - 1u);
     q_out = q;
 }
-__global__ __launch_bounds__(256) void backlog_select_rows(uint32_t N, uint32_t D, uint32_t RB, uint32_t md, gw_backlog_policy pol,
+__global__ __launch_bounds__(256) void backlog_select_rows(uint32_t N, uint32_t D, uint32_t RB, uint32_t tq, uint32_t md, gw_backlog_policy pol,
                                                            const uint8_t* __restrict__ qb, int32_t* __restrict__ device_out,
                                                            int32_t* __restrict__ duration_out, int32_t* __restrict__ seen_len)
 {
     const uint32_t e = blockIdx.x * blockDim.x + threadIdx.x;
     if (e >= N) return;
     uint32_t d, du, q;
-    gw_backlog_select<false>(qb + (size_t)e * RB, D, md, pol, d, du, q);
+    gw_backlog_select<false>(qb + (size_t)e * RB, tq != 0u, D, md, pol, d, du, q);
     device_out[e] = (int32_t)d;
     duration_out[e] = (int32_t)du;
     seen_len[e] = (int32_t)q;
 }
-__global__ __launch_bounds__(256) void backlog_select_pop_rows(uint32_t N, uint32_t D, uint32_t RB, uint32_t md, uint32_t M,
+__global__ __launch_bounds__(256) void backlog_select_pop_rows(uint32_t N, uint32_t D, uint32_t RB, uint32_t tq, uint32_t md, uint32_t M,
                                                                const gw_backlog_policy* __restrict__ policies,
                                                                const uint8_t* __restrict__ qb, int32_t* __restrict__ device_out,
                                                                int32_t* __restrict__ duration_out)
@@ -180,7 +182,7 @@
     const uint32_t e = blockIdx.x * blockDim.x + threadIdx.x;
     if (e >= N) return;
     uint32_t d, du, q;
-    gw_backlog_select<true>(qb + (size_t)e * RB, D, md, policies[e / M], d, du, q);
+    gw_backlog_select<true>(qb + (size_t)e * RB, tq != 0u, D, md, policies[e / M], d, du, q);
     device_out[e] = (int32_t)d;
     duration_out[e] = (int32_t)du;
 }
@@ -199,8 +201,8 @@
                              void* stream)
 {
     hipLaunchKernelGGL(backlog_select_rows, dim3((unsigned)((st.N + 255) / 256)), dim3(256), 0, (hipStream_t)stream, (uint32_t)st.N,
-                       (uint32_t)st.D, (uint32_t)st.RB, (uint32_t)cst.max_duration, pol, (const uint8_t*)st.qb, row.device, row.duration,
-                       seen_len);
+                       (uint32_t)st.D, st.qb ? (uint32_t)st.RB : 16u, st.qb ? 0u : 1u, (uint32_t)cst.max_duration, pol,
+                       st.qb ? (const uint8_t*)st.qb : (const uint8_t*)st.tq, row.device, row.duration, seen_len);
     return gw_launch_status();
 }
 
@@ -214,7 +216,8 @@
 int gw_launch_backlog_select_pop(const GwState& st, const GwDevConst& cst, const gw_backlog_population& pop, const GwRows& row, void* stream)
 {
     hipLaunchKernelGGL(backlog_select_pop_rows, dim3((unsigned)((st.N + 255) / 256)), dim3(256), 0, (hipStream_t)stream, (uint32_t)st.N,
-                       (uint32_t)st.D, (uint32_t)st.RB, (uint32_t)cst.max_duration, (uint32_t)pop.envs_per_policy, pop.policies_dev,
-                       (const uint8_t*)st.qb, row.device, row.duration);
+                       (uint32_t)st.D, st.qb ? (uint32_t)st.RB : 16u, st.qb ? 0u : 1u, (uint32_t)cst.max_duration,
+                       (uint32_t)pop.envs_per_policy, pop.policies_dev, st.qb ? (const uint8_t*)st.qb : (const uint8_t*)st.tq, row.device,
+                       row.duration);
     return gw_launch_status();
 }
diff --git a/gymwipe_amd/csrc/ct_rollout_sfx.hip b/gymwipe_amd/csrc/ct_rollout_sfx.hip
--- a/gymwipe_amd/csrc/ct_rollout_sfx.hip
+++ b/gymwipe_amd/csrc/ct_rollout_sfx.hip
@@ -142,7 +142,8 @@
     const uint32_t o16 = e << 4, oq = e * RB;
     const uint4 ip = ld<uint4>(st.ip, o16);
     const double2 tw = ld<double2>(st.tw, o16);
-    const uint4 tk = ld<uint4>(st.tk, o16);
+    uint64_t tqf;
+    const uint4 tk = gw_ld_tk<DT>(st, o16, tqf);
     typename ArrSel<GEN, DM>::rw len, tb;
     typename ArrSel<GEN, DM + 1>::rw sta;
     if constexpr (GEN) {
@@ -152,8 +153,7 @@
         for (int j = 0; j < R; ++j) sta[j] = st.qb[oq + (uint32_t)(D + j)];
     } else {
         uint4 qw[NWC];
-#pragma unroll
-        for (int w = 0; w < NWC; ++w) qw[w] = ld<uint4>(st.qb, oq + 16u * w);
+        gw_ld_qw<DT, true>(st, oq, tqf, qw);
 #pragma unroll
         for (int i = 0; i < DT; ++i) len[i] = (word_of(qw[i >> 4], (i >> 2) & 3) >> ((i & 3) * 8)) & 0xffu;
 #pragma unroll
@@ -167,7 +167,7 @@
     bpp.t0 = ip.z; bpp.c0 = ip.w;
     const GwBp* hist = st.bph + ((size_t)e << 7);
     uint32_t rvm = tk.z;
-    int32_t last_abs = (int32_t)(tk.w & 0x7fffffffu);
+    int32_t last_abs = gw_tkq_last_abs<DT>(tk.w, c.payload_value);
     uint32_t dn = tk.w >> 31;
 
     constexpr bool FAST = MODE >= 1, NOLIM = MODE == 2;
@@ -421,11 +421,11 @@
             o.y = nb[b + 4] | (nb[b + 5] << 8) | (nb[b + 6] << 16) | (nb[b + 7] << 24);
             o.z = nb[b + 8] | (nb[b + 9] << 8) | (nb[b + 10] << 16) | (nb[b + 11] << 24);
             o.w = nb[b + 12] | (nb[b + 13] << 8) | (nb[b + 14] << 16) | (nb[b + 15] << 24);
-            st_plain(st.qb, oq + 16u * w, o);
+            gw_st_qw<DT, false>(st, o16, oq, w, o, tau, nbp, rvm, last_abs, dn);
         }
     }
     st_plain(st.tw, o16, make_double2(now, wake));
-    st_plain(st.tk, o16, make_uint4(tau, nbp, rvm, (uint32_t)last_abs | (dn << 31)));
+    gw_st_tk<DT, false>(st, o16, tau, nbp, rvm, last_abs, dn);
     publish_env_counters(st.sa, N, e, kt.pop, kt.deliv, k_bad, fl, (uint32_t)K);
 }
 
diff --git a/gymwipe_amd/csrc/ct_rollout_sync_body.h b/gymwipe_amd/csrc/ct_rollout_sync_body.h
--- a/gymwipe_amd/csrc/ct_rollout_sync_body.h
+++ b/gymwipe_amd/csrc/ct_rollout_sync_body.h
@@ -33,7 +33,8 @@
     const uint32_t o16 = e << 4, oq = e * RB;
     const uint4 ip = ld<uint4>(st.ip, o16);
     const double2 tw = ld<double2>(st.tw, o16);
-    const uint4 tk = ld<uint4>(st.tk, o16);
+    uint64_t tqf;
+    const uint4 tk = gw_ld_tk<DT>(st, o16, tqf);
     typename ArrSel<GEN, DM>::rw len, tb;
     typename ArrSel<GEN, DM + 1>::rw sta;
     if constexpr (GEN) {
@@ -43,8 +44,7 @@
         for (int j = 0; j < R; ++j) sta[j] = st.qb[oq + (uint32_t)(D + j)];
     } else {
         uint4 qw[NWC];
-#pragma unroll
-        for (int w = 0; w < NWC; ++w) qw[w] = ld<uint4>(st.qb, oq + 16u * w);
+        gw_ld_qw<DT, true>(st, oq, tqf, qw);
 #pragma unroll
         for (int i = 0; i < DT; ++i) len[i] = (word_of(qw[i >> 4], (i >> 2) & 3) >> ((i & 3) * 8)) & 0xffu;
 #pragma unroll
@@ -58,7 +58,7 @@
     bpp.t0 = ip.z; bpp.c0 = ip.w;
     const GwBp* hist = st.bph + ((size_t)e << 7);
     uint32_t rvm = tk.z;
-    int32_t last_abs = (int32_t)(tk.w & 0x7fffffffu);
+    int32_t last_abs = gw_tkq_last_abs<DT>(tk.w, c.payload_value);
     uint32_t dn = tk.w >> 31;
 
     constexpr bool FAST = MODE >= 1, NOLIM = MODE == 2;
@@ -354,11 +354,11 @@
             o.y = nb[b + 4] | (nb[b + 5] << 8) | (nb[b + 6] << 16) | (nb[b + 7] << 24);
             o.z = nb[b + 8] | (nb[b + 9] << 8) | (nb[b + 10] << 16) | (nb[b + 11] << 24);
             o.w = nb[b + 12] | (nb[b + 13] << 8) | (nb[b + 14] << 16) | (nb[b + 15] << 24);
-            st_plain(st.qb, oq + 16u * w, o);
+            gw_st_qw<DT, false>(st, o16, oq, w, o, tau, nbp, rvm, last_abs, dn);
         }
     }
     st_plain(st.tw, o16, make_double2(now, wake));
-    st_plain(st.tk, o16, make_uint4(tau, nbp, rvm, (uint32_t)last_abs | (dn << 31)));
+    gw_st_tk<DT, false>(st, o16, tau, nbp, rvm, last_abs, dn);
     publish_env_counters(st.sa, N, e, kt.pop, kt.deliv, k_bad, fl, (uint32_t)K);
 #undef GW_ROLLOUT_SRC_RESETS
 #undef GW_ROLLOUT_SRC_QUEUES
diff --git a/gymwipe_amd/csrc/ct_step_sfx.hip b/gymwipe_amd/csrc/ct_step_sfx.hip
--- a/gymwipe_amd/csrc/ct_step_sfx.hip
+++ b/gymwipe_amd/csrc/ct_step_sfx.hip
@@ -24,6 +24,7 @@
                                                  double& now_out, bool& live_out)
 {
     constexpr bool PACKED = DT > 0;
+    constexpr bool TQ = gw_tq_dt(DT);
     constexpr bool FAST = MODE >= 1, NOLIM = MODE == 2;
     constexpr int NWC = DT > 0 ? (2 * DT + 1 + 15) / 16 : 1;
     const uint32_t N = (uint32_t)st.N;
@@ -65,10 +66,10 @@
     int du = duration[el];
     uint4 ip = ld<uint4>(st.ip, o16l);
     const double2 tw = ld<double2>(st.tw, o16l);
-    const uint4 tk = ld<uint4>(st.tk, o16l);
+    uint64_t tqf;
+    const uint4 tk = gw_ld_tk<DT>(st, o16l, tqf);
     uint4 qw[NWC];
-#pragma unroll
-    for (int w = 0; w < NWC; ++w) qw[w] = PACKED ? ld<uint4>(st.qb, oql + 16u * w) : make_uint4(0u, 0u, 0u, 0u);
+    gw_ld_qw<DT, PACKED>(st, oql, tqf, qw);
     now_out = tw.x;
     live_out = live;
     if (one_pass) {
@@ -117,7 +118,7 @@
         asm volatile("" : "+v"(rvm));
 #endif
         STAMP(3);
-        int32_t last_abs = (int32_t)(tk.w & 0x7fffffffu);
+        int32_t last_abs = gw_tkq_last_abs<DT>(tk.w, pv);
         uint32_t dn = tk.w >> 31;
         uint32_t fl = 0;
 
@@ -137,7 +138,12 @@
             const bool idem = FAST || idem_i != 0;
 
             uint32_t len_d, s_d_old, s_r_old;
-            if (PACKED) {
+            if constexpr (TQ) {
+                asm volatile("" : "+v"(tqf));
+                len_d = gw_tq_len(tqf, (uint32_t)d);
+                s_d_old = gw_tq_state(tqf, (uint32_t)d);
+                s_r_old = gw_tq_state(tqf, (uint32_t)DT);
+            } else if (PACKED) {
                 if (NWC == 1) {
                     uint32_t q0 = qw[0].x, q1 = qw[0].y, q2 = qw[0].z, q3 = qw[0].w;
                     asm volatile("" : "+v"(q0), "+v"(q1), "+v"(q2), "+v"(q3));
@@ -376,8 +382,13 @@
                     o[w].w = nb[b + 12] | (nb[b + 13] << 8) | (nb[b + 14] << 16) | (nb[b + 15] << 24);
                 }
                 STAMP(9);
-#pragma unroll
-                for (int w = 0; w < NWC; ++w) st_(st.qb, oq + 16u * w, o[w]);
+                int32_t abs_q = 0;
+                if constexpr (TQ) {
+                    const int32_t latest_q = pv * ((int)(rvm & 1u) - (int)((rvm >> 1) & 1u));
+                    abs_q = latest_q < 0 ? -latest_q : latest_q;
+                }
+#pragma unroll
+                for (int w = 0; w < NWC; ++w) gw_st_qw<DT, true>(st, o16, oq, w, o[w], tau, nbp, rvm, abs_q, dn);
             } else {
                 for (int i = 0; i < D; ++i) {
                     if (i == d) continue;
@@ -408,7 +419,7 @@
             now_out = t_end;
 
             st_(st.tw, o16, make_double2(t_end, wake));
-            st_(st.tk, o16, make_uint4(tau, nbp, rvm, (uint32_t)last_abs | (dn << 31)));
+            gw_st_tk<DT, true>(st, o16, tau, nbp, rvm, last_abs, dn);
         }
         STAMP(11);
         publish_env_counters(st.sa, N, e, k.pop, k.deliv, k_bad, fl, 1u);
@@ -430,7 +441,7 @@
     uint8_t* __restrict__ done = gw_global_at<uint8_t>(done_a);
     uint8_t* __restrict__ fb = gw_global_at<uint8_t>(fb_a);
     const int n_dev = (int)(dev_stage & 0xffu);
-    const GwState st = hdr_state<DT>(ip, tw, tk, qb, n_envs, n_dev);
+    const GwState st = hdr_state<DT, gw_tq_dt(DT)>(ip, tw, tk, qb, n_envs, n_dev);
     const GwDevConst c = hdr_const<DT>(ip, n_dev);
     double now_new;
     bool live;
@@ -445,7 +456,7 @@
                                                        double* __restrict__ angle_deg)
 {
     const int n_dev = (int)(dev_stage & 0xffu);
-    const GwState st = hdr_state<2>(ip, tw, tk, qb, n_envs, n_dev);
+    const GwState st = hdr_state<2, gw_tq_dt(2)>(ip, tw, tk, qb, n_envs, n_dev);
     const GwDevConst c = hdr_const<2>(ip, n_dev);
     constexpr int EPW = HALF ? 32 : 64;
     constexpr int NR = EPW / 16;
@@ -550,9 +561,13 @@
     if (e >= (uint32_t)st.N) return;
     const uint32_t o16 = e << 4;
     st_(st.tw, o16, make_double2(st.cst->start_time, st.cst->start_time));
-    st_(st.tk, o16, make_uint4(0u, 1u, 0u, 0u));
     st_(st.ip, o16, make_uint4(0u, 1u, 0u, 0u));
-    for (int b = 0; b < st.RB; ++b) st.qb[e * (uint32_t)st.RB + b] = 0;
+    if (st.tk) {
+        st_(st.tk, o16, make_uint4(0u, 1u, 0u, 0u));
+        for (int b = 0; b < st.RB; ++b) st.qb[e * (uint32_t)st.RB + b] = 0;
+    } else {
+        st_(st.tq, o16, make_uint4(0u, 0u, 0u, 1u));
+    }
     GwBp b0; b0.t0 = 0u; b0.c0 = 1u;
     st.bph[(size_t)e << 7] = b0;
     for (int w = 0; w < GW_SA_WORDS; ++w) st.sa[(size_t)w * st.N + e] = 0u;
@@ -566,13 +581,15 @@
     if (e >= n_envs) return;
     const uint8_t* base = reinterpret_cast<const uint8_t*>(ip) - gw_blob_header((int)n_dev);
     const GW_AS_CONST GwState* hs = (const GW_AS_CONST GwState*)(base + gw_hdr_st_off((int)n_dev));
-    uint32_t* tkp = gw_as_global(hs->tk);
+    const bool packed = hs->tk == nullptr;
+    uint32_t* tkp = gw_as_global(packed ? hs->tq : hs->tk);
     GwBp* bph = gw_as_global(hs->bph);
     const GW_AS_CONST GwDevConst* c = (const GW_AS_CONST GwDevConst*)(base + gw_hdr_cst_off((int)n_dev));
     const uint32_t o16 = e << 4;
     uint32_t rvm;
     if (!mask || mask[e]) {
-        uint4 tk = ld<uint4>(tkp, o16);
+        const uint4 rec = ld<uint4>(tkp, o16);
+        uint4 tk = packed ? make_uint4(rec.z, rec.w, 0u, 0u) : rec;
         uint4 bp = ld<uint4>(ip, o16);
         GwBp cur; cur.t0 = bp.x; cur.c0 = 0u;
         if (bp.x == tk.x) {
@@ -585,11 +602,16 @@
             tk.y += 1u; bp.x = cur.t0; bp.y = 0u;
         }
         tk.z = 0u; tk.w = 0u;
+        if (packed) {
+            const uint64_t f = gw_tq_set_done(gw_tq_set_la(gw_tq_set_rvm((uint64_t)rec.x | ((uint64_t)rec.y << 32), 0u), 0u), 0u);
+            tk = make_uint4((uint32_t)f, (uint32_t)(f >> 32), tk.x, tk.y);
+        }
         st_(tkp, o16, tk);
         st_(ip, o16, bp);
         rvm = 0u;
     } else {
-        rvm = ld<uint4>(tkp, o16).z;
+        const uint4 rec = ld<uint4>(tkp, o16);
+        rvm = packed ? gw_tq_rvm((uint64_t)rec.x | ((uint64_t)rec.y << 32)) : rec.z;
     }
     if (obs) obs[e] = c->payload_value * ((int)(rvm & 1u) - (int)((rvm >> 1) & 1u)) + c->counter_bound;
 }
@@ -601,7 +623,9 @@
     if (idx >= st.N * D) return;
     const uint32_t e = (uint32_t)(idx / D);
     const int i = (int)(idx - (int64_t)e * D);
-    const uint32_t rvm = ld<uint4>(st.tk, e << 4).z;
+    uint32_t rvm;
+    if (st.tk) rvm = ld<uint4>(st.tk, e << 4).z;
+    else { const uint4 rec = ld<uint4>(st.tq, e << 4); rvm = gw_tq_rvm((uint64_t)rec.x | ((uint64_t)rec.y << 32)); }
     out[idx] = ((rvm >> i) & 1u) ? st.cst->payload_value : 0;
 }
 
@@ -659,7 +683,7 @@
     const uint32_t dev_stage = (uint32_t)st.D | ((uint32_t)st.stage_chunks << 8);
     if (fns && fns->step[mode]) {
         gw_note_launch(rec, fns->step_slot + mode);
-        StepArgs a = {(uint64_t)st.ip, (uint64_t)st.tw, (uint64_t)st.tk, (uint64_t)st.qb, (uint64_t)device, (uint64_t)duration,
+        StepArgs a = {(uint64_t)st.ip, (uint64_t)st.tw, (uint64_t)gw_tk_or_tq(st), (uint64_t)st.qb, (uint64_t)device, (uint64_t)duration,
                       (uint32_t)st.N, dev_stage, (uint64_t)obs, (uint64_t)reward, (uint64_t)done, (uint64_t)fb};
         size_t size = sizeof a;
         void* extra[] = {HIP_LAUNCH_PARAM_BUFFER_POINTER, &a, HIP_LAUNCH_PARAM_BUFFER_SIZE, &size, HIP_LAUNCH_PARAM_END};
@@ -669,7 +693,7 @@
         gw_with_mode(mode, [&](auto m) {
             gw_note_launch(rec, GW_LS_STEP_SFX + 3 * gw_ls_dt(decltype(dt)::value) + decltype(m)::value);
             hipLaunchKernelGGL((ct_step_sfx_kernel<decltype(dt)::value, decltype(m)::value>), dim3(grid), dim3(64), 0, (hipStream_t)stream,
-                               (uint64_t)st.ip, (uint64_t)st.tw, (uint64_t)st.tk, (uint64_t)st.qb, (uint64_t)device, (uint64_t)duration,
+                               (uint64_t)st.ip, (uint64_t)st.tw, (uint64_t)gw_tk_or_tq(st), (uint64_t)st.qb, (uint64_t)device, (uint64_t)duration,
                                (uint32_t)st.N, dev_stage, (uint64_t)obs, (uint64_t)reward, (uint64_t)done, (uint64_t)fb);
         });
     });
diff --git a/gymwipe_amd/csrc/gw_api.cpp b/gymwipe_amd/csrc/gw_api.cpp
--- a/gymwipe_amd/csrc/gw_api.cpp
+++ b/gymwipe_amd/csrc/gw_api.cpp
@@ -189,8 +189,8 @@
                 int32_t* obs, float* reward, uint8_t* done, void* stream, uint8_t* fb, bool* fb_done)
 {
     if (fb_done) *fb_done = false;
-    if (env->dyn && env->st.tk) return gw_launch_step_dyn(env->st, env->cst_host, device, duration, obs, reward, done, stream, env->launches);
-    if (env->st.tk) {
+    if (env->dyn && env->st.tw) return gw_launch_step_dyn(env->st, env->cst_host, device, duration, obs, reward, done, stream, env->launches);
+    if (env->st.tw) {
         if (fb_done) *fb_done = true;
         return gw_launch_step_sfx(env->st, env->cst_host, device, duration, obs, reward, done, fb, stream, gw_env_below_limits(env, stream),
                                   env->launches, &env->fns);
@@ -252,16 +252,39 @@
 int gw_validate_config(const gw_config& cfg) { return validate(cfg); }
 
 struct GwEnvCounts { std::vector<uint64_t> steps, tx, deliv, app, pop, drop, bad; std::vector<uint32_t> flags; };
-static int derive_env_counts(gw_env* env, GwEnvCounts& c)
+static int read_tk_qb(const gw_env* env, std::vector<uint32_t>& tk, std::vector<uint8_t>& qb)
 {
     const GwState& st = env->st;
     const int64_t N = st.N;
     const int D = st.D, RB = st.RB;
-    std::vector<uint32_t> sa((size_t)N * GW_SA_WORDS + 2), tk((size_t)N * 4);
-    std::vector<uint8_t> qb((size_t)N * RB);
+    tk.assign((size_t)N * 4, 0u);
+    qb.assign((size_t)N * RB, 0);
+    if (st.tk) {
+        HIP_TRY(hipMemcpy(tk.data(), st.tk, tk.size() * sizeof(uint32_t), hipMemcpyDeviceToHost));
+        HIP_TRY(hipMemcpy(qb.data(), st.qb, qb.size(), hipMemcpyDeviceToHost));
+        return GW_OK;
+    }
+    std::vector<uint32_t> tq((size_t)N * 4);
+    HIP_TRY(hipMemcpy(tq.data(), st.tq, tq.size() * sizeof(uint32_t), hipMemcpyDeviceToHost));
+    for (int64_t e = 0; e < N; ++e) {
+        GwTqFields v;
+        gw_tq_unpack(&tq[(size_t)e * 4], D, v);
+        tk[(size_t)e * 4] = v.tau; tk[(size_t)e * 4 + 1] = v.nbp; tk[(size_t)e * 4 + 2] = v.rvm;
+        tk[(size_t)e * 4 + 3] = (uint32_t)gw_tq_last_abs(v.la, env->cfg.payload_value) | (v.done << 31);
+        for (int i = 0; i < D; ++i) qb[(size_t)e * RB + i] = (uint8_t)v.len[i];
+        for (int j = 0; j <= D; ++j) qb[(size_t)e * RB + D + j] = (uint8_t)v.state[j];
+    }
+    return GW_OK;
+}
+static int derive_env_counts(gw_env* env, GwEnvCounts& c)
+{
+    const GwState& st = env->st;
+    const int64_t N = st.N;
+    const int D = st.D, RB = st.RB;
+    std::vector<uint32_t> sa((size_t)N * GW_SA_WORDS + 2), tk;
+    std::vector<uint8_t> qb;
     HIP_TRY(hipMemcpy(sa.data(), st.sa, sa.size() * sizeof(uint32_t), hipMemcpyDeviceToHost));
-    HIP_TRY(hipMemcpy(tk.data(), st.tk, tk.size() * sizeof(uint32_t), hipMemcpyDeviceToHost));
-    HIP_TRY(hipMemcpy(qb.data(), st.qb, qb.size(), hipMemcpyDeviceToHost));
+    if (const int rc_rd = read_tk_qb(env, tk, qb)) return rc_rd;
     uint64_t mult_sum = 0;
     for (int i = 0; i < D; ++i) mult_sum += (uint64_t)env->cfg.mult[i];
     const uint64_t n_steps = (uint64_t)sa[(size_t)4 * N] | ((uint64_t)sa[(size_t)4 * N + 1] << 32);
@@ -309,7 +332,7 @@
 static int fused_chunks(gw_env* env, int32_t steps, void* stream, int32_t* s, F&& launch, int32_t longest)
 {
     const int32_t cap = env->st.rcap < longest ? env->st.rcap : longest;
-    while (env->st.tk && !env->dyn && cap > 0 && *s < steps) {
+    while (env->st.tw && !env->dyn && cap > 0 && *s < steps) {
         const int32_t chunk = steps - *s < cap ? steps - *s : cap;
         const bool below = gw_env_below_limits(env, stream) && env->t_bound + (double)(chunk + 1) * env->step_max < env->t_limit;
         const int rc = launch(*s, GwChunk{chunk, stream, below, env->launches});
@@ -380,11 +403,14 @@
         alloc(st.xw, N * 2);    alloc(st.xc, N * 4);    alloc(st.xs, N * st.XB);
         alloc(st.qrec, N * D);  alloc(st.runs, N * D * GW_RING_PHYS);
     } else {
+        const bool packed = !env->dyn && gw_tq_dt(D);
         st.RB = 16 * ((2 * D + 1 + 15) / 16);
-        alloc(st.tw, N * 2);   alloc(st.tk, N * 4);
+        alloc(st.tw, N * 2);
+        if (packed) alloc(st.tq, N * 4); else alloc(st.tk, N * 4);
         alloc(st.blob, (size_t)gw_blob_header(D) + (size_t)N * 16);
         if (!rc) st.ip = reinterpret_cast<uint32_t*>(const_cast<uint8_t*>(st.blob) + gw_blob_header(D));
-        alloc(st.qb, N * st.RB);  alloc(st.bph, N * GW_RING_PHYS);
+        if (!packed) alloc(st.qb, N * st.RB);
+        alloc(st.bph, N * GW_RING_PHYS);
         alloc(st.sa, N * GW_SA_WORDS + 2);
         const char* rc_env = getenv("GW_ROLLOUT_CAP");
         int cap = rc_env ? atoi(rc_env) : 64;
@@ -654,7 +680,7 @@
     if (!env) return fail(GW_EINVAL, "env is NULL");
     int rc = select_device(env);
     if (rc) return rc;
-    if (env->st.tk ? gw_launch_reset_sfx(env->st, mask_dev, obs_dev, stream, &env->fns)
+    if (env->st.tw ? gw_launch_reset_sfx(env->st, mask_dev, obs_dev, stream, &env->fns)
                     : gw_launch_reset(env->st, mask_dev, obs_dev, stream))
         return fail(GW_EHIP, "reset kernel launch failed");
     return GW_OK;
@@ -1214,7 +1240,7 @@
     if (!env || !out_dev) return fail(GW_EINVAL, "env/out is NULL");
     int rc = select_device(env);
     if (rc) return rc;
-    if (env->st.tk ? gw_launch_received_sfx(env->st, out_dev, stream) : gw_launch_received(env->st, out_dev, stream))
+    if (env->st.tw ? gw_launch_received_sfx(env->st, out_dev, stream) : gw_launch_received(env->st, out_dev, stream))
         return fail(GW_EHIP, "received kernel launch failed");
     return GW_OK;
 }
@@ -1321,6 +1347,8 @@
     GwSnapHeader h;
     memcpy(&h, src, sizeof h);
     if (h.magic != kSnapMagic || h.abi != (uint32_t)GW_ABI_VERSION || h.total != bytes) return fail(GW_EINVAL, "not a snapshot of this ABI");
+    if (h.nblocks < 0 || h.nblocks > (int32_t)(sizeof h.block_bytes / sizeof h.block_bytes[0]))
+        return fail(GW_EINVAL, "snapshot header claims %d blocks", (int)h.nblocks);
     gw_config a = h.cfg, b = env->cfg;
     a.hip_device = b.hip_device = 0;
     if (memcmp(&a, &b, sizeof a) != 0 || h.nblocks != env->nblocks_create || h.dyn != env->dyn)
@@ -1437,6 +1465,12 @@
     if (max_noise_states) *max_noise_states = mx;
     delete tab;
     return (k.fast_fmod ? 1 : 0) | (k.fast_div ? 2 : 0) | (k.fast_decide ? 4 : 0) | (k.idem_states ? 8 : 0) | (k.fast_ticks ? 16 : 0);
+}
+
+int gw_selftest_tq(int32_t num_devices)
+{
+    if (!gw_tq_dt(num_devices)) return fail(GW_EINVAL, "gw_selftest_tq: no packed record at %d senders", (int)num_devices);
+    return gw_tq_selftest(num_devices);
 }
 
 int gw_selftest_queue(uint64_t seed, int32_t operations, int32_t mult, int32_t counter_bound)
@@ -1620,7 +1654,7 @@
         return GW_OK;
     }
 #endif
-    if (st.tk) {
+    if (st.tw) {
         {
             static const char* names[6] = {"n_tx", "n_delivered", "n_appended", "n_popped", "n_dropped", "flags"};
             for (int k = 0; k < 6; ++k)
@@ -1636,12 +1670,11 @@
         }
         const int RB = st.RB;
         std::vector<double> tw((size_t)N * 2);
-        std::vector<uint32_t> tk((size_t)N * 4), ip((size_t)N * 4);
-        std::vector<uint8_t> qb((size_t)N * RB);
+        std::vector<uint32_t> tk, ip((size_t)N * 4);
+        std::vector<uint8_t> qb;
         HIP_TRY(hipMemcpy(tw.data(), st.tw, tw.size() * sizeof(double), hipMemcpyDeviceToHost));
-        HIP_TRY(hipMemcpy(tk.data(), st.tk, tk.size() * sizeof(uint32_t), hipMemcpyDeviceToHost));
+        if ((rc = read_tk_qb(env, tk, qb))) return rc;
         HIP_TRY(hipMemcpy(ip.data(), st.ip, ip.size() * sizeof(uint32_t), hipMemcpyDeviceToHost));
-        HIP_TRY(hipMemcpy(qb.data(), st.qb, qb.size(), hipMemcpyDeviceToHost));
         const uint32_t bound = (uint32_t)env->cfg.counter_bound;
         const int pv = env->cfg.payload_value;
         if (!strcmp(field, "now")) { NEED(N, double); double* o = (double*)dst; for (int64_t e = 0; e < N; ++e) o[e] = tw[e * 2]; return GW_OK; }
diff --git a/gymwipe_amd/csrc/gw_internal.h b/gymwipe_amd/csrc/gw_internal.h
--- a/gymwipe_amd/csrc/gw_internal.h
+++ b/gymwipe_amd/csrc/gw_internal.h
@@ -2,7 +2,9 @@
 #include <stdint.h>
 #include <stddef.h>
 #include <vector>
+#include <initializer_list>
 #include "../../include/gymwipe_amd.h"
+#include "gw_tq.h"
 
 #define GW_RING_PHYS      128
 #define GW_RING_MASK      (GW_RING_PHYS - 1)
@@ -45,7 +47,10 @@
 
     double*   xw;
     uint32_t* xc;
+    union {
     uint8_t*  xs;
+    uint32_t* tq;
+    };
     int32_t   XB;
     GwRec*    qrec;
     uint64_t* runs;
@@ -86,6 +91,7 @@
     double*   rxr;
     uint64_t* talk;
 };
+inline uint32_t* gw_tk_or_tq(const GwState& st) { return st.tk ? st.tk : st.tq; }
 #if defined(__HIPCC__)
 __host__ __device__
 #endif
@@ -325,6 +331,14 @@
 #define GW_DTS_LIVE          2, 3, 4, 6, 8, 16, 32
 #define GW_DTS_GENERIC       2, 3, 4, 8, 16
 #define GW_DTS_GENERIC_LIVE  4, 16
+constexpr bool gw_dts_has(int D, std::initializer_list<int> dts) { for (int v : dts) if (v == D) return true; return false; }
+constexpr bool gw_dts_cover_tq(std::initializer_list<int> dts)
+{
+    for (int D = 2; D <= GW_TQ_MAX_D; ++D) if (!gw_dts_has(D, dts)) return false;
+    return true;
+}
+static_assert(gw_dts_cover_tq({GW_DTS_STEP}) && gw_dts_cover_tq({GW_DTS_ROLLOUT_SYNC}) && gw_dts_cover_tq({GW_DTS_ROLLOUT_LOOP}),
+              "a packed sender count without a register instantiation in some suffix-kernel family");
 
 #define GW_LS_DTS GW_DTS_STEP, 0
 enum {
diff --git a/gymwipe_amd/csrc/gw_plant_api.cpp b/gymwipe_amd/csrc/gw_plant_api.cpp
--- a/gymwipe_amd/csrc/gw_plant_api.cpp
+++ b/gymwipe_amd/csrc/gw_plant_api.cpp
@@ -170,7 +170,7 @@
     const GwState* st = nullptr; const GwDevConst* cst = nullptr; int dev = 0;
     int rc = gw_env_internals(env, &st, &cst, &dev);
     if (rc) return rc;
-    if (!st->tk) return gw_set_error(GW_EUNSUPPORTED, "gw_pendulum_step needs the default (suffix) queue mode");
+    if (!st->tw) return gw_set_error(GW_EUNSUPPORTED, "gw_pendulum_step needs the default (suffix) queue mode");
     if (st->D != 2) return gw_set_error(GW_EUNSUPPORTED, "gw_pendulum_step: the env's network has two assignable devices (sensor, controller)");
     if (st->N != p->dev.N || dev != p->cfg.hip_device) return gw_set_error(GW_EINVAL, "env and plant differ in num_envs or hip_device");
     PLANT_HIP(hipSetDevice(dev), (void)0);
diff --git a/gymwipe_amd/csrc/gw_tq.h b/gymwipe_amd/csrc/gw_tq.h
--- /dev/null
+++ b/gymwipe_amd/csrc/gw_tq.h
@@ -0,0 +1,122 @@
+#pragma once
+#include <stdint.h>
+#include "../../include/gymwipe_amd.h"
+
+#ifndef GW_MAX_NSTATES
+#define GW_MAX_NSTATES 16
+#endif
+#if defined(__HIPCC__)
+#define GW_TQ_HD __host__ __device__ inline
+#else
+#define GW_TQ_HD inline
+#endif
+
+#define GW_TQ_MAX_D 4
+
+enum {
+    GW_TQ_LEN_BITS = 7, GW_TQ_STATE_BITS = 4,
+    GW_TQ_LEN_AT = 0,
+    GW_TQ_STATE_AT = GW_TQ_LEN_AT + GW_TQ_LEN_BITS * GW_TQ_MAX_D,
+    GW_TQ_RVM_AT = GW_TQ_STATE_AT + GW_TQ_STATE_BITS * (GW_TQ_MAX_D + 1),
+    GW_TQ_LA_AT = GW_TQ_RVM_AT + GW_TQ_MAX_D,
+    GW_TQ_DONE_AT = GW_TQ_LA_AT + 1,
+    GW_TQ_USED_BITS = GW_TQ_DONE_AT + 1
+};
+static_assert(GW_QUEUE_CAP < (1 << GW_TQ_LEN_BITS), "a queue length must fit its tq field");
+static_assert(GW_MAX_NSTATES <= (1 << GW_TQ_STATE_BITS), "a noise-state index must fit its tq field");
+static_assert(GW_TQ_MAX_D <= 4 && GW_TQ_USED_BITS <= 64, "the tq record's small fields must fit 64 bits");
+static_assert(GW_TQ_STATE_AT == 28 && GW_TQ_RVM_AT == 48 && GW_TQ_LA_AT == 52 && GW_TQ_DONE_AT == 53, "tq field positions (DESIGN section 4)");
+
+constexpr bool gw_tq_dt(int D) { return D >= 2 && D <= GW_TQ_MAX_D; }
+
+GW_TQ_HD uint32_t gw_tq_len(uint64_t f, uint32_t i) { return (uint32_t)(f >> (GW_TQ_LEN_AT + GW_TQ_LEN_BITS * i)) & ((1u << GW_TQ_LEN_BITS) - 1u); }
+GW_TQ_HD uint32_t gw_tq_state(uint64_t f, uint32_t j) { return (uint32_t)(f >> (GW_TQ_STATE_AT + GW_TQ_STATE_BITS * j)) & ((1u << GW_TQ_STATE_BITS) - 1u); }
+GW_TQ_HD uint32_t gw_tq_rvm(uint64_t f) { return (uint32_t)(f >> GW_TQ_RVM_AT) & ((1u << GW_TQ_MAX_D) - 1u); }
+GW_TQ_HD uint32_t gw_tq_la(uint64_t f) { return (uint32_t)(f >> GW_TQ_LA_AT) & 1u; }
+GW_TQ_HD uint32_t gw_tq_done(uint64_t f) { return (uint32_t)(f >> GW_TQ_DONE_AT) & 1u; }
+
+GW_TQ_HD uint64_t gw_tq_put(uint64_t f, int at, int bits, uint32_t v)
+{
+    const uint64_t m = ((1ull << bits) - 1ull) << at;
+    return (f & ~m) | (((uint64_t)v << at) & m);
+}
+GW_TQ_HD uint64_t gw_tq_set_len(uint64_t f, uint32_t i, uint32_t v) { return gw_tq_put(f, GW_TQ_LEN_AT + GW_TQ_LEN_BITS * (int)i, GW_TQ_LEN_BITS, v); }
+GW_TQ_HD uint64_t gw_tq_set_state(uint64_t f, uint32_t j, uint32_t v) { return gw_tq_put(f, GW_TQ_STATE_AT + GW_TQ_STATE_BITS * (int)j, GW_TQ_STATE_BITS, v); }
+GW_TQ_HD uint64_t gw_tq_set_rvm(uint64_t f, uint32_t v) { return gw_tq_put(f, GW_TQ_RVM_AT, GW_TQ_MAX_D, v); }
+GW_TQ_HD uint64_t gw_tq_set_la(uint64_t f, uint32_t v) { return gw_tq_put(f, GW_TQ_LA_AT, 1, v); }
+GW_TQ_HD uint64_t gw_tq_set_done(uint64_t f, uint32_t v) { return gw_tq_put(f, GW_TQ_DONE_AT, 1, v); }
+
+struct GwTqFields {
+    uint32_t len[GW_TQ_MAX_D], state[GW_TQ_MAX_D + 1];
+    uint32_t rvm, la, done, tau, nbp;
+};
+GW_TQ_HD void gw_tq_pack(const GwTqFields& v, int D, uint32_t out[4])
+{
+    uint64_t f = 0;
+    for (int i = 0; i < D; ++i) f = gw_tq_set_len(f, (uint32_t)i, v.len[i]);
+    for (int j = 0; j <= D; ++j) f = gw_tq_set_state(f, (uint32_t)j, v.state[j]);
+    f = gw_tq_set_rvm(f, v.rvm);
+    f = gw_tq_set_la(f, v.la);
+    f = gw_tq_set_done(f, v.done);
+    out[0] = (uint32_t)f; out[1] = (uint32_t)(f >> 32); out[2] = v.tau; out[3] = v.nbp;
+}
+GW_TQ_HD void gw_tq_unpack(const uint32_t in[4], int D, GwTqFields& v)
+{
+    const uint64_t f = (uint64_t)in[0] | ((uint64_t)in[1] << 32);
+    for (int i = 0; i < GW_TQ_MAX_D; ++i) v.len[i] = i < D ? gw_tq_len(f, (uint32_t)i) : 0u;
+    for (int j = 0; j <= GW_TQ_MAX_D; ++j) v.state[j] = j <= D ? gw_tq_state(f, (uint32_t)j) : 0u;
+    v.rvm = gw_tq_rvm(f); v.la = gw_tq_la(f); v.done = gw_tq_done(f);
+    v.tau = in[2]; v.nbp = in[3];
+}
+GW_TQ_HD int32_t gw_tq_last_abs(uint32_t la, int32_t payload_value) { return la ? (payload_value < 0 ? -payload_value : payload_value) : 0; }
+
+inline int gw_tq_selftest(int D)
+{
+    if (!gw_tq_dt(D)) return 1;
+    const uint32_t len_x[2] = {0u, (uint32_t)GW_QUEUE_CAP}, st_x[2] = {0u, (uint32_t)GW_MAX_NSTATES - 1u}, w_x[2] = {0u, 0xffffffffu};
+    int check = 2;
+    for (uint32_t rvm = 0; rvm < (1u << D); ++rvm)
+        for (int bits = 0; bits < 64; ++bits) {
+            GwTqFields v = {}, r = {};
+            for (int i = 0; i < D; ++i) v.len[i] = len_x[((bits >> 2) ^ i) & 1];
+            for (int j = 0; j <= D; ++j) v.state[j] = st_x[((bits >> 3) ^ j) & 1];
+            v.rvm = rvm; v.la = bits & 1; v.done = (bits >> 1) & 1; v.tau = w_x[(bits >> 4) & 1]; v.nbp = w_x[(bits >> 5) & 1];
+            uint32_t w[4];
+            gw_tq_pack(v, D, w);
+            if (((uint64_t)w[1] << 32 | w[0]) >> GW_TQ_USED_BITS) return check;
+            gw_tq_unpack(w, D, r);
+            for (int i = 0; i < GW_TQ_MAX_D; ++i) if (r.len[i] != (i < D ? v.len[i] : 0u)) return check + 1;
+            for (int j = 0; j <= GW_TQ_MAX_D; ++j) if (r.state[j] != (j <= D ? v.state[j] : 0u)) return check + 2;
+            if (r.rvm != v.rvm || r.la != v.la || r.done != v.done || r.tau != v.tau || r.nbp != v.nbp) return check + 3;
+        }
+    check = 10;
+    const uint64_t used = (1ull << GW_TQ_USED_BITS) - 1ull;
+    for (int bg = 0; bg < 2; ++bg) {
+        const uint64_t f0 = bg ? used : 0ull;
+        const int n_fields = D + (D + 1) + 3;
+        for (int k = 0; k < n_fields; ++k)
+            for (int x = 0; x < 2; ++x) {
+                uint64_t f = f0, mask;
+                uint32_t want;
+                if (k < D) { want = len_x[x]; f = gw_tq_set_len(f, (uint32_t)k, want); mask = 127ull << (7 * k); }
+                else if (k < 2 * D + 1) { const int j = k - D; want = st_x[x]; f = gw_tq_set_state(f, (uint32_t)j, want); mask = 15ull << (28 + 4 * j); }
+                else if (k == 2 * D + 1) { want = x ? 15u : 0u; f = gw_tq_set_rvm(f, want); mask = 15ull << 48; }
+                else if (k == 2 * D + 2) { want = (uint32_t)x; f = gw_tq_set_la(f, want); mask = 1ull << 52; }
+                else { want = (uint32_t)x; f = gw_tq_set_done(f, want); mask = 1ull << 53; }
+                if ((f ^ f0) & ~mask) return check;
+                if (f >> GW_TQ_USED_BITS) return check + 1;
+                const uint32_t got = k < D ? gw_tq_len(f, (uint32_t)k) : (k < 2 * D + 1 ? gw_tq_state(f, (uint32_t)(k - D))
+                                   : (k == 2 * D + 1 ? gw_tq_rvm(f) : (k == 2 * D + 2 ? gw_tq_la(f) : gw_tq_done(f))));
+                if (got != want) return check + 2;
+                for (int o = 0; o < n_fields; ++o) {
+                    if (o == k) continue;
+                    const uint32_t other = o < D ? gw_tq_len(f, (uint32_t)o) : (o < 2 * D + 1 ? gw_tq_state(f, (uint32_t)(o - D))
+                                         : (o == 2 * D + 1 ? gw_tq_rvm(f) : (o == 2 * D + 2 ? gw_tq_la(f) : gw_tq_done(f))));
+                    const uint32_t full = o < D ? 127u : (o <= 2 * D + 1 ? 15u : 1u);
+                    if (other != (bg ? full : 0u)) return check + 3;
+                }
+            }
+    }
+    if (gw_tq_last_abs(1u, -7) != 7 || gw_tq_last_abs(1u, 7) != 7 || gw_tq_last_abs(0u, 7) != 0) return 20;
+    return 0;
+}
diff --git a/include/gymwipe_amd.h b/include/gymwipe_amd.h
--- a/include/gymwipe_amd.h
+++ b/include/gymwipe_amd.h
@@ -345,6 +345,8 @@
 
 int gw_selftest_runq(uint64_t seed, int32_t operations, int32_t mult, int32_t counter_bound);
 
+int gw_selftest_tq(int32_t num_devices);
+
 int gw_selftest_fastmath(const gw_config* cfg, int32_t* max_noise_states);
 
 int64_t gw_selftest_launches(gw_env* env, char* out, int64_t cap);
```

After: 17.96 billion, median of 6. +2.7%, better.
